# skit-ai/N-Best-ASR-Transformer

Hardware: AMD Instinct MI355X
Metric: utterances/sec fine-tune (bert-base, seq128, n_best=5) (higher is better)
Workload: dtype bf16

## Files before the change

### include/nbest_hip.h

```cpp
#ifndef NBEST_HIP_H
#define NBEST_HIP_H

#include <stddef.h>
#include <stdint.h>

#ifdef __cplusplus
extern "C" {
#endif

#define NBEST_ABI_VERSION 1

enum { NBEST_OK = 0, NBEST_ERR_ARG = -1, NBEST_ERR_SHAPE = -2, NBEST_ERR_DTYPE = -3, NBEST_ERR_ALIGN = -4,
       NBEST_ERR_LAUNCH = -5, NBEST_ERR_WORKSPACE = -6 };
enum { NBEST_F32 = 0, NBEST_BF16 = 1 };

typedef void* nbest_stream_t;

int nbest_version(void);
int nbest_last_error(char* buf, size_t n);

int nbest_embed_ln_fwd(const int64_t* ids, const int64_t* seg, const int64_t* pos, const void* word,
                       const void* type, const void* ptab, const float* gamma, const float* beta, void* out,
                       float* stats, int64_t M, int H, float eps, int dtype, float drop_p, uint64_t seed,
                       uint32_t drop_stream, nbest_stream_t stream);
int nbest_embed_ln_bwd(const int64_t* ids, const int64_t* seg, const int64_t* pos, const int32_t* perm, const void* word,
                       const void* type, const void* ptab, const float* gamma, const float* stats,
                       const void* dout, float* dword, float* dtype_tab, float* dptab, float* dgamma,
                       float* dbeta, int B, int S, int H, int n_types, int dtype, int64_t word_pad_id,
                       int64_t pos_pad_id, int accumulate, int tables_accumulate, float drop_p, uint64_t seed,
                       uint32_t drop_stream, void* ws, size_t ws_bytes, nbest_stream_t stream);
size_t nbest_embed_bwd_ws_bytes(int64_t M, int64_t H);
int nbest_embed_ln_fwd_interp(const int64_t* ids, const int64_t* base_ids, const float* alpha, const int64_t* seg, const int64_t* pos,
                              const void* word, const void* type, const void* ptab, const float* gamma, const float* beta, void* out,
                              float* stats, int B, int S, int H, float eps, int dtype, float drop_p, uint64_t seed, uint32_t drop_stream,
                              nbest_stream_t stream);
int nbest_embed_attrib(const int64_t* ids, const int64_t* base_ids, const float* alpha, const int64_t* seg, const int64_t* pos,
                       const void* word, const void* type, const void* ptab, const float* gamma, const void* dhidden, float* attr,
                       int pairs, int m, int S, int H, float eps, int dtype, nbest_stream_t stream);

int nbest_rows_gather(const float* table, const int64_t* rows, int64_t n_rows, int64_t cap, int64_t* ids_out, float* vals_out, int H,
                      nbest_stream_t stream);
int nbest_rows_zero(float* table, const int64_t* ids, int64_t n, int H, nbest_stream_t stream);
int nbest_rows_add(float* table, const int64_t* ids, const float* vals, int64_t n, int H, nbest_stream_t stream);

enum {
  NBEST_EPI_NONE = 0,
  NBEST_EPI_BIAS = 1,
  NBEST_EPI_BIAS_GELU = 2,
  NBEST_EPI_BIAS_DROP_RES = 3,
  NBEST_EPI_DGELU = 4,
  NBEST_EPI_RES = 5,
  NBEST_EPI_F32_SPLITK = 6
};
typedef struct nbest_gemm_args {
  const void* A;
  const void* B;
  void* C;
  const float* bias;
  const void* R;
  void* U;
  void* ws;
  size_t ws_bytes;
  int64_t M, N, K;
  int64_t lda, ldb, ldc, ldr, ldu;
  int32_t trans_a, trans_b;
  int32_t epilogue;
  int32_t dtype;
  int32_t accumulate;
  float drop_p;
  uint32_t drop_stream;
  uint64_t seed;
  float* colsum_out;
  int32_t colsum_accumulate;
  int32_t flags;
  const void* B_packed;
  int32_t b_pack_bn;
  int32_t pad_;
} nbest_gemm_args;
#define NBEST_GEMM_DEFER_REDUCE 1
size_t nbest_gemm_ws_bytes(const nbest_gemm_args* a);
int nbest_gemm(const nbest_gemm_args* a, nbest_stream_t stream);

size_t nbest_wgrad_pair_ws_bytes(const nbest_gemm_args* a, const nbest_gemm_args* b);
int nbest_wgrad_pair(const nbest_gemm_args* a, const nbest_gemm_args* b, nbest_stream_t stream);
int nbest_wgrad_group(const nbest_gemm_args* problems, int n, nbest_stream_t stream);

typedef struct nbest_gemm_fp8_args {
  const void* A;
  const void* B;
  void* C;
  const float* bias;
  const void* R;
  void* U;
  void* C8;
  int64_t M, N, K;
  int64_t lda, ldb, ldc, ldr, ldu, ldc8;
  int32_t epilogue;
  float out_scale;
  float drop_p;
  uint32_t drop_stream;
  uint64_t seed;
  const float* out_scale_dev;
  const uint32_t* a_amax;
  const uint32_t* c8_amax_prev;
  uint32_t* c8_amax_new;
  float* colsum_out;
  int32_t colsum_accumulate;
  int32_t pad;
  void* ws;
  size_t ws_bytes;
  const void* B_packed;
  int32_t b_pack_bn;
  int32_t pad3;
} nbest_gemm_fp8_args;
size_t nbest_gemm_fp8_ws_bytes(const nbest_gemm_fp8_args* a);
int nbest_gemm_fp8(const nbest_gemm_fp8_args* a, nbest_stream_t stream);
size_t nbest_wgrad_fp8_ws_bytes(int64_t M, int64_t N, int64_t K);
int nbest_wgrad_fp8(const void* dY8, const void* X8, float* dW, int64_t M, int64_t N, int64_t K, int64_t lda, int64_t ldb,
                    int64_t ldc, const uint32_t* a_amax, const uint32_t* x_amax, int accumulate, void* ws, size_t ws_bytes,
                    nbest_stream_t stream);
size_t nbest_wgrad_fp8_pair_ws_bytes(int64_t Ma, int64_t Mb, int64_t N, int64_t K);
int nbest_wgrad_fp8_pair(const void* dY8a, const void* X8a, float* dWa, int64_t Ma, int64_t lda_a, int64_t ldb_a, int64_t ldc_a,
                         const uint32_t* amax_a, const uint32_t* xamax_a, const void* dY8b, const void* X8b, float* dWb, int64_t Mb,
                         int64_t lda_b, int64_t ldb_b, int64_t ldc_b, const uint32_t* amax_b, const uint32_t* xamax_b, int64_t N, int64_t K,
                         int accumulate, void* ws, size_t ws_bytes, nbest_stream_t stream);
int nbest_cast_bf16_to_fp8(const void* src, void* dst, int64_t n, nbest_stream_t stream);

int nbest_attention_fwd(const void* qkv, const uint8_t* key_mask, void* ctx, float* lse, int B, int S,
                        int heads, int d, int dtype, float drop_p, uint64_t seed, uint32_t drop_stream,
                        nbest_stream_t stream);
// ... 75 lines not shown
int nbest_adam_clip_coef(const float* partial, int n_partial, float max_grad_norm, float* clip, nbest_stream_t stream);
int nbest_adam_update(int mode, float* p, const float* g, float* m, float* v, void* p_lowp, const nbest_tensor_desc* descs,
                      int n_tensors, int n_blocks, int blk_lo, int blk_hi, const float* clip, float lr_mult, float bc1,
                      float bc2_sqrt, double b1, double b2, float eps, nbest_stream_t stream);
int nbest_adam_step(int mode, float* p, float* g, float* m, float* v, void* p_lowp, const nbest_tensor_desc* descs,
                    int n_tensors, int n_blocks, float lr_mult, float bc1, float bc2_sqrt, double b1, double b2, float eps,
                    float max_grad_norm, void* ws, size_t ws_bytes, nbest_stream_t stream);
typedef struct nbest_matrix_desc {
  int64_t offset;
  int32_t rows, cols;
  int32_t tile_start, pad;
} nbest_matrix_desc;
#define NBEST_AMAX_TENSOR_WORDS 1024
int nbest_fp8_amax_fold(void* slots, void* out, int32_t n_tensors, nbest_stream_t stream);
int nbest_quantize_weights_fp8(const float* master, void* w8, void* w8t, const nbest_matrix_desc* descs, int n_matrices,
                               int n_tiles, float* inv_scale, void* ws, size_t ws_bytes, nbest_stream_t stream);
int nbest_transpose_weights(const void* src, void* dst, const nbest_matrix_desc* descs, int n_matrices, int n_tiles,
                            nbest_stream_t stream);
int nbest_pack_bn(int64_t N);
int nbest_pack_bn_fp8(int64_t N, int64_t K);
int nbest_pack_weights_fp8(const void* src, void* dst, const nbest_matrix_desc* descs, int n_matrices, int n_stages, nbest_stream_t stream);
int nbest_pack_weights(const void* src, void* dst, const nbest_matrix_desc* descs, int n_matrices, int n_stages, nbest_stream_t stream);
int nbest_cast_f32_to_bf16(const float* src, void* dst, int64_t n, nbest_stream_t stream);

typedef struct nbest_layer_offsets {
  int64_t wqkv, bqkv, wo, bo, ln1_g, ln1_b, w1, b1, w2, b2, ln2_g, ln2_b;
} nbest_layer_offsets;
typedef struct nbest_encoder_desc {
  int32_t dtype, B, S, H, L, heads, F;
  int32_t vocab, max_pos, n_types;
  float ln_eps, hidden_drop, attn_drop;
  int64_t word_pad_id, pos_pad_id;
  int64_t off_word, off_pos, off_type, off_emb_ln_g, off_emb_ln_b;
  const nbest_layer_offsets* layers_host;
  uint64_t seed;
  uint32_t drop_stream_base;
  int32_t wgrad_events_n;
  void** wgrad_events;
  const void* w8;
  const float* w8_inv_scale;
  const void* w8t;
  const uint32_t* gamax_prev;
  uint32_t* gamax_new;
  int32_t fp8_bwd;
  int32_t pad2;
  const void* wpk;
  const void* wpkt;
  const void* w8p;
  const void* w8tp;
  const int32_t* word_perm;
  const uint32_t* aamax_prev;
  uint32_t* aamax_new;
  int32_t fp8_act;
  int32_t pad4;
  int32_t first_trainable;
  int32_t no_input_grad;
  const uint8_t* wgrad_skip_host;
  const int64_t* base_ids;
  const float* alpha;
  int32_t no_param_grad;
  int32_t wgrad_group;
} nbest_encoder_desc;
enum { NBEST_WGRAD_GROUP_PLAN = 0, NBEST_WGRAD_GROUP_NEVER = 1, NBEST_WGRAD_GROUP_ALWAYS = 2 };
size_t nbest_encoder_act_bytes(const nbest_encoder_desc* d);
int nbest_encoder_act_view(const nbest_encoder_desc* d, void* act, int layer, void** qkv, float** lse);
size_t nbest_encoder_ws_bytes(const nbest_encoder_desc* d);
int nbest_encoder_wgrad_launches_per_layer(const nbest_encoder_desc* d);
int nbest_encoder_forward(const nbest_encoder_desc* d, const void* wts, const float* prm, const int64_t* ids,
                          const int64_t* seg, const int64_t* pos, const uint8_t* key_mask, void* act,
                          size_t act_bytes, void* ws, size_t ws_bytes, void** hidden_out, nbest_stream_t stream);
int nbest_encoder_backward(const nbest_encoder_desc* d, const void* wts, const void* wts_t, const float* prm, float* grad,
                           const int64_t* ids, const int64_t* seg, const int64_t* pos, const uint8_t* key_mask,
                           void* act, size_t act_bytes, void* dhidden, void* ws, size_t ws_bytes, int accumulate,
                           int layer_begin, int layer_end, int with_embeddings, nbest_stream_t stream);

size_t nbest_encoder_infer_ws_bytes(const nbest_encoder_desc* d);
int nbest_encoder_infer(const nbest_encoder_desc* d, const void* wts, const float* prm, const int64_t* ids, const int64_t* seg,
                        const int64_t* pos, const uint8_t* key_mask, void* ws, size_t ws_bytes, void* cls_out, nbest_stream_t stream);
int nbest_encoder_infer_attn(const nbest_encoder_desc* d, const void* wts, const float* prm, const int64_t* ids, const int64_t* seg,
                             const int64_t* pos, const uint8_t* key_mask, void* ws, size_t ws_bytes, void* cls_out, float* cls_attn,
                             nbest_stream_t stream);

#ifdef __cplusplus
}
#endif
#endif
```

### n-best-asr-transformer_amd/csrc/common.h

```cpp
#pragma once
#include <hip/hip_runtime.h>
#include <stdint.h>
#include <math.h>

#include "../../include/nbest_hip.h"
#include "internal.h"

typedef __bf16 bf16;
typedef __attribute__((ext_vector_type(2))) __bf16 bf16x2;
typedef __attribute__((ext_vector_type(4))) __bf16 bf16x4;
typedef __attribute__((ext_vector_type(8))) __bf16 bf16x8;
typedef __attribute__((ext_vector_type(2))) float f32x2;
typedef __attribute__((ext_vector_type(4))) float f32x4;
typedef __attribute__((ext_vector_type(16))) float f32x16;
typedef __attribute__((ext_vector_type(4))) int i32x4;
typedef __attribute__((ext_vector_type(2))) int i32x2;

#define LDS_PTR(p) ((void __attribute__((address_space(3)))*)(p))

#define NB_CHECK(cond, code, ...)            \
  do {                                       \
    if (!(cond)) {                           \
      nbest_set_error(__VA_ARGS__);          \
      return (code);                         \
// ... 236 lines not shown

struct Fp8Grad {
  uint8_t* out8;
  const uint32_t* amax_prev;
  uint32_t* amax_new;
};
__host__ __device__ __forceinline__ float fp8_pow2_scale(float amax, float target) {
  if (!(amax >= 7.8886e-31f) || !(amax <= 3.0e38f)) return 1.f;
  const float e = floorf(log2f(target / amax));
  return exp2f(e < -100.f ? -100.f : (e > 100.f ? 100.f : e));
}
__host__ __device__ __forceinline__ float fp8_scale_of(float amax) { return fp8_pow2_scale(amax, 224.f); }
__host__ __device__ __forceinline__ float fp8_gscale_of(float amax) { return fp8_pow2_scale(amax, 56.f); }
__device__ __forceinline__ float fp8_grad_scale(const uint32_t* amax_prev) { return amax_prev ? fp8_gscale_of(__uint_as_float(*amax_prev)) : 1.f; }
__host__ __device__ __forceinline__ float fp8_ascale_of(float amax) { return fp8_pow2_scale(amax, 224.f); }
__device__ __forceinline__ float fp8_act_scale(const uint32_t* amax_prev) { return amax_prev ? fp8_ascale_of(__uint_as_float(*amax_prev)) : 1.f; }
constexpr int kAmaxSlots = 16, kAmaxSlotStride = NBEST_AMAX_TENSOR_WORDS / 16;
__device__ __forceinline__ void amax_update(uint32_t* p, float v) {
  p += ((blockIdx.x + 5 * blockIdx.y + 3 * blockIdx.z) & (kAmaxSlots - 1)) * kAmaxSlotStride;
  const uint32_t b = __float_as_uint(v);
  if (b > __hip_atomic_load(p, __ATOMIC_RELAXED, __HIP_MEMORY_SCOPE_AGENT)) atomicMax(p, b);
}

__device__ __forceinline__ uint32_t nb_hash32(uint32_t x) {
  x ^= x >> 16; x *= 0x7feb352dU; x ^= x >> 15; x *= 0x846ca68bU; x ^= x >> 16;
  return x;
}
struct DropCfg {
  uint32_t thr16;
  float scale;
  uint32_t key;
};
__host__ __device__ __forceinline__ uint32_t nb_mix_key(uint64_t seed, uint32_t stream) {
  uint64_t z = seed + 0x9E3779B97F4A7C15ULL * (uint64_t)(stream + 1);
  z = (z ^ (z >> 30)) * 0xBF58476D1CE4E5B9ULL;
  z = (z ^ (z >> 27)) * 0x94D049BB133111EBULL;
  return (uint32_t)(z ^ (z >> 31));
}
__device__ __forceinline__ bool nb_keep(const DropCfg& d, uint32_t idx) {
  const uint32_t h = nb_hash32((idx >> 1) * 0x9E3779B9U + d.key);
  const uint32_t u = (idx & 1) ? (h >> 16) : (h & 0xFFFFu);
  return u >= d.thr16;
}
__device__ __forceinline__ uint32_t nb_keep2(const DropCfg& d, uint32_t idx) {
  const uint32_t h = nb_hash32((idx >> 1) * 0x9E3779B9U + d.key);
  return ((h & 0xFFFFu) >= d.thr16 ? 1u : 0u) | ((h >> 16) >= d.thr16 ? 2u : 0u);
}
__device__ __forceinline__ uint32_t nb_keep4(const DropCfg& d, uint32_t idx) {
  const uint32_t h0 = nb_hash32((idx >> 1) * 0x9E3779B9U + d.key);
  const uint32_t h1 = nb_hash32(((idx >> 1) + 1) * 0x9E3779B9U + d.key);
  return ((h0 & 0xFFFFu) >= d.thr16 ? 1u : 0u) | ((h0 >> 16) >= d.thr16 ? 2u : 0u) |
         ((h1 & 0xFFFFu) >= d.thr16 ? 4u : 0u) | ((h1 >> 16) >= d.thr16 ? 8u : 0u);
}
static inline DropCfg make_drop(float p, uint64_t seed, uint32_t stream) {
  DropCfg d;
  uint32_t thr = (p <= 0.f) ? 0u : (uint32_t)lrintf(p * 65536.0f);
  if (thr > 65535u) thr = 65535u;
  d.thr16 = thr;
  d.scale = 65536.0f / (float)(65536u - thr);
  d.key = nb_mix_key(seed, stream);
  return d;
}
```

### n-best-asr-transformer_amd/csrc/encoder.hip

```cpp
#include <algorithm>

#include "common.h"

namespace {

static inline size_t al(size_t x) { return (x + 255) & ~(size_t)255; }
static inline size_t take(size_t& o, size_t bytes) { const size_t at = o; o += bytes; return at; }

struct Sizes {
  size_t esz, MH, MF, M3H, MH8, MF8, st, lse;
  int64_t M;
};

static Sizes sizes(const nbest_encoder_desc* d) {
  Sizes z;
  z.esz = d->dtype == NBEST_BF16 ? 2 : 4;
  z.M = (int64_t)d->B * d->S;
  const size_t MHe = (size_t)z.M * d->H, MFe = (size_t)z.M * d->F;
  z.MH = al(MHe * z.esz); z.MF = al(MFe * z.esz); z.M3H = al(3 * MHe * z.esz);
  z.MH8 = al(MHe); z.MF8 = al(MFe);
  z.st = al((size_t)z.M * 2 * sizeof(float));
  z.lse = al((size_t)d->B * d->heads * d->S * sizeof(float));
  return z;
}

struct ActLayout {
  size_t X, emb_stats, layer0, layer_stride;
  size_t o_qkv, o_ctx, o_lse, o_r1, o_st1, o_x1, o_u, o_hact, o_r2, o_st2;
  size_t o_x8, o_ctx8, o_x18, o_h8;
  size_t o_keep, keep_bytes;
  size_t total;
  int K;
};

static int first_trainable(const nbest_encoder_desc* d) { return d->first_trainable < 0 ? 0 : (d->first_trainable > d->L ? d->L : d->first_trainable); }

static ActLayout act_layout(const nbest_encoder_desc* d, const Sizes& z) {
  ActLayout a;
  const bool bf16 = d->dtype == NBEST_BF16;
  a.K = first_trainable(d);
  size_t o = 0, p = 0;
  a.X = take(o, (size_t)(d->L + 1 - a.K) * z.MH);
  a.emb_stats = take(o, a.K ? 0 : z.st);
  a.layer0 = o;
  a.o_qkv = take(p, z.M3H); a.o_ctx = take(p, z.MH); a.o_lse = take(p, z.lse);
  a.o_r1 = take(p, z.MH); a.o_st1 = take(p, z.st); a.o_x1 = take(p, z.MH);
  a.o_u = take(p, bf16 ? z.MF8 : z.MF);
  a.o_hact = take(p, z.MF); a.o_r2 = take(p, z.MH); a.o_st2 = take(p, z.st);
  a.keep_bytes = bf16 ? nbest_internal_attention_keep_bytes(d->B, d->S, d->heads) : 0;
  a.o_keep = take(p, al(a.keep_bytes));
  a.o_x8 = a.o_ctx8 = a.o_x18 = a.o_h8 = 0;
  if (d->w8) {
    a.o_x8 = take(p, z.MH8); a.o_ctx8 = take(p, z.MH8); a.o_x18 = take(p, z.MH8); a.o_h8 = take(p, z.MF8);
  }
  a.layer_stride = p;
  a.total = o + (size_t)(d->L - a.K) * p;
  return a;
}

struct WsLayout {
  size_t dR, dRd, dB1, dctx, dBig, dqkv, red, slab, slab_bytes, red_bytes, emb, emb_bytes, f8, f8_bytes, total;
  size_t gset[2][4];
  size_t fz_x0, fz_x1, fz_emb_stats, fz_lse, fz_st1, fz_st2, fz_u;
};

static nbest_gemm_args wgrad_args(int dtype, int64_t rows, int64_t cols, int64_t tokens) {
  nbest_gemm_args g = {};
  g.M = rows; g.N = cols; g.K = tokens; g.lda = rows; g.ldb = cols; g.ldc = cols;
  g.trans_a = g.trans_b = 1; g.epilogue = NBEST_EPI_F32_SPLITK; g.dtype = dtype;
  return g;
}

static size_t wgrad_pair_bytes(const nbest_encoder_desc* d, bool fp8) {
  const int64_t H = d->H, M = (int64_t)d->B * d->S;
  if (fp8) return nbest_wgrad_fp8_pair_ws_bytes(3 * H, H, H, M);
  const nbest_gemm_args g1 = wgrad_args(NBEST_BF16, 3 * H, H, M), g2 = wgrad_args(NBEST_BF16, H, H, M);
  return nbest_wgrad_pair_ws_bytes(&g1, &g2);
}

static size_t max_splitk_bytes(const nbest_encoder_desc* d, int64_t M) {
  size_t mx = 0;
  const int64_t shapes[4][2] = {{3 * (int64_t)d->H, d->H}, {d->H, d->H}, {d->F, d->H}, {d->H, d->F}};
  for (int i = 0; i < 4; ++i) {
    const nbest_gemm_args g = wgrad_args(d->dtype, shapes[i][0], shapes[i][1], M);
    mx = std::max(mx, nbest_gemm_ws_bytes(&g));
    if (d->dtype == NBEST_BF16 && shapes[i][0] % 256 == 0 && shapes[i][1] % 256 == 0)
      mx = std::max(mx, nbest_wgrad_fp8_ws_bytes(shapes[i][0], shapes[i][1], M));
  }
// ... 73 lines not shown
  if (d->dtype == NBEST_BF16)
    NB_CHECK(d->H % 128 == 0 && d->F % 128 == 0, NBEST_ERR_SHAPE, "encoder(bf16): H and F must be multiples of 128");
  if (d->w8) NB_CHECK(d->dtype == NBEST_BF16 && d->w8_inv_scale && d->H % 256 == 0 && d->H <= 1024 && d->F % 256 == 0, NBEST_ERR_SHAPE,
                      "encoder(fp8 forward): needs the bf16 path, inverse scales and H, F multiples of 256");
  NB_CHECK(0 <= d->first_trainable && d->first_trainable <= d->L, NBEST_ERR_ARG, "encoder: first_trainable %d outside [0, L=%d]",
           d->first_trainable, d->L);
  NB_CHECK(!d->base_ids == !d->alpha, NBEST_ERR_ARG, "encoder: interpolated embeddings need both base_ids and alpha (or neither)");
  return NBEST_OK;
}

struct Ptrs {
  const char* wts;
  const float* prm;
  size_t esz;
  const void* W(int64_t off) const { return wts + (size_t)off * esz; }
  const float* P(int64_t off) const { return prm + off; }
};

#define RUN(x) do { int rc__ = (x); if (rc__) return rc__; } while (0)

static nbest_gemm_args gemm_nt(int dtype, const void* A, const void* B, void* C, int64_t M, int64_t N, int64_t K) {
  nbest_gemm_args g = {};
  g.A = A; g.B = B; g.C = C; g.dtype = dtype;
  g.M = M; g.N = N; g.K = K; g.lda = K; g.ldb = K; g.ldc = N;
  return g;
}

static void use_packed(nbest_gemm_args& g, const void* arena, int64_t off) {
  if (!arena || g.dtype != NBEST_BF16 || g.trans_a || g.trans_b) return;
  g.B_packed = (const char*)arena + off * 2;
  g.b_pack_bn = nbest_pack_bn(g.N);
}
static void use_packed(nbest_gemm_fp8_args& g, const void* arena, int64_t off) {
  if (!arena) return;
  g.B_packed = (const uint8_t*)arena + off;
  g.b_pack_bn = nbest_pack_bn_fp8(g.N, g.K);
}

struct GemmPass {
  int dtype; int64_t M; nbest_stream_t stream;
  uint64_t seed;
  Ptrs W; const void* packed; bool b_kn;
  bool fp8; const void *w8, *w8_packed; const float* inv_scale; const uint32_t* amax_prev; uint32_t* amax_new;
  void* colsum_ws; size_t colsum_ws_bytes; int accumulate;
};
struct GemmOp {
  const void* A; const uint8_t* A8; int a_idx;
  int64_t w_off; int mat;
  void* C; int64_t N, K; int epilogue;
  const float* bias;
  const void* R; float drop_p; uint32_t drop_stream;
  void* U; float* colsum;
  uint8_t* C8; int c_idx;
};

static int layer_gemm(const GemmPass& c, const GemmOp& o) {
  if (c.fp8) {
    nbest_gemm_fp8_args g = {};
    g.A = o.A8; g.B = (const uint8_t*)c.w8 + o.w_off; g.C = o.C; g.bias = o.bias; g.R = o.R; g.U = o.U; g.C8 = o.C8;
    g.M = c.M; g.N = o.N; g.K = o.K;
    g.lda = g.ldb = o.K; g.ldc = g.ldr = g.ldu = g.ldc8 = o.N;
    use_packed(g, c.w8_packed, o.w_off);
    g.epilogue = o.epilogue; g.out_scale = 1.f; g.out_scale_dev = c.inv_scale + o.mat;
    g.drop_p = o.drop_p; g.drop_stream = o.drop_stream; g.seed = c.seed;
    g.a_amax = c.amax_prev + o.a_idx;
    if (o.C8) {
      g.c8_amax_prev = c.amax_prev + o.c_idx;
      g.c8_amax_new = c.amax_new ? c.amax_new + (int64_t)o.c_idx * NBEST_AMAX_TENSOR_WORDS : nullptr;
    }
    g.colsum_out = o.colsum; g.colsum_accumulate = c.accumulate; g.ws = c.colsum_ws; g.ws_bytes = c.colsum_ws_bytes;
    return nbest_gemm_fp8(&g, c.stream);
  }
  nbest_gemm_args g = gemm_nt(c.dtype, o.A, c.W.W(o.w_off), o.C, c.M, o.N, o.K);
  if (c.b_kn) { g.trans_b = 1; g.ldb = o.N; }
  g.epilogue = o.epilogue; g.bias = o.bias;
  if (o.R) { g.R = o.R; g.ldr = o.N; }
  if (o.epilogue == NBEST_EPI_BIAS_DROP_RES) { g.drop_p = o.drop_p; g.drop_stream = o.drop_stream; g.seed = c.seed; }
  if (o.epilogue == NBEST_EPI_BIAS_GELU || o.epilogue == NBEST_EPI_DGELU) { g.U = o.U; g.ldu = o.N; }
  if (o.epilogue == NBEST_EPI_DGELU) {
    g.colsum_out = o.colsum; g.colsum_accumulate = g.accumulate = c.accumulate; g.ws = c.colsum_ws; g.ws_bytes = c.colsum_ws_bytes;
  }
  use_packed(g, c.packed, o.w_off);
  return nbest_gemm(&g, c.stream);
}

struct LayerBufs {
  void *qkv, *ctx, *r1, *x1, *u, *hact, *r2;
  float *lse, *st1, *st2;
  uint32_t* keep;
  uint8_t *x8, *ctx8, *x18, *h8;
};

static LayerBufs stashed_layer(const nbest_encoder_desc* d, const ActLayout& a, void* act, int l) {
  char* Lb = (char*)act + a.layer0 + (size_t)(l - a.K) * a.layer_stride;
  LayerBufs b = {};
  b.qkv = Lb + a.o_qkv; b.ctx = Lb + a.o_ctx; b.lse = (float*)(Lb + a.o_lse);
  b.r1 = Lb + a.o_r1; b.st1 = (float*)(Lb + a.o_st1); b.x1 = Lb + a.o_x1;
  b.u = Lb + a.o_u; b.r2 = Lb + a.o_r2; b.st2 = (float*)(Lb + a.o_st2);
  b.hact = fp8_backward_active(d) ? nullptr : Lb + a.o_hact;
  if (a.keep_bytes && d->attn_drop > 0.f) b.keep = (uint32_t*)(Lb + a.o_keep);
  if (fp8_forward_active(d)) {
    b.x8 = (uint8_t*)(Lb + a.o_x8); b.ctx8 = (uint8_t*)(Lb + a.o_ctx8);
    b.x18 = (uint8_t*)(Lb + a.o_x18); b.h8 = (uint8_t*)(Lb + a.o_h8);
  }
  return b;
}

static LayerBufs frozen_layer(const nbest_encoder_desc* d, const WsLayout& w, const Sizes& z, void* ws) {
  char* W = (char*)ws;
  const bool f8 = fp8_forward_active(d);
  LayerBufs b = {};
  b.qkv = W + w.dqkv; b.ctx = W + w.dctx; b.lse = (float*)(W + w.fz_lse);
  b.r1 = W + w.dR; b.st1 = (float*)(W + w.fz_st1); b.x1 = W + w.dRd;
  b.r2 = W + w.dB1; b.st2 = (float*)(W + w.fz_st2);
  b.u = f8 ? W + w.fz_u : nullptr; b.hact = f8 ? nullptr : W + w.dBig;
  if (f8) { b.x8 = (uint8_t*)(W + w.f8); b.ctx8 = b.x8 + z.MH8; b.x18 = b.ctx8 + z.MH8; b.h8 = b.x18 + z.MH8; }
  return b;
}

struct Fwd {
  const nbest_encoder_desc* d;
  GemmPass g;
  const uint8_t* key_mask;
  bool arec;
  const uint32_t* AP(int idx) const { return g.fp8 ? d->aamax_prev + idx : nullptr; }
  uint32_t* AN(int idx) const { return (g.fp8 && arec) ? d->aamax_new + (int64_t)idx * NBEST_AMAX_TENSOR_WORDS : nullptr; }
  int calib(const void* t, int64_t n, int idx) const {
    if (!arec || g.fp8) return NBEST_OK;
    return nbest_internal_amax_bf16(t, n, d->aamax_new + (int64_t)idx * NBEST_AMAX_TENSOR_WORDS, (hipStream_t)g.stream);
  }
};

static Fwd make_fwd(const nbest_encoder_desc* d, const void* wts, const float* prm, const Sizes& z, const uint8_t* key_mask,
                    nbest_stream_t stream) {
  const GemmPass g = {d->dtype, z.M, stream, d->seed, Ptrs{(const char*)wts, prm, z.esz}, d->wpk, false, fp8_forward_active(d),
                      d->w8, d->w8p, d->w8_inv_scale, d->aamax_prev, d->aamax_new, nullptr, 0, 0};
  return Fwd{d, g, key_mask, d->w8 && d->aamax_new && d->dtype == NBEST_BF16};
}

static int layer_forward(const Fwd& c, int l, const void* xin, void* xout, const LayerBufs& b, uint8_t* x8_next, float* cls_probs) {
  const nbest_encoder_desc* d = c.d;
  const nbest_layer_offsets& o = d->layers_host[l];
  const Ptrs& P = c.g.W;
  const nbest_stream_t stream = c.g.stream;
  const int64_t M = c.g.M;
  const int H = d->H, F = d->F, dt = d->dtype, t = 4 * l;
  const uint32_t s0 = d->drop_stream_base + 1 + 4 * l;
  if (c.g.fp8 && l == 0)
    RUN(nbest_internal_cast_bf16_to_fp8(xin, b.x8, M * H, c.AP(0), c.AN(0), (hipStream_t)stream));
  const GemmOp wqkv = {xin, b.x8, t + 0, o.wqkv, t + 0, b.qkv, 3 * H, H, NBEST_EPI_BIAS, P.P(o.bqkv)};
  RUN(layer_gemm(c.g, wqkv));
  if (cls_probs)
    RUN(nbest_internal_attention_cls_probs(b.qkv, (int64_t)d->S * H * 3, (const char*)b.qkv + H * P.esz, 3 * H, c.key_mask, cls_probs, d->S,
                                           d->B, d->S, d->heads, 64, dt, stream));
  RUN(c.calib(xin, M * H, t + 0));
  RUN(nbest_internal_attention_fwd8(b.qkv, c.key_mask, b.ctx, b.ctx8, b.lse, d->B, d->S, d->heads, 64, dt, d->attn_drop, d->seed, s0 + 0,
                                    stream, b.keep, c.AP(t + 1), c.AN(t + 1)));
  RUN(c.calib(b.ctx, M * H, t + 1));
  GemmOp wo = {b.ctx, b.ctx8, t + 1, o.wo, t + 1, b.r1, H, H, NBEST_EPI_BIAS_DROP_RES, P.P(o.bo)};
  wo.R = xin; wo.drop_p = d->hidden_drop; wo.drop_stream = s0 + 1;
  RUN(layer_gemm(c.g, wo));
  RUN(nbest_internal_layernorm_fwd8(b.r1, P.P(o.ln1_g), P.P(o.ln1_b), b.x1, b.x18, b.st1, M, H, d->ln_eps, dt, stream, c.AP(t + 2), c.AN(t + 2)));
  RUN(c.calib(b.x1, M * H, t + 2));
  GemmOp w1 = {b.x1, b.x18, t + 2, o.w1, t + 2, b.hact, F, H, NBEST_EPI_BIAS_GELU, P.P(o.b1)};
  w1.U = b.u; w1.C8 = b.h8; w1.c_idx = t + 3;
  RUN(layer_gemm(c.g, w1));
  GemmOp w2 = {b.hact, b.h8, t + 3, o.w2, t + 3, b.r2, H, F, NBEST_EPI_BIAS_DROP_RES, P.P(o.b2)};
  w2.R = b.x1; w2.drop_p = d->hidden_drop; w2.drop_stream = s0 + 2;
  RUN(layer_gemm(c.g, w2));
  RUN(c.calib(b.hact, M * F, t + 3));
  RUN(nbest_internal_layernorm_fwd8(b.r2, P.P(o.ln2_g), P.P(o.ln2_b), xout, x8_next, b.st2, M, H, d->ln_eps, dt, stream,
                                    x8_next ? c.AP(t + 4) : nullptr, x8_next ? c.AN(t + 4) : nullptr));
  return NBEST_OK;
}

}

extern "C" size_t nbest_encoder_act_bytes(const nbest_encoder_desc* d) { return d ? act_layout(d, sizes(d)).total : 0; }

extern "C" int nbest_encoder_act_view(const nbest_encoder_desc* d, void* act, int layer, void** qkv, float** lse) {
  RUN(check_desc(d));
  NB_CHECK(act && qkv && lse, NBEST_ERR_ARG, "encoder_act_view: null pointer");
  NB_CHECK(0 <= layer && layer < d->L, NBEST_ERR_ARG, "encoder_act_view: layer %d outside [0, L=%d)", layer, d->L);
  const ActLayout a = act_layout(d, sizes(d));
  NB_CHECK(layer >= a.K, NBEST_ERR_ARG, "encoder_act_view: layer %d < first_trainable %d (frozen layers are not stashed)", layer, a.K);
  const LayerBufs b = stashed_layer(d, a, act, layer);
  *qkv = b.qkv; *lse = b.lse;
  return NBEST_OK;
}
extern "C" size_t nbest_encoder_ws_bytes(const nbest_encoder_desc* d) { return d ? ws_layout(d, sizes(d)).total : 0; }
extern "C" int nbest_encoder_wgrad_launches_per_layer(const nbest_encoder_desc* d) {
  if (!d) return 0;
  if (wgrad_group_layers(d) > 0) return 1;
  return wgrad_paired(d, fp8_backward_active(d)) ? 3 : 4;
}

extern "C" int nbest_encoder_forward(const nbest_encoder_desc* d, const void* wts, const float* prm, const int64_t* ids,
                                     const int64_t* seg, const int64_t* pos, const uint8_t* key_mask, void* act, size_t act_bytes,
                                     void* ws, size_t ws_bytes, void** hidden_out, nbest_stream_t stream) {
  RUN(check_desc(d));
  NB_CHECK(wts && prm && ids && pos && key_mask && act, NBEST_ERR_ARG, "encoder_forward: null pointer");
  const Sizes z = sizes(d);
  const ActLayout a = act_layout(d, z);
  NB_CHECK(act_bytes >= a.total, NBEST_ERR_WORKSPACE, "encoder_forward: activation stash too small (%zu < %zu)", act_bytes, a.total);
  const Fwd c = make_fwd(d, wts, prm, z, key_mask, stream);
  const WsLayout wl = ws_layout(d, z);
  const int FT = a.K;
  if (c.g.fp8 || FT > 0)
    NB_CHECK(ws && ws_bytes >= wl.total, NBEST_ERR_WORKSPACE, "encoder_forward(%s): workspace too small (%zu < %zu)",
             FT > 0 ? "first_trainable > 0" : "fp8", ws_bytes, wl.total);
  const Ptrs& P = c.g.W;
  char *A = (char*)act, *W = (char*)ws;
  const int H = d->H, dt = d->dtype;
  auto X = [&](int l) { return l >= FT ? (void*)(A + a.X + (size_t)(l - FT) * z.MH) : (void*)(W + ((l & 1) ? wl.fz_x1 : wl.fz_x0)); };
  auto bufs = [&](int l) { return l >= FT ? stashed_layer(d, a, act, l) : frozen_layer(d, wl, z, ws); };

  float* emb_stats = (float*)(FT > 0 ? W + wl.fz_emb_stats : A + a.emb_stats);
  if (d->base_ids)
    RUN(nbest_embed_ln_fwd_interp(ids, d->base_ids, d->alpha, seg, pos, P.W(d->off_word), P.W(d->off_type), P.W(d->off_pos),
                                  P.P(d->off_emb_ln_g), P.P(d->off_emb_ln_b), X(0), emb_stats, d->B, d->S, H, d->ln_eps, dt,
                                  d->hidden_drop, d->seed, d->drop_stream_base, (hipStream_t)stream));
  else
    RUN(nbest_embed_ln_fwd(ids, seg, pos, P.W(d->off_word), P.W(d->off_type), P.W(d->off_pos), P.P(d->off_emb_ln_g),
                           P.P(d->off_emb_ln_b), X(0), emb_stats, z.M, H, d->ln_eps, dt, d->hidden_drop, d->seed, d->drop_stream_base,
                           (hipStream_t)stream));
  for (int l = 0; l < d->L; ++l) {
    uint8_t* x8_next = (l + 1 < d->L) ? bufs(l + 1).x8 : nullptr;
    RUN(layer_forward(c, l, X(l), X(l + 1), bufs(l), x8_next, nullptr));
  }
  if (hidden_out) *hidden_out = X(d->L);
  return NBEST_OK;
}

namespace {
struct WGrad {
  const void *dY, *X;
  const uint8_t *dY8, *X8;
  int64_t w_off, rows, cols;
  int g_idx, a_idx;
};
}

extern "C" int nbest_encoder_backward(const nbest_encoder_desc* d, const void* wts, const void* wts_t, const float* prm, float* grad,
                                      const int64_t* ids, const int64_t* seg, const int64_t* pos, const uint8_t* key_mask,
                                      void* act, size_t act_bytes, void* dhidden, void* ws, size_t ws_bytes, int accumulate,
                                      int layer_begin, int layer_end, int with_embeddings, nbest_stream_t stream) {
  RUN(check_desc(d));
  NB_CHECK(0 <= layer_begin && layer_begin <= layer_end && layer_end <= d->L, NBEST_ERR_ARG, "encoder_backward: bad layer range");
  const bool npg = d->no_param_grad != 0;
  NB_CHECK(!npg || (!with_embeddings && d->first_trainable == 0 && !d->no_input_grad && !d->w8), NBEST_ERR_ARG,
           "encoder_backward: no_param_grad refuses with_embeddings (%d), first_trainable > 0 (%d), no_input_grad (%d) and the fp8 "
           "forward (w8): it forms the input gradient only, of a full stash", with_embeddings, d->first_trainable, d->no_input_grad);
  NB_CHECK(wts && prm && (grad || npg) && ids && pos && key_mask && act && dhidden && ws, NBEST_ERR_ARG, "encoder_backward: null pointer");
  NB_CHECK(!with_embeddings || d->word_perm, NBEST_ERR_ARG, "encoder_backward: desc.word_perm (stable argsort of this pass's ids) is required");
  NB_CHECK(layer_begin >= d->first_trainable, NBEST_ERR_ARG, "encoder_backward: layer_begin %d < first_trainable %d (those layers are not stashed)",
           layer_begin, d->first_trainable);
  NB_CHECK(!with_embeddings || (d->first_trainable == 0 && !d->no_input_grad), NBEST_ERR_ARG,
           "encoder_backward: with_embeddings needs first_trainable == 0 and no_input_grad == 0");
  const Sizes z = sizes(d);
  const ActLayout a = act_layout(d, z);
  const WsLayout w = ws_layout(d, z);
  NB_CHECK(act_bytes >= a.total, NBEST_ERR_WORKSPACE, "encoder_backward: activation stash too small");
  NB_CHECK(ws_bytes >= w.total, NBEST_ERR_WORKSPACE, "encoder_backward: workspace too small (%zu < %zu)", ws_bytes, w.total);
  hipStream_t st = (hipStream_t)stream;
  const Ptrs P{(const char*)wts, prm, z.esz};
  const bool wt = (wts_t != nullptr);
  char *A = (char*)act, *W = (char*)ws;
  const int64_t M = z.M;
  const int H = d->H, F = d->F, dt = d->dtype;
  const int FT = a.K;
  auto X = [&](int l) { return (void*)(A + a.X + (size_t)(l - FT) * z.MH); };
  auto G = [&](int64_t off) { return grad + off; };
  auto GP = [&](int64_t off) -> float* { return npg ? nullptr : grad + off; };
  auto skip = [&](int l, int j) -> bool { return npg || (d->wgrad_skip_host && d->wgrad_skip_host[4 * l + j]); };
  void* dA = dhidden; void* dR = W + w.dR;
  const bool hdrop = d->hidden_drop > 0.f;
  void* dRd = hdrop ? (void*)(W + w.dRd) : dR;
  void* dB1 = W + w.dB1; void* dctx = W + w.dctx; void* dBig = W + w.dBig; void* dqkv = W + w.dqkv;
  void* red = W + w.red; void* slab = W + w.slab;
  void* red1 = W + w.red + w.red_bytes; void* red2 = W + w.red + 2 * w.red_bytes; void* red3 = W + w.red + 3 * w.red_bytes;
  const bool f8b = fp8_backward_active(d);
  const bool paired = wgrad_paired(d, f8b);
  const int gl = wgrad_group_layers(d);
  const bool grouped = gl > 0;
  int ev_i = (grouped ? 1 : paired ? 3 : 4) * (d->L - layer_end);
  auto stamp = [&](int which) {
    if (d->wgrad_events && 2 * ev_i + which < d->wgrad_events_n) (void)hipEventRecord((hipEvent_t)d->wgrad_events[2 * ev_i + which], st);
    ev_i += which;
  };

  const bool rec = !npg && d->gamax_new && dt == NBEST_BF16;
  uint8_t* dqkv8 = f8b ? (uint8_t*)W + w.f8 : nullptr;
  uint8_t* dBig8 = f8b ? dqkv8 + 3 * z.MH8 : nullptr;
  uint8_t* dRd8 = f8b ? dBig8 + z.MF8 : nullptr;
  auto GN = [&](int idx) { return d->gamax_new + (int64_t)idx * NBEST_AMAX_TENSOR_WORDS; };
  auto fg = [&](uint8_t* out8, int idx) -> Fp8Grad {
    if (!rec) return Fp8Grad{nullptr, nullptr, nullptr};
    return Fp8Grad{f8b ? out8 : nullptr, f8b ? d->gamax_prev + idx : nullptr, GN(idx)};
  };
  const GemmPass dg = {dt, M, stream, 0, Ptrs{(const char*)(wt ? wts_t : wts), prm, z.esz}, wt ? d->wpkt : nullptr, !wt, f8b,
                       d->w8t, d->w8tp, d->w8_inv_scale, d->gamax_prev, d->gamax_new, red1, w.red_bytes, accumulate};
  auto wgrad_args_of = [&](const WGrad* x) {
    nbest_gemm_args g = wgrad_args(dt, x->rows, x->cols, M);
    g.A = x->dY; g.B = x->X; g.C = G(x->w_off); g.accumulate = accumulate;
    return g;
  };
  auto wgrad_launch = [&](int l, const WGrad* wg, int j, int j2) -> int {
    const WGrad* p = skip(l, j) ? nullptr : wg + j;
    const WGrad* q = (j2 >= 0 && !skip(l, j2)) ? wg + j2 : nullptr;
    if (!p) { p = q; q = nullptr; }
    if (p && f8b) {
      const uint32_t *gp = d->gamax_prev, *ap = d->aamax_prev;
      if (q)
        RUN(nbest_wgrad_fp8_pair(p->dY8, p->X8, G(p->w_off), p->rows, p->rows, p->cols, p->cols, gp + p->g_idx, ap + p->a_idx, q->dY8, q->X8,
                                 G(q->w_off), q->rows, q->rows, q->cols, q->cols, gp + q->g_idx, ap + q->a_idx, p->cols, M, accumulate, slab,
                                 w.slab_bytes, stream));
      else
        RUN(nbest_wgrad_fp8(p->dY8, p->X8, G(p->w_off), p->rows, p->cols, M, p->rows, p->cols, p->cols, gp + p->g_idx, ap + p->a_idx,
                            accumulate, slab, w.slab_bytes, stream));
    } else if (p) {
      nbest_gemm_args g1 = wgrad_args_of(p), g2 = wgrad_args_of(q ? q : p);
      g1.ws = slab; g1.ws_bytes = w.slab_bytes;
      RUN(q ? nbest_wgrad_pair(&g1, &g2, stream) : nbest_gemm(&g1, stream));
    }
    return NBEST_OK;
  };
  auto wgrad = [&](int l, const WGrad* wg, int j, int j2) -> int {
    stamp(0);
    RUN(wgrad_launch(l, wg, j, j2));
    stamp(1);
    return NBEST_OK;
  };
  nbest_gemm_args pend[8];
  int n_pend = 0;

  struct BatchGuard { ~BatchGuard() { nbest_internal_rowred_batch_abort(); } } batch_guard;
  for (int l = layer_end - 1; l >= layer_begin; --l) {
    const nbest_layer_offsets& o = d->layers_host[l];
    const LayerBufs b = stashed_layer(d, a, act, l);
    const bool input_grad = !(d->no_input_grad && l == FT);
    const int t = 4 * l;
    const uint32_t s0 = d->drop_stream_base + 1 + 4 * l;
    const int gpos = grouped ? (layer_end - 1 - l) % gl : 0;
    const bool group_ends = grouped && (gpos == gl - 1 || l == layer_begin);
    void *dR2 = dR, *dR1 = dR, *dRd2 = dRd, *dRd1 = dRd, *dBigL = dBig, *dqkvL = dqkv;
    if (grouped) {
      dRd2 = W + w.gset[gpos][0]; dBigL = W + w.gset[gpos][1]; dRd1 = W + w.gset[gpos][2]; dqkvL = W + w.gset[gpos][3];
      if (!hdrop) { dR2 = dRd2; dR1 = dRd1; }
    }
    const WGrad wg[4] = {{dqkvL, X(l), dqkv8, b.x8, o.wqkv, 3 * H, H, t + 3, t + 0},
                         {dRd1, b.ctx, dRd8, b.ctx8, o.wo, H, H, t + 2, t + 1},
                         {dBigL, b.x1, dBig8, b.x18, o.w1, F, H, t + 1, t + 2},
                         {dRd2, b.hact, dRd8, b.h8, o.w2, H, F, t + 0, t + 3}};
    if (!npg) nbest_internal_rowred_batch_begin();
    RUN(nbest_internal_layernorm_bwd8(dA, b.r2, b.st2, P.P(o.ln2_g), dR2, (hdrop && !f8b) ? dRd2 : nullptr, GP(o.ln2_g), GP(o.ln2_b), GP(o.b2), M, H,
                                      dt, accumulate, d->hidden_drop, d->seed, s0 + 2, red, w.red_bytes, stream, fg(dRd8, t + 0)));
    GemmOp dw2 = {dRd2, dRd8, t + 0, o.w2, t + 3, f8b ? nullptr : dBigL, F, H, NBEST_EPI_DGELU};
    dw2.U = b.u; dw2.colsum = GP(o.b1); dw2.C8 = dBig8; dw2.c_idx = t + 1;
    RUN(layer_gemm(dg, dw2));
    if (rec && !f8b) RUN(nbest_internal_amax_bf16(dBigL, M * F, GN(t + 1), st));
    if (!grouped) RUN(wgrad(l, wg, 3, -1));
    GemmOp dw1 = {dBigL, dBig8, t + 1, o.w1, t + 2, dB1, H, F, NBEST_EPI_RES};
    dw1.R = dR2;
    RUN(layer_gemm(dg, dw1));
    if (!grouped) RUN(wgrad(l, wg, 2, -1));
    RUN(nbest_internal_layernorm_bwd8(dB1, b.r1, b.st1, P.P(o.ln1_g), dR1, (hdrop && !f8b) ? dRd1 : nullptr, GP(o.ln1_g), GP(o.ln1_b), GP(o.bo), M, H,
                                      dt, accumulate, d->hidden_drop, d->seed, s0 + 1, red2, w.red_bytes, stream, fg(dRd8, t + 2)));
    const GemmOp dwo = {dRd1, dRd8, t + 2, o.wo, t + 1, dctx, H, H, NBEST_EPI_NONE};
    RUN(layer_gemm(dg, dwo));
    if (!paired && !grouped) RUN(wgrad(l, wg, 1, -1));
    RUN(nbest_internal_attention_bwd8(b.qkv, key_mask, b.ctx, dctx, b.lse, f8b ? nullptr : dqkvL, GP(o.bqkv), accumulate, red3, w.red_bytes, d->B, d->S,
                                      d->heads, 64, dt, d->attn_drop, d->seed, s0 + 0, stream, fg(dqkv8, t + 3), b.keep));
    if (input_grad) {
      GemmOp dwqkv = {dqkvL, dqkv8, t + 3, o.wqkv, t + 0, dA, H, 3 * H, NBEST_EPI_RES};
      dwqkv.R = dR1;
      RUN(layer_gemm(dg, dwqkv));
    }
    if (!grouped) {
      RUN(wgrad(l, wg, 0, paired ? 1 : -1));
    } else if (group_ends && gpos + 1 < gl && d->wgrad_group != NBEST_WGRAD_GROUP_ALWAYS) {
      stamp(0);
      RUN(wgrad_launch(l, wg, 3, -1));
      RUN(wgrad_launch(l, wg, 2, -1));
      if (!paired) RUN(wgrad_launch(l, wg, 1, -1));
      RUN(wgrad_launch(l, wg, 0, paired ? 1 : -1));
      stamp(1);
    } else {
      for (int j = 0; j < 4; ++j)
        if (!skip(l, j)) pend[n_pend++] = wgrad_args_of(wg + j);
      if (group_ends) {
        stamp(0);
        if (n_pend) RUN(nbest_wgrad_group(pend, n_pend, stream));
        stamp(1);
        for (int i = 0; i < gpos; ++i) { stamp(0); stamp(1); }
        n_pend = 0;
      }
    }
    if (!npg) RUN(nbest_internal_rowred_batch_flush(st));
  }
  if (!with_embeddings) return NBEST_OK;
  if (!accumulate) {
    hipError_t e = hipMemsetAsync(G(d->off_word), 0, (size_t)d->vocab * H * sizeof(float), st);
    if (e == hipSuccess) e = hipMemsetAsync(G(d->off_pos), 0, (size_t)d->max_pos * H * sizeof(float), st);
    if (e == hipSuccess) e = hipMemsetAsync(G(d->off_type), 0, (size_t)d->n_types * H * sizeof(float), st);
    NB_CHECK(e == hipSuccess, NBEST_ERR_LAUNCH, "encoder_backward: memset failed: %s", hipGetErrorString(e));
  }
  RUN(nbest_embed_ln_bwd(ids, seg, pos, d->word_perm, P.W(d->off_word), P.W(d->off_type), P.W(d->off_pos), P.P(d->off_emb_ln_g),
                         (const float*)(A + a.emb_stats), dA, G(d->off_word), G(d->off_type), G(d->off_pos), G(d->off_emb_ln_g),
                         G(d->off_emb_ln_b), d->B, d->S, H, d->n_types, dt, d->word_pad_id, d->pos_pad_id, accumulate, accumulate,
                         d->hidden_drop, d->seed, d->drop_stream_base, W + w.emb, w.emb_bytes, stream));
  return NBEST_OK;
}

namespace {
struct InferLayout {
  size_t X0, X1, emb_stats, qkv, ctx, r1, x1, r2, hact, lse, st1, st2, total;
};
static InferLayout infer_layout(const Sizes& z) {
  InferLayout w;
  size_t o = 0;
  w.X0 = take(o, z.MH); w.X1 = take(o, z.MH); w.emb_stats = take(o, z.st);
  w.qkv = take(o, z.M3H); w.ctx = take(o, z.MH); w.r1 = take(o, z.MH); w.x1 = take(o, z.MH); w.r2 = take(o, z.MH);
  w.hact = take(o, z.MF); w.lse = take(o, z.lse); w.st1 = take(o, z.st); w.st2 = take(o, z.st);
  w.total = o;
  return w;
}
static LayerBufs infer_layer(const InferLayout& w, void* ws) {
  char* W = (char*)ws;
  LayerBufs b = {};
  b.qkv = W + w.qkv; b.ctx = W + w.ctx; b.lse = (float*)(W + w.lse);
  b.r1 = W + w.r1; b.st1 = (float*)(W + w.st1); b.x1 = W + w.x1;
  b.hact = W + w.hact; b.r2 = W + w.r2; b.st2 = (float*)(W + w.st2);
  return b;
}
}

extern "C" size_t nbest_encoder_infer_ws_bytes(const nbest_encoder_desc* d) { return d ? infer_layout(sizes(d)).total : 0; }

extern "C" int nbest_encoder_infer_attn(const nbest_encoder_desc* d, const void* wts, const float* prm, const int64_t* ids, const int64_t* seg,
                                        const int64_t* pos, const uint8_t* key_mask, void* ws, size_t ws_bytes, void* cls_out,
                                        float* cls_attn, nbest_stream_t stream) {
  RUN(check_desc(d));
// ... 54 lines not shown
```

### n-best-asr-transformer_amd/csrc/gemm.hip

```cpp
#include "common.h"

namespace {

__global__ __launch_bounds__(256) void splitk_reduce_kernel(const float* __restrict__ slab, float* __restrict__ C, int64_t MN,
                                                            int64_t N, int64_t ldc, int splits, int accumulate,
                                                            float* __restrict__ C2, int64_t m_split, int64_t ldc2) {
  for (int64_t i = ((int64_t)blockIdx.x * blockDim.x + threadIdx.x) * 4; i < MN; i += (int64_t)gridDim.x * blockDim.x * 4) {
    f32x4 s = *(const f32x4*)(slab + i);
    for (int z = 1; z < splits; ++z) s += *(const f32x4*)(slab + (int64_t)z * MN + i);
    const int64_t m = i / N, n = i - m * N;
    float* c = (m < m_split) ? C + m * ldc + n : C2 + (m - m_split) * ldc2 + n;
    if (accumulate) s += *(const f32x4*)c;
    *(f32x4*)c = s;
  }
}

int check_epilogue_operands(const nbest_gemm_args* a, int64_t ld_mult, uintptr_t align) {
  const int epi = a->epilogue;
  if (epi == NBEST_EPI_BIAS || epi == NBEST_EPI_BIAS_GELU || epi == NBEST_EPI_BIAS_DROP_RES)
    NB_CHECK(a->bias, NBEST_ERR_ARG, "gemm: epilogue %d needs bias", epi);
  if (epi == NBEST_EPI_BIAS_DROP_RES || epi == NBEST_EPI_RES)
    NB_CHECK(a->R && a->ldr % ld_mult == 0 && ((uintptr_t)a->R & (align - 1)) == 0, NBEST_ERR_ARG, "gemm: epilogue %d needs R", epi);
  if ((epi == NBEST_EPI_BIAS_GELU && a->U) || epi == NBEST_EPI_DGELU)
    NB_CHECK(a->U && a->ldu % ld_mult == 0 && ((uintptr_t)a->U & (align - 1)) == 0, NBEST_ERR_ARG, "gemm: epilogue %d needs U", epi);
  return NBEST_OK;
}

int check_bf16(const nbest_gemm_args* a) {
  NB_CHECK(!(a->trans_a && !a->trans_b), NBEST_ERR_ARG, "gemm(bf16): trans_a without trans_b is not built");
  NB_CHECK(!a->trans_a || a->M % 128 == 0, NBEST_ERR_SHAPE, "gemm(bf16): trans_a needs M %% 128 == 0");
  NB_CHECK(a->lda % 8 == 0 && a->ldb % 8 == 0 && a->ldc % 8 == 0, NBEST_ERR_ALIGN, "gemm(bf16): leading dimensions must be multiples of 8");
  NB_CHECK(((uintptr_t)a->A & 15) == 0 && ((uintptr_t)a->B & 15) == 0 && ((uintptr_t)a->C & 15) == 0, NBEST_ERR_ALIGN,
           "gemm(bf16): pointers must be 16-byte aligned");
  const int64_t a_rows = a->trans_a ? a->K : a->M, a_cols = a->trans_a ? a->M : a->K;
  const int64_t b_rows = a->trans_b ? a->K : a->N, b_cols = a->trans_b ? a->N : a->K;
  const int64_t ab = ((a_rows - 1) * a->lda + a_cols) * 2, bb = ((b_rows - 1) * a->ldb + b_cols) * 2;
  NB_CHECK(ab < ((int64_t)1 << 32) && bb < ((int64_t)1 << 32), NBEST_ERR_SHAPE, "gemm(bf16): operand larger than 4 GiB");
  NB_CHECK(a->M * a->N < ((int64_t)1 << 32) || make_drop(a->drop_p, a->seed, a->drop_stream).thr16 == 0, NBEST_ERR_SHAPE,
           "gemm(bf16): dropout counter overflow");
  return check_epilogue_operands(a, 8, 16);
}

}

void nb_splitk_plan(int64_t tiles, int64_t K, int64_t slots, int64_t min_blocks, int* splits, int64_t* k_per_split) {
  const int64_t maxs = (K / 512 < 1) ? 1 : ((K / 512 > 32) ? 32 : K / 512);
  int64_t best_s = 1;
  double best = -1.0;
  for (int64_t s = 1; s <= maxs; ++s) {
    const int64_t blocks = tiles * s;
    const double eff = (double)blocks / (double)(((blocks + slots - 1) / slots) * slots);
    if (eff > best + 1e-9) { best = eff; best_s = s; }
    if (blocks >= min_blocks && eff >= 0.93) { best_s = s; break; }
  }
  const int64_t k = round_up((K + best_s - 1) / best_s, 64);
  *splits = (int)((K + k - 1) / k);
  *k_per_split = k;
}

int nbest_internal_splitk_reduce(const float* slab, float* C, int64_t M, int64_t N, int64_t ldc, int splits, int accumulate,
                                 float* C2, int64_t m_split, int64_t ldc2, hipStream_t st) {
  const int64_t MN = M * N;
  int64_t g = (MN / 4 + 255) / 256;
  if (g > 2048) g = 2048;
  splitk_reduce_kernel<<<(int)g, 256, 0, st>>>(slab, C, MN, N, ldc, splits, accumulate, C2, m_split, ldc2);
  NB_LAUNCH_CHECK();
  return NBEST_OK;
}

extern "C" size_t nbest_gemm_ws_bytes(const nbest_gemm_args* a) {
  if (!a) return 0;
  if (a->dtype == NBEST_F32) return (a->colsum_out && a->epilogue != NBEST_EPI_F32_SPLITK) ? nbest_rowred_ws_bytes(a->M, a->N) : 0;
  if (a->dtype != NBEST_BF16) return 0;
  const size_t w1 = nbest_gemm_bf16_ws_bytes(a), w2 = nbest_gemm_bf16_v2_ws_bytes(a);
  return w1 > w2 ? w1 : w2;
}

extern "C" int nbest_gemm(const nbest_gemm_args* a, nbest_stream_t stream) {
  NB_CHECK(a && a->A && a->B && a->C, NBEST_ERR_ARG, "gemm: null pointer");
  NB_CHECK(a->M > 0 && a->N > 0 && a->K > 0, NBEST_ERR_SHAPE, "gemm: bad shape %lld x %lld x %lld", (long long)a->M,
           (long long)a->N, (long long)a->K);
  if (a->dtype == NBEST_F32) {
    if (int rc = check_epilogue_operands(a, 1, 1)) return rc;
    if (int rc = nbest_gemm_f32(a, (hipStream_t)stream)) return rc;
    if (a->colsum_out && a->epilogue != NBEST_EPI_F32_SPLITK) {
      NB_CHECK(a->ws && a->ws_bytes >= nbest_rowred_ws_bytes(a->M, a->N), NBEST_ERR_WORKSPACE, "gemm(f32): column-sum workspace too small");
      return nbest_colsum(a->C, a->colsum_out, a->M, a->N, a->ldc, NBEST_F32, a->colsum_accumulate, a->ws, a->ws_bytes, stream);
    }
    return NBEST_OK;
  }
  if (a->dtype == NBEST_BF16) {
    if (int rc = check_bf16(a)) return rc;
// ... 43 lines not shown
```

### n-best-asr-transformer_amd/csrc/gemm_bf16.hip

```cpp
#include "common.h"

namespace {

constexpr int BM = 128, BN = 128, BK = 64;
constexpr int kTileBytes = BM * BK * 2;
constexpr int kStageBytes = 2 * kTileBytes;
constexpr int kLdsBytes = 2 * kStageBytes;

struct GemmP {
  const bf16* A; const bf16* B; void* C; const float* bias; const bf16* R; bf16* U; float* slab; float* colpart;
  int64_t M, N, K, lda, ldb, ldc, ldr, ldu;
  int64_t k_per_split;
  int tiles_m, tiles_n, splits, accumulate;
  uint32_t a_bytes, b_bytes;
  DropCfg drop;
  int stream_out;
  int gn;
};

template <bool TR>
__device__ __forceinline__ void stage_tile(__amdgpu_buffer_rsrc_t rs, char* lds_tile, int64_t row0, int64_t k0, int64_t ld,
                                           int tid) {
  const int wave = tid >> 6;
#pragma unroll
  for (int i = 0; i < 4; ++i) {
    const int p = i * 256 + tid;
    uint32_t voff;
    if (!TR) {
      const int row = p >> 3, slot = p & 7;
      const int kc = slot ^ ((row >> 1) & 7);
      voff = (uint32_t)(((row0 + row) * ld + k0 + kc * 8) * 2);
    } else {
      const int krow = p >> 4, slot = p & 15;
      const int mc = slot ^ (2 * (krow & 3) + 8 * ((krow >> 3) & 1));
      voff = (uint32_t)(((k0 + krow) * ld + row0 + mc * 8) * 2);
    }
    char* dst = lds_tile + (i * 256 + wave * 64) * 16;
    __builtin_amdgcn_raw_ptr_buffer_load_lds(rs, LDS_PTR(dst), 16, voff, 0, 0, 0);
  }
}

template <bool TR>
__device__ __forceinline__ bf16x8 read_frag(const char* lds_tile, int row_base, int ks, int lane) {
  if (!TR) {
    const int row = row_base + (lane & 15);
    const int kc = (lane >> 4) + 4 * ks;
    return *(const bf16x8*)(lds_tile + row * 128 + ((kc ^ ((row >> 1) & 7)) << 4));
  } else {
    const int g = lane >> 4, i = lane & 15, q = i >> 2, pq = i & 3;
    const int col = row_base + 4 * pq;
    bf16x8 out;
#pragma unroll
    for (int half = 0; half < 2; ++half) {
      const int krow = 32 * ks + 8 * g + 4 * half + q;
      const int f = 2 * (krow & 3) + 8 * ((krow >> 3) & 1);
      const char* addr = lds_tile + krow * 256 + (((col >> 3) ^ f) << 4) + ((col & 4) ? 8 : 0);
      bf16x4 v = __builtin_amdgcn_ds_read_tr16_b64_v4bf16((bf16x4 __attribute__((address_space(3)))*)addr);
      out[4 * half + 0] = v[0]; out[4 * half + 1] = v[1]; out[4 * half + 2] = v[2]; out[4 * half + 3] = v[3];
    }
    return out;
  }
}

template <bool TA, bool TB, int EPI>
__global__ __launch_bounds__(256) void gemm_bf16_kernel(GemmP p) {
// ... 64 lines not shown
      }
      if (kt + 1 < nk) {
        char* nxt = lds + ((kt + 1) & 1) * kStageBytes;
        const int64_t k0 = kbeg + (int64_t)(kt + 1) * BK;
        stage_tile<TA>(rsA, nxt, m0, k0, p.lda, tid);
        stage_tile<TB>(rsB, nxt + kTileBytes, n0, k0, p.ldb, tid);
      }
#pragma unroll
      for (int ks = 0; ks < 2; ++ks)
#pragma unroll
        for (int i = 0; i < 4; ++i)
#pragma unroll
          for (int j = 0; j < 4; ++j)
            acc[i][j] = __builtin_amdgcn_mfma_f32_16x16x32_bf16(bfr[ks][j], af[ks][i], acc[i][j], 0, 0, 0);
    } else {
      if (kt + 1 < nk) {
        char* nxt = lds + ((kt + 1) & 1) * kStageBytes;
        const int64_t k0 = kbeg + (int64_t)(kt + 1) * BK;
        stage_tile<TA>(rsA, nxt, m0, k0, p.lda, tid);
        stage_tile<TB>(rsB, nxt + kTileBytes, n0, k0, p.ldb, tid);
      }
#pragma unroll
      for (int ks = 0; ks < 2; ++ks) {
        bf16x8 af[4], bfr[4];
#pragma unroll
        for (int i = 0; i < 4; ++i) af[i] = read_frag<TA>(cur, wm * 64 + i * 16, ks, lane);
#pragma unroll
        for (int j = 0; j < 4; ++j) bfr[j] = read_frag<TB>(cur + kTileBytes, wn * 64 + j * 16, ks, lane);
#pragma unroll
        for (int i = 0; i < 4; ++i)
#pragma unroll
          for (int j = 0; j < 4; ++j)
            acc[i][j] = __builtin_amdgcn_mfma_f32_16x16x32_bf16(bfr[j], af[i], acc[i][j], 0, 0, 0);
      }
    }
  }

  __syncthreads();
  float* ep = (float*)lds + wave * 4096;
#pragma unroll
  for (int i = 0; i < 4; ++i) {
    const int row = i * 16 + (lane & 15);
#pragma unroll
    for (int j = 0; j < 4; ++j) {
      const int c = j * 4 + (lane >> 4);
      *(f32x4*)(ep + row * 64 + ((c ^ (row & 15)) << 2)) = acc[i][j];
    }
  }
  asm volatile("s_waitcnt lgkmcnt(0)" ::: "memory");
  float colacc[8] = {0, 0, 0, 0, 0, 0, 0, 0};
  const int64_t er0 = m0 + wm * 64 + (lane >> 3), ec8 = n0 + wn * 64 + (lane & 7) * 8;
  int64_t oC = er0 * p.ldc + ec8, oU = er0 * p.ldu + ec8, oS = ((int64_t)z * p.M + er0) * p.N + ec8;
  const int64_t sC = 8 * p.ldc, sU = 8 * p.ldu, sS = 8 * p.N;
  uint32_t dbase = (uint32_t)(er0 * p.N + ec8);
  const uint32_t sD = 8u * (uint32_t)p.N;
#pragma unroll
  for (int it = 0; it < 8; ++it, oC += sC, oU += sU, oS += sS, dbase += sD) {
    const int pidx = it * 64 + lane, row = pidx >> 3, c8 = pidx & 7;
    const int64_t m = m0 + wm * 64 + row;
    f32x4 v0 = *(const f32x4*)(ep + row * 64 + (((2 * c8) ^ (row & 15)) << 2));
    f32x4 v1 = *(const f32x4*)(ep + row * 64 + (((2 * c8 + 1) ^ (row & 15)) << 2));
    if (m >= p.M) continue;
    if (EPI == NBEST_EPI_F32_SPLITK) {
      float* c = (p.splits > 1) ? p.slab + oS : (float*)p.C + oC;
      if (p.splits == 1 && p.accumulate) { v0 += *(const f32x4*)c; v1 += *(const f32x4*)(c + 4); }
      *(f32x4*)c = v0;
      *(f32x4*)(c + 4) = v1;
      continue;
    }
    float v[8] = {v0[0], v0[1], v0[2], v0[3], v1[0], v1[1], v1[2], v1[3]};
    if (kHasBias) {
#pragma unroll
      for (int e = 0; e < 4; ++e) { v[e] += pb0[e]; v[4 + e] += pb1[e]; }
    }
    if (EPI == kEpiBiasGeluNoU) {
#pragma unroll
      for (int e = 0; e < 8; e += 2) {
        f32x2 h2, g2;
        gelu_pair_fast(f32x2{v[e], v[e + 1]}, h2, g2);
        v[e] = h2[0]; v[e + 1] = h2[1];
      }
    }
    if (EPI == NBEST_EPI_BIAS_GELU) {
      float gp[8];
#pragma unroll
      for (int e = 0; e < 8; e += 2) {
        f32x2 h2, g2;
        gelu_pair_fast(f32x2{v[e], v[e + 1]}, h2, g2);
        gp[e] = g2[0]; gp[e + 1] = g2[1]; v[e] = h2[0]; v[e + 1] = h2[1];
      }
      st_stream((i32x2*)((uint8_t*)p.U + oU), i32x2{(int)gd_pack4(gp), (int)gd_pack4(gp + 4)}, p.stream_out);
    }
    if (EPI == NBEST_EPI_BIAS_DROP_RES) {
      if (p.drop.thr16) {
        const uint32_t k = nb_keep4(p.drop, dbase) | (nb_keep4(p.drop, dbase + 4) << 4);
#pragma unroll
        for (int e = 0; e < 8; ++e) v[e] = (k >> e & 1) ? v[e] * p.drop.scale : 0.f;
      }
    }
    if (EPI == NBEST_EPI_BIAS_DROP_RES || EPI == NBEST_EPI_RES) {
      const bf16x8 r = __builtin_bit_cast(bf16x8, pre[it]);
#pragma unroll
      for (int e = 0; e < 8; ++e) v[e] += (float)r[e];
    }
    if (EPI == NBEST_EPI_DGELU) {
      float gd[8];
      gd_unpack4((uint32_t)pre[it][0], gd);
      gd_unpack4((uint32_t)pre[it][1], gd + 4);
// ... 27 lines not shown
  if (a->epilogue == NBEST_EPI_F32_SPLITK) nb_splitk_plan(((a->M + BM - 1) / BM) * (a->N / BN), a->K, 512, 400, splits, kps);
}

template <bool TA, bool TB>
static int launch_epi(const GemmP& p, int epi, int grid, hipStream_t st) {
#define L(E)                                                                          \
  case E:                                                                             \
    (void)hipFuncSetAttribute((const void*)gemm_bf16_kernel<TA, TB, E>, hipFuncAttributeMaxDynamicSharedMemorySize, kLdsBytes); \
    gemm_bf16_kernel<TA, TB, E><<<grid, 256, kLdsBytes, st>>>(p);                      \
    break;
  switch (epi) {
    L(NBEST_EPI_NONE) L(NBEST_EPI_BIAS) L(NBEST_EPI_BIAS_GELU) L(NBEST_EPI_BIAS_DROP_RES) L(NBEST_EPI_DGELU)
    L(NBEST_EPI_RES) L(NBEST_EPI_F32_SPLITK) L(kEpiBiasGeluNoU)
    default:
      nbest_set_error("gemm: bad epilogue %d", epi);
      return NBEST_ERR_ARG;
  }
#undef L
  NB_LAUNCH_CHECK();
  return NBEST_OK;
}

}

size_t nbest_gemm_bf16_ws_bytes(const nbest_gemm_args* a) {
  if (a->epilogue != NBEST_EPI_F32_SPLITK) return a->colsum_out ? (size_t)((a->M + BM - 1) / BM) * 2 * a->N * sizeof(float) : 0;
  int splits;
  int64_t kps;
  plan_splits(a, &splits, &kps);
  return splits > 1 ? (size_t)splits * a->M * a->N * sizeof(float) : 0;
}

int nbest_gemm_bf16(const nbest_gemm_args* a, hipStream_t st) {
  NB_CHECK(a->N % BN == 0, NBEST_ERR_SHAPE, "gemm(bf16): N=%lld must be a multiple of %d", (long long)a->N, BN);
  NB_CHECK(a->trans_a || a->K % BK == 0, NBEST_ERR_SHAPE, "gemm(bf16): K=%lld must be a multiple of %d", (long long)a->K, BK);
  GemmP p;
  p.A = (const bf16*)a->A; p.B = (const bf16*)a->B; p.C = a->C; p.bias = a->bias; p.R = (const bf16*)a->R; p.U = (bf16*)a->U;
  p.M = a->M; p.N = a->N; p.K = a->K; p.lda = a->lda; p.ldb = a->ldb; p.ldc = a->ldc; p.ldr = a->ldr; p.ldu = a->ldu;
  p.tiles_m = (int)((a->M + BM - 1) / BM);
  p.tiles_n = (int)(a->N / BN);
  plan_splits(a, &p.splits, &p.k_per_split);
  p.accumulate = a->accumulate;
  p.slab = (float*)a->ws;
  p.colpart = nullptr;
  if (a->colsum_out && a->epilogue != NBEST_EPI_F32_SPLITK) {
    NB_CHECK(a->ws && a->ws_bytes >= nbest_gemm_bf16_ws_bytes(a), NBEST_ERR_WORKSPACE, "gemm: column-sum workspace too small");
    p.colpart = (float*)a->ws;
  }
  const int64_t a_rows = a->trans_a ? a->K : a->M, a_cols = a->trans_a ? a->M : a->K;
  const int64_t b_rows = a->trans_b ? a->K : a->N, b_cols = a->trans_b ? a->N : a->K;
  const int64_t ab = ((a_rows - 1) * a->lda + a_cols) * 2, bb = ((b_rows - 1) * a->ldb + b_cols) * 2;
  p.a_bytes = (uint32_t)ab; p.b_bytes = (uint32_t)bb;
  p.drop = make_drop(a->drop_p, a->seed, a->drop_stream);
  p.stream_out = 1;
  p.gn = (int)(a->N / BN);
  const int epi = a->epilogue;
  if (epi == NBEST_EPI_F32_SPLITK && p.splits > 1)
    NB_CHECK(a->ws && a->ws_bytes >= (size_t)p.splits * a->M * a->N * sizeof(float), NBEST_ERR_WORKSPACE,
             "gemm: split-K workspace too small (%zu < %zu)", a->ws_bytes, (size_t)p.splits * a->M * a->N * sizeof(float));
  const int grid = p.tiles_m * p.tiles_n * p.splits;
  int rc;
  const int kepi = nb_kernel_epilogue(epi, a->U);
  if (!a->trans_a && !a->trans_b) rc = launch_epi<false, false>(p, kepi, grid, st);
  else if (!a->trans_a && a->trans_b) rc = launch_epi<false, true>(p, kepi, grid, st);
  else rc = launch_epi<true, true>(p, kepi, grid, st);
  if (rc) return rc;
  if (p.colpart) return nbest_internal_partial_rows_sum(p.colpart, p.tiles_m * 2, (int)a->N, a->colsum_out, a->colsum_accumulate, st);
  if (epi == NBEST_EPI_F32_SPLITK && p.splits > 1 && !(a->flags & NBEST_GEMM_DEFER_REDUCE))
    return nbest_internal_splitk_reduce(p.slab, (float*)a->C, a->M, a->N, a->ldc, p.splits, a->accumulate, nullptr, a->M, 0, st);
  return NBEST_OK;
}
```

### n-best-asr-transformer_amd/csrc/gemm_bf16_v2.hip

```cpp
#include "common.h"
#include <type_traits>

namespace {

constexpr int BK = 32;

struct GemmP2 {
  const bf16* A; const bf16* B; void* C; const float* bias; const bf16* R; bf16* U; float* slab; float* colpart;
  int64_t M, N, K, lda, ldb, ldc, ldr, ldu;
  int64_t k_per_split;
  int tiles_m, tiles_n, splits, accumulate;
  uint32_t a_bytes, b_bytes;
  uint32_t c_bytes, r_bytes, u_bytes;
  DropCfg drop;
  int stream_out;
  int gn;
  const bf16* A2; const bf16* B2;
  int64_t lda2, ldb2, m_split;
  uint32_t a2_bytes, b2_bytes;
  const bf16* Bp;
  uint32_t bp_bytes;
  int bp_bn;
};

template <bool TR, int ROWS, int NT, int PW = 0>
__device__ __forceinline__ void stage_tile2(__amdgpu_buffer_rsrc_t rs, char* tile, int64_t row0, int64_t k0, int64_t ld, int tid,
                                            char* dump = nullptr) {
  const int wave = tid >> 6;
  constexpr int NI = (ROWS * 4 + NT - 1) / NT;
#pragma unroll
  for (int i = 0; i < NI; ++i) {
    const int p = i * NT + tid;
    uint32_t voff;
    if (!TR) {
      const int row = p >> 2, slot = p & 3;
      const int kc = slot ^ ((-(row >> 2)) & 3);
      int grow = row;
      if constexpr (PW > 0) { const int x = row % PW; grow = row - x + (PW / 16) * (x & 15) + (x >> 4); }
      voff = (uint32_t)(((row0 + grow) * ld + k0 + kc * 8) * 2);

    } else {
      constexpr int CPR = ROWS / 8;
      const int krow = p / CPR, slot = p % CPR;
      const int mc = slot ^ (2 * (krow & 3) + 8 * ((krow >> 3) & 1));
      voff = (uint32_t)(((k0 + krow) * ld + row0 + mc * 8) * 2);
    }
    char* dst = tile + (i * NT + wave * 64) * 16;
    if constexpr ((ROWS * 4) % NT != 0) {
      if (i == NI - 1 && (i * NT + wave * 64) * 16 >= ROWS * 64) {
        voff = 0xFFFFFFF0u;
        dst = dump + (wave % (NT / 64)) * 1024;
      }
    }
    __builtin_amdgcn_raw_ptr_buffer_load_lds(rs, LDS_PTR(dst), 16, voff, 0, 0, 0);
  }
}

template <int ROWS, int NT>
__device__ __forceinline__ void stage_tile_packed(__amdgpu_buffer_rsrc_t rs, char* tile, uint32_t stage_byte0, int tid, char* dump = nullptr) {
  const int wave = tid >> 6;
  constexpr int NI = (ROWS * 4 + NT - 1) / NT;
#pragma unroll
  for (int i = 0; i < NI; ++i) {
// ... 503 lines not shown
      __builtin_amdgcn_sched_barrier(0);
      __builtin_amdgcn_s_barrier();
      __builtin_amdgcn_sched_barrier(0);
      buf = (buf + 1 == STAGES) ? 0 : buf + 1;
    }
    if (grp == 0) __builtin_amdgcn_s_barrier();
  } else {
#pragma unroll
  for (int s = 0; s < STAGES - 1; ++s) {
    if (s < nk) {
      stage_tile2<TA, BM, NT>(rsA, lds + s * STAGE, m0a, kbeg + (int64_t)s * BK, lda_, tid);
      stage_tile2<TB, BN, NT, kPW>(rsB, lds + s * STAGE + A_BYTES, n0, kbeg + (int64_t)s * BK, ldb_, tid);
    }
  }
  int buf = 0;
  for (int kt = 0; kt < nk; ++kt) {
    const int younger = (nk - 1 - kt < STAGES - 2) ? nk - 1 - kt : STAGES - 2;
    if (STAGES >= 4 && younger == 2) wait_vm<2 * NDMA>();
    else if (younger >= 1) wait_vm<NDMA>();
    else wait_vm<0>();
    __builtin_amdgcn_s_barrier();
    asm volatile("" ::: "memory");
    if (kt + STAGES - 1 < nk) {
      int nb = buf + STAGES - 1;
      if (nb >= STAGES) nb -= STAGES;
      const int64_t k0 = kbeg + (int64_t)(kt + STAGES - 1) * BK;
      stage_tile2<TA, BM, NT>(rsA, lds + nb * STAGE, m0a, k0, lda_, tid);
      stage_tile2<TB, BN, NT, kPW>(rsB, lds + nb * STAGE + A_BYTES, n0, k0, ldb_, tid, lds + STAGES * STAGE);
    }
    const char* cur = lds + buf * STAGE;
    bf16x8 af[TMt], bfr[TNt];
#pragma unroll
    for (int j = 0; j < TNt; ++j) bfr[j] = read_frag2<TB, BN>(cur + A_BYTES, wn * WTN + j * 16, lane);
#pragma unroll
    for (int i = 0; i < TMt; ++i) af[i] = read_frag2<TA, BM>(cur, wm * WTM + i * 16, lane);
#pragma unroll
    for (int i = 0; i < TMt; ++i)
#pragma unroll
      for (int j = 0; j < TNt; ++j) acc[i][j] = kDirect ? __builtin_amdgcn_mfma_f32_16x16x32_bf16(af[i], bfr[j], acc[i][j], 0, 0, 0)
                                : __builtin_amdgcn_mfma_f32_16x16x32_bf16(bfr[j], af[i], acc[i][j], 0, 0, 0);
    buf = (buf + 1 == STAGES) ? 0 : buf + 1;
  }
  }

  if constexpr (kDirect) {
    if (kHasR || kHasUin) {
#pragma unroll
      for (int i = 1; i < TMt; ++i) load_dpre(i);
    }
    float colacc[TNt];
#pragma unroll
    for (int j = 0; j < TNt; ++j) colacc[j] = 0.f;
    const uint32_t voC = (uint32_t)((drow0 * p.ldc + dcol) * 2), svC = (uint32_t)(2 * p.ldc);
    const uint32_t dbase0 = (uint32_t)(drow0 * p.N + dcol), sD = (uint32_t)p.N;
    constexpr bool kCols = (EPI == NBEST_EPI_DGELU);
    const bool want_cols = kCols && p.colpart != nullptr;
#pragma unroll
    for (int i = 0; i < TMt; ++i) {
#pragma unroll
      for (int e = 0; e < 4; ++e) {
        const uint32_t rr = (uint32_t)(16 * i + e);
        float v[TNt];
#pragma unroll
        for (int j = 0; j < TNt; ++j) v[j] = acc[i][j][e];
        if (kHasBias) {
#pragma unroll
          for (int j = 0; j < TNt; ++j) v[j] += db[j];
        }
        if (EPI == kEpiBiasGeluNoU) {
#pragma unroll
          for (int j = 0; j < TNt; j += 2) {
            f32x2 h2, g2;
            gelu_pair_fast(f32x2{v[j], v[j + 1]}, h2, g2);
            v[j] = h2[0]; v[j + 1] = h2[1];
          }
        }
        if (EPI == NBEST_EPI_BIAS_GELU) {
          float gp[TNt];
#pragma unroll
          for (int j = 0; j < TNt; j += 2) {
            f32x2 h2, g2;
            gelu_pair_fast(f32x2{v[j], v[j + 1]}, h2, g2);
            gp[j] = g2[0]; gp[j + 1] = g2[1]; v[j] = h2[0]; v[j + 1] = h2[1];
          }
          if constexpr (TNt == 8) nb_bstore8(rsU, voU + rr * svU, gd_pack4(gp), gd_pack4(gp + 4));
          else __builtin_amdgcn_raw_buffer_store_b32(gd_pack4(gp), rsU, voU + rr * svU, 0, 2);
        }
        if (EPI == NBEST_EPI_BIAS_DROP_RES && p.drop.thr16) {
          const uint32_t dbase = dbase0 + rr * sD;
          uint32_t k = 0;
#pragma unroll
          for (int q = 0; q < TNt / 2; ++q) k |= nb_keep2(p.drop, dbase + 2 * q) << (2 * q);
#pragma unroll
          for (int j = 0; j < TNt; ++j) v[j] = (k >> j & 1) ? v[j] * p.drop.scale : 0.f;
        }
        if (kHasR) {
          const bf16x8 r8 = __builtin_bit_cast(bf16x8, dpre[i][e]);
#pragma unroll
          for (int j = 0; j < TNt; ++j) v[j] += (float)r8[j];
        }
        if (kHasUin) {
          float gd[8];
          gd_unpack4(dpre[i][e][0], gd);
          if constexpr (TNt == 8) gd_unpack4(dpre[i][e][1], gd + 4);
#pragma unroll
          for (int j = 0; j < TNt; ++j) v[j] *= gd[j];
        }
        if constexpr (TNt == 8) nb_bstore_bf16x8(rsC, voC + rr * svC, v);
        else if constexpr (TNt == 6) {
          bf16x2 o0 = {(bf16)v[0], (bf16)v[1]}, o1 = {(bf16)v[2], (bf16)v[3]}, o2 = {(bf16)v[4], (bf16)v[5]};
          __builtin_amdgcn_raw_buffer_store_b96(u32x3{__builtin_bit_cast(uint32_t, o0), __builtin_bit_cast(uint32_t, o1), __builtin_bit_cast(uint32_t, o2)},
                                                rsC, voC + rr * svC, 0, 2);
        } else {
          bf16x4 o;
#pragma unroll
          for (int j = 0; j < 4; ++j) o[j] = (bf16)v[j];
          __builtin_amdgcn_raw_buffer_store_b64(__builtin_bit_cast(u32x2, o), rsC, voC + rr * svC, 0, 2);
        }
        if constexpr (kCols) {
          const bool live = want_cols && (drow0 + rr) < p.M;
#pragma unroll
          for (int j = 0; j < TNt; ++j) colacc[j] += live ? v[j] : 0.f;
        }
      }
    }
    if (kCols && want_cols) {
#pragma unroll
      for (int j = 0; j < TNt; ++j) {
        float x = colacc[j];
        x += __shfl_xor(x, 16, 64); x += __shfl_xor(x, 32, 64);
        colacc[j] = x;
      }
      if (dg == 0) {
        float* o = p.colpart + ((int64_t)tile_m * WM + wm) * p.N + dcol;
#pragma unroll
        for (int q = 0; q < TNt / 2; ++q) *(f32x2*)(o + 2 * q) = f32x2{colacc[2 * q], colacc[2 * q + 1]};
      }
    }
    return;
  }
  float* ep = (float*)lds + wave * 2048;
  float colacc[8] = {0, 0, 0, 0, 0, 0, 0, 0};
  if (kPre) {
#pragma unroll
    for (int c = 1; c < TMt / 2; ++c)
#pragma unroll
      for (int it = 0; it < 4; ++it) pre[c][it] = load_pre(erow0 + c * 32 + it * 8);
  }
  __builtin_amdgcn_s_barrier();
  asm volatile("" ::: "memory");
  int64_t oC = erow0 * p.ldc + en8, oU = erow0 * p.ldu + en8;
  int64_t oS = ((int64_t)z * p.M + erow0) * p.N + en8;
  const int64_t sC = 8 * p.ldc, sU = 8 * p.ldu, sS = 8 * p.N;
  uint32_t dbase = (uint32_t)(erow0 * p.N + en8);
  const uint32_t sD = 8u * (uint32_t)p.N;
#pragma unroll
  for (int c = 0; c < TMt / 2; ++c) {
#pragma unroll
    for (int ii = 0; ii < 2; ++ii) {
      const int row = ii * 16 + (lane & 15);
#pragma unroll
      for (int j = 0; j < TNt; ++j) {
        const int cidx = j * 4 + (lane >> 4);
        *(f32x4*)(ep + row * 64 + ((cidx ^ (row & 15)) << 2)) = acc[2 * c + ii][j];
      }
    }
    asm volatile("s_waitcnt lgkmcnt(0)" ::: "memory");
#pragma unroll
    for (int it = 0; it < 4; ++it) {
      const int pidx = it * 64 + lane, row = pidx >> 3, c8 = pidx & 7;
      const int64_t m = m0 + wm * WTM + c * 32 + row;
      f32x4 v0 = *(const f32x4*)(ep + row * 64 + (((2 * c8) ^ (row & 15)) << 2));
      f32x4 v1 = *(const f32x4*)(ep + row * 64 + (((2 * c8 + 1) ^ (row & 15)) << 2));
      if (m < p.M) {
      if (EPI == NBEST_EPI_F32_SPLITK) {
        float* cp = (p.splits > 1) ? p.slab + oS : (float*)p.C + oC;
        if (p.splits == 1 && p.accumulate) { v0 += *(const f32x4*)cp; v1 += *(const f32x4*)(cp + 4); }
        *(f32x4*)cp = v0;
        *(f32x4*)(cp + 4) = v1;
      } else {
      float v[8] = {v0[0], v0[1], v0[2], v0[3], v1[0], v1[1], v1[2], v1[3]};
      if (kHasBias) {
#pragma unroll
        for (int e = 0; e < 4; ++e) { v[e] += pb0[e]; v[4 + e] += pb1[e]; }
      }
      if (EPI == kEpiBiasGeluNoU) {
#pragma unroll
        for (int e = 0; e < 8; e += 2) {
          f32x2 h2, g2;
          gelu_pair_fast(f32x2{v[e], v[e + 1]}, h2, g2);
          v[e] = h2[0]; v[e + 1] = h2[1];
        }
      }
      if (EPI == NBEST_EPI_BIAS_GELU) {
        float gp[8];
#pragma unroll
        for (int e = 0; e < 8; e += 2) {
          f32x2 h2, g2;
          gelu_pair_fast(f32x2{v[e], v[e + 1]}, h2, g2);
          gp[e] = g2[0]; gp[e + 1] = g2[1]; v[e] = h2[0]; v[e + 1] = h2[1];
        }
        st_stream((i32x2*)((uint8_t*)p.U + oU), i32x2{(int)gd_pack4(gp), (int)gd_pack4(gp + 4)}, p.stream_out);
      }
      if (EPI == NBEST_EPI_BIAS_DROP_RES && p.drop.thr16) {
        const uint32_t k = nb_keep4(p.drop, dbase) | (nb_keep4(p.drop, dbase + 4) << 4);
#pragma unroll
        for (int e = 0; e < 8; ++e) v[e] = (k >> e & 1) ? v[e] * p.drop.scale : 0.f;
      }
// ... 188 lines not shown
  const Plan pl = make_plan(a);
  return pl.splits > 1 ? (size_t)pl.splits * a->M * a->N * sizeof(float) : 0;
}

static int gemm_v2_impl(const nbest_gemm_args* a, const nbest_gemm_args* b2, int64_t m_split, hipStream_t st) {
  NB_CHECK(a->N % 64 == 0, NBEST_ERR_SHAPE, "gemm(bf16): N=%lld must be a multiple of 64", (long long)a->N);
  NB_CHECK(a->trans_a || a->K % BK == 0, NBEST_ERR_SHAPE, "gemm(bf16): K=%lld must be a multiple of %d", (long long)a->K, BK);
  const Plan pl = make_plan(a);
  GemmP2 p;
  p.A = (const bf16*)a->A; p.B = (const bf16*)a->B; p.C = a->C; p.bias = a->bias; p.R = (const bf16*)a->R; p.U = (bf16*)a->U;
  p.M = a->M; p.N = a->N; p.K = a->K; p.lda = a->lda; p.ldb = a->ldb; p.ldc = a->ldc; p.ldr = a->ldr; p.ldu = a->ldu;
  p.tiles_m = (int)((a->M + pl.bm - 1) / pl.bm);
  p.tiles_n = (int)(a->N / pl.bn);
  p.splits = pl.splits;
  p.k_per_split = pl.kps;
  p.accumulate = a->accumulate;
  p.slab = (float*)a->ws;
  p.colpart = nullptr;
  p.A2 = p.B2 = nullptr; p.lda2 = p.ldb2 = p.m_split = 0; p.a2_bytes = p.b2_bytes = 0;
  p.Bp = nullptr; p.bp_bytes = 0; p.bp_bn = 0;
  if (a->B_packed && ((a->b_pack_bn == pl.bn && pl.bm == 256 && (pl.bn == 256 || pl.bn == 192)) || (pl.bm == 128 && pl.bn == 384 && a->b_pack_bn == 192) || (pl.bm == 128 && pl.bn == 512 && a->b_pack_bn == 256)) &&
      !a->trans_a && !a->trans_b &&
      a->epilogue != NBEST_EPI_F32_SPLITK && a->K % BK == 0 && a->N * a->K * 2 < ((int64_t)1 << 32) && ((uintptr_t)a->B_packed & 15) == 0) {
    p.Bp = (const bf16*)a->B_packed;
    p.bp_bytes = (uint32_t)(a->N * a->K * 2);
    p.bp_bn = a->b_pack_bn;
  }
  if (a->colsum_out && a->epilogue != NBEST_EPI_F32_SPLITK) {
    NB_CHECK(a->epilogue == NBEST_EPI_DGELU || a->trans_a || a->trans_b, NBEST_ERR_ARG,
             "gemm(bf16, generation 2): column sums are fused into the x GELU' epilogue only (nbest_gemm routes the others to generation 1)");
    NB_CHECK(a->ws && a->ws_bytes >= nbest_gemm_bf16_v2_ws_bytes(a), NBEST_ERR_WORKSPACE, "gemm: column-sum workspace too small");
    p.colpart = (float*)a->ws;
  }
  const int64_t a_rows = a->trans_a ? a->K : a->M, a_cols = a->trans_a ? (b2 ? m_split : a->M) : a->K;
  const int64_t b_rows = a->trans_b ? a->K : a->N, b_cols = a->trans_b ? a->N : a->K;
  const int64_t ab = ((a_rows - 1) * a->lda + a_cols) * 2, bb = ((b_rows - 1) * a->ldb + b_cols) * 2;
  p.a_bytes = (uint32_t)ab; p.b_bytes = (uint32_t)bb;
  if (b2) {
    const int64_t ab2 = ((a->K - 1) * b2->lda + b2->M) * 2, bb2 = ((a->K - 1) * b2->ldb + a->N) * 2;
    p.A2 = (const bf16*)b2->A; p.B2 = (const bf16*)b2->B; p.lda2 = b2->lda; p.ldb2 = b2->ldb; p.m_split = m_split;
    p.a2_bytes = (uint32_t)ab2; p.b2_bytes = (uint32_t)bb2;
    NB_CHECK(pl.bm == 256 && pl.bn == 256 && pl.splits > 1 && m_split % 256 == 0, NBEST_ERR_SHAPE, "wgrad pair: not a 256 x 256 split-K plan");
  }
  p.c_bytes = p.r_bytes = p.u_bytes = 0;
  if (a->epilogue != NBEST_EPI_F32_SPLITK) {
    const int64_t mpad = a->M + 256;
    NB_CHECK(mpad * a->ldc * 2 < ((int64_t)1 << 32) && mpad * a->ldr * 2 < ((int64_t)1 << 32) && mpad * a->ldu < ((int64_t)1 << 32),
             NBEST_ERR_SHAPE, "gemm(bf16): output / residual larger than 4 GiB");
    p.c_bytes = (uint32_t)(a->M * a->ldc * 2);
    p.r_bytes = a->R ? (uint32_t)(a->M * a->ldr * 2) : 0;
    p.u_bytes = a->U ? (uint32_t)(a->M * a->ldu) : 0;
  }
  p.drop = make_drop(a->drop_p, a->seed, a->drop_stream);
  p.stream_out = 1;
  p.gn = (!a->trans_a && !a->trans_b) ? nb_group_cols(a->N / pl.bn, (int64_t)pl.bn * a->K * 2, 2400) : (int)(a->N / pl.bn);
  if (pl.bm == 128 && pl.bn >= 384 && (a->N / pl.bn) % 2 == 0) p.gn = 2;
  const int epi = a->epilogue;
  if (epi == NBEST_EPI_F32_SPLITK && p.splits > 1)
    NB_CHECK(a->ws && a->ws_bytes >= (size_t)p.splits * a->M * a->N * sizeof(float), NBEST_ERR_WORKSPACE,
             "gemm: split-K workspace too small (%zu < %zu)", a->ws_bytes, (size_t)p.splits * a->M * a->N * sizeof(float));
  const int grid = p.tiles_m * p.tiles_n * p.splits;
  const int kepi = nb_kernel_epilogue(epi, a->U);
  int rc, wave_rows = 2;
  NB_CHECK(a->N % pl.bn == 0, NBEST_ERR_SHAPE, "gemm(bf16): N=%lld is not a multiple of the %d-column tile", (long long)a->N, pl.bn);
  if (pl.bm == 128 && pl.bn == 512) {
    rc = launch2<128, 512, 2, 4, 4, false, false>(p, kepi, grid, st);
  } else if (pl.bm == 128 && pl.bn == 384) {
    if (a->K >= 2048) rc = launch2<128, 384, 2, 4, 5, false, false>(p, kepi, grid, st);
    else rc = launch2<128, 384, 2, 4, 4, false, false>(p, kepi, grid, st);
  } else if (pl.bm == 256 && pl.bn == 192) {
    if (a->K >= 2048) rc = launch2<256, 192, 4, 2, 5, false, false>(p, kepi, grid, st);
    else rc = launch2<256, 192, 4, 2, 4, false, false>(p, kepi, grid, st);
    wave_rows = 4;
  } else if (pl.bm == 256 && pl.bn == 256) {
    if (!a->trans_a && !a->trans_b && epi != NBEST_EPI_F32_SPLITK) {
      if (a->K >= 2048) rc = launch2<256, 256, 4, 2, 5, false, false>(p, kepi, grid, st);
      else rc = launch2<256, 256, 4, 2, 4, false, false>(p, kepi, grid, st);
      wave_rows = 4;
    }
    else if (!a->trans_a && !a->trans_b) rc = launch2<256, 256, 2, 4, 4, false, false>(p, kepi, grid, st);
    else if (!a->trans_a && a->trans_b) rc = launch2<256, 256, 2, 4, 4, false, true>(p, kepi, grid, st);
    else rc = launch2<256, 256, 2, 4, 4, true, true>(p, kepi, grid, st);
  } else if (pl.bm == 256) {
    if (!a->trans_b && epi != NBEST_EPI_F32_SPLITK) { rc = launch2<256, 128, 4, 1, 3, false, false>(p, kepi, grid, st); wave_rows = 4; }
    else if (!a->trans_b) rc = launch2<256, 128, 2, 2, 3, false, false>(p, kepi, grid, st);
    else rc = launch2<256, 128, 2, 2, 3, false, true>(p, kepi, grid, st);
  } else {
    nbest_set_error("gemm(bf16, generation 2): no kernel for the %d x %d plan", pl.bm, pl.bn);
    return NBEST_ERR_SHAPE;
  }
  if (rc) return rc;
  if (p.colpart) return nbest_internal_partial_rows_sum(p.colpart, p.tiles_m * wave_rows, (int)a->N, a->colsum_out, a->colsum_accumulate, st);
  if (epi == NBEST_EPI_F32_SPLITK && p.splits > 1 && !(a->flags & NBEST_GEMM_DEFER_REDUCE))
    return nbest_internal_splitk_reduce(p.slab, (float*)a->C, a->M, a->N, a->ldc, p.splits, a->accumulate, b2 ? (float*)b2->C : nullptr,
                                        b2 ? m_split : a->M, b2 ? b2->ldc : 0, st);
  return NBEST_OK;
}

int nbest_gemm_bf16_v2(const nbest_gemm_args* a, hipStream_t st) { return gemm_v2_impl(a, nullptr, 0, st); }

static bool pair_virtual(const nbest_gemm_args* a, const nbest_gemm_args* b, nbest_gemm_args* v) {
  if (a->dtype != NBEST_BF16 || b->dtype != NBEST_BF16 || !a->trans_a || !a->trans_b || !b->trans_a || !b->trans_b) return false;
  if (a->epilogue != NBEST_EPI_F32_SPLITK || b->epilogue != NBEST_EPI_F32_SPLITK) return false;
  if (a->N != b->N || a->K != b->K || a->accumulate != b->accumulate || a->M % 256 || b->M % 256 || a->N % 256) return false;
  if ((a->flags | b->flags) & NBEST_GEMM_DEFER_REDUCE) return false;
  *v = *a;
// ... 56 lines not shown
```

### n-best-asr-transformer_amd/csrc/gemm_f32.hip

```cpp
#include "common.h"

namespace {

constexpr int TM = 64, TN = 64, TK = 16;

struct GemmF {
  const float* A; const float* B; float* C; const float* bias; const float* R; float* U;
  int64_t M, N, K, lda, ldb, ldc, ldr, ldu;
  int accumulate;
  DropCfg drop;
};

template <bool TA, bool TB, int EPI>
__global__ __launch_bounds__(256) void gemm_f32_kernel(GemmF p) {
  __shared__ float As[TK][TM + 4];
  __shared__ float Bs[TK][TN + 4];
  const int tid = threadIdx.x, tx = tid & 15, ty = tid >> 4;
  const int64_t m0 = (int64_t)blockIdx.y * TM, n0 = (int64_t)blockIdx.x * TN;
  float acc[4][4] = {};
  for (int64_t k0 = 0; k0 < p.K; k0 += TK) {
#pragma unroll
    for (int i = 0; i < 4; ++i) {
      const int idx = tid + 256 * i;
      int mm, kk;
      if (TA) { kk = idx >> 6; mm = idx & 63; } else { mm = idx >> 4; kk = idx & 15; }
      const int64_t m = m0 + mm, k = k0 + kk;
      float v = 0.f;
      if (m < p.M && k < p.K) v = TA ? p.A[k * p.lda + m] : p.A[m * p.lda + k];
      As[kk][mm] = v;
      int nn;
      if (TB) { kk = idx >> 6; nn = idx & 63; } else { nn = idx >> 4; kk = idx & 15; }
      const int64_t n = n0 + nn;
      const int64_t kb = k0 + kk;
      v = 0.f;
      if (n < p.N && kb < p.K) v = TB ? p.B[kb * p.ldb + n] : p.B[n * p.ldb + kb];
      Bs[kk][nn] = v;
    }
    __syncthreads();
#pragma unroll
    for (int kk = 0; kk < TK; ++kk) {
      float a[4], b[4];
#pragma unroll
      for (int i = 0; i < 4; ++i) a[i] = As[kk][ty * 4 + i];
#pragma unroll
      for (int j = 0; j < 4; ++j) b[j] = Bs[kk][tx * 4 + j];
#pragma unroll
      for (int i = 0; i < 4; ++i)
#pragma unroll
        for (int j = 0; j < 4; ++j) acc[i][j] = fmaf(a[i], b[j], acc[i][j]);
    }
    __syncthreads();
  }
#pragma unroll
  for (int i = 0; i < 4; ++i) {
    const int64_t m = m0 + ty * 4 + i;
    if (m >= p.M) continue;
#pragma unroll
    for (int j = 0; j < 4; ++j) {
      const int64_t n = n0 + tx * 4 + j;
      if (n >= p.N) continue;
      float v = acc[i][j];
      if (EPI == NBEST_EPI_F32_SPLITK) {
        float* c = p.C + m * p.ldc + n;
        *c = p.accumulate ? *c + v : v;
        continue;
      }
      if (EPI == NBEST_EPI_BIAS || EPI == NBEST_EPI_BIAS_GELU || EPI == kEpiBiasGeluNoU || EPI == NBEST_EPI_BIAS_DROP_RES) v += p.bias[n];
      if (EPI == NBEST_EPI_BIAS_GELU) { p.U[m * p.ldu + n] = dgelu_f(v); v = gelu_f(v); }
      if (EPI == kEpiBiasGeluNoU) v = gelu_f(v);
      if (EPI == NBEST_EPI_BIAS_DROP_RES) {
        if (p.drop.thr16) v = nb_keep(p.drop, (uint32_t)(m * p.N + n)) ? v * p.drop.scale : 0.f;
        v += p.R[m * p.ldr + n];
      }
      if (EPI == NBEST_EPI_RES) v += p.R[m * p.ldr + n];
      if (EPI == NBEST_EPI_DGELU) v *= p.U[m * p.ldu + n];
      p.C[m * p.ldc + n] = v;
    }
  }
}

template <bool TA, bool TB>
static int launch_epi(const GemmF& p, int epi, dim3 grid, hipStream_t st) {
#define L(E) case E: gemm_f32_kernel<TA, TB, E><<<grid, 256, 0, st>>>(p); break;
  switch (epi) {
    L(NBEST_EPI_NONE) L(NBEST_EPI_BIAS) L(NBEST_EPI_BIAS_GELU) L(NBEST_EPI_BIAS_DROP_RES) L(NBEST_EPI_DGELU)
    L(NBEST_EPI_RES) L(NBEST_EPI_F32_SPLITK) L(kEpiBiasGeluNoU)
    default:
      nbest_set_error("gemm: bad epilogue %d", epi);
      return NBEST_ERR_ARG;
  }
#undef L
  NB_LAUNCH_CHECK();
  return NBEST_OK;
}

}

int nbest_gemm_f32(const nbest_gemm_args* a, hipStream_t st) {
  GemmF p;
  p.A = (const float*)a->A; p.B = (const float*)a->B; p.C = (float*)a->C; p.bias = a->bias; p.R = (const float*)a->R;
  p.U = (float*)a->U;
  p.M = a->M; p.N = a->N; p.K = a->K; p.lda = a->lda; p.ldb = a->ldb; p.ldc = a->ldc; p.ldr = a->ldr; p.ldu = a->ldu;
  p.accumulate = a->accumulate;
  p.drop = make_drop(a->drop_p, a->seed, a->drop_stream);
  dim3 grid((unsigned)((a->N + TN - 1) / TN), (unsigned)((a->M + TM - 1) / TM));
  const int kepi = nb_kernel_epilogue(a->epilogue, a->U);
  if (!a->trans_a && !a->trans_b) return launch_epi<false, false>(p, kepi, grid, st);
  if (!a->trans_a && a->trans_b) return launch_epi<false, true>(p, kepi, grid, st);
  if (a->trans_a && a->trans_b) return launch_epi<true, true>(p, kepi, grid, st);
  return launch_epi<true, false>(p, kepi, grid, st);
}
```

### n-best-asr-transformer_amd/csrc/internal.h

```cpp
#pragma once
#include <hip/hip_runtime_api.h>
#include <stddef.h>
#include <stdint.h>

#include "../../include/nbest_hip.h"

struct Fp8Grad;

void nbest_set_error(const char* fmt, ...);

int nbest_internal_layernorm_fwd8(const void* x, const float* gamma, const float* beta, void* y, void* y8, float* stats,
                                  int64_t M, int H, float eps, int dtype, nbest_stream_t stream, const uint32_t* a_prev, uint32_t* a_new);
int nbest_internal_layernorm_bwd8(const void* dy, const void* x, const float* stats, const float* gamma, void* dx,
                                  void* dx_drop, float* dgamma, float* dbeta, float* dbias, int64_t M, int H, int dtype,
                                  int accumulate, float drop_p, uint64_t seed, uint32_t drop_stream, void* ws,
                                  size_t ws_bytes, nbest_stream_t stream, Fp8Grad f8);
int nbest_internal_partial_rows_sum(const float* part, int nrows, int N, float* out, int accumulate, hipStream_t st);
void nbest_internal_rowred_batch_begin();
void nbest_internal_rowred_batch_abort();
int nbest_internal_rowred_batch_flush(hipStream_t st);

int nbest_internal_attention_fwd8(const void* qkv, const uint8_t* key_mask, void* ctx, void* ctx8, float* lse, int B, int S, int heads,
                                  int d, int dtype, float drop_p, uint64_t seed, uint32_t drop_stream, nbest_stream_t stream,
                                  uint32_t* keep, const uint32_t* a_prev, uint32_t* a_new);
int nbest_internal_attention_bwd8(const void* qkv, const uint8_t* key_mask, const void* ctx, const void* dctx, const float* lse,
                                  void* dqkv, float* dbias, int accumulate, void* ws, size_t ws_bytes, int B, int S, int heads,
                                  int d, int dtype, float drop_p, uint64_t seed, uint32_t drop_stream, nbest_stream_t stream, Fp8Grad f8,
                                  const uint32_t* keep);
size_t nbest_internal_attention_keep_bytes(int B, int S, int heads);
int nbest_attention_cls_fwd_internal(const void* q, int64_t ldq, const void* kv, int64_t ldkv, const uint8_t* key_mask, void* ctx,
                                     int64_t ldctx, int B, int S, int heads, int d, int dtype, nbest_stream_t stream);
int nbest_internal_attention_cls_probs(const void* q, int64_t ldq, const void* kv, int64_t ldkv, const uint8_t* key_mask, float* probs,
                                       int64_t ldp, int B, int S, int heads, int d, int dtype, nbest_stream_t stream);

void nb_splitk_plan(int64_t tiles, int64_t K, int64_t slots, int64_t min_blocks, int* splits, int64_t* k_per_split);
int nbest_internal_splitk_reduce(const float* slab, float* C, int64_t M, int64_t N, int64_t ldc, int splits, int accumulate,
                                 float* C2, int64_t m_split, int64_t ldc2, hipStream_t st);

int nbest_gemm_f32(const nbest_gemm_args* a, hipStream_t st);
size_t nbest_gemm_bf16_ws_bytes(const nbest_gemm_args* a);
int nbest_gemm_bf16(const nbest_gemm_args* a, hipStream_t st);
size_t nbest_gemm_bf16_v2_ws_bytes(const nbest_gemm_args* a);
int nbest_gemm_bf16_v2(const nbest_gemm_args* a, hipStream_t st);
bool nbest_gemm_bf16_v2_wins(const nbest_gemm_args* a);
size_t nbest_wgrad_pair_bf16_ws_bytes(const nbest_gemm_args* a, const nbest_gemm_args* b);
int nbest_wgrad_pair_bf16(const nbest_gemm_args* a, const nbest_gemm_args* b, hipStream_t st);
int nbest_wgrad_group_bf16(const nbest_gemm_args* problems, int n, hipStream_t st);
int nbest_pack_bn_internal(int64_t N);
int nbest_pack_weights_bf16(const void* src, void* dst, const nbest_matrix_desc* descs, int n_matrices, int n_stages, hipStream_t st);

int nbest_internal_amax_bf16(const void* x, int64_t n, uint32_t* out, hipStream_t st);
int nbest_internal_cast_bf16_to_fp8(const void* src, void* dst, int64_t n, const uint32_t* a_prev, uint32_t* a_new, hipStream_t st);
```

### n-best-asr-transformer_amd/csrc/norm_embed.hip

```cpp
#include "common.h"

namespace {

constexpr int kMaxRowredBlocks = 512;
constexpr int kMaxLnBwdBlocks = 1024;
static inline int rowred_blocks(int64_t M) {
  int64_t b = (M + 31) / 32;
  if (b < 1) b = 1;
  if (b > kMaxRowredBlocks) b = kMaxRowredBlocks;
  return (int)b;
}

__device__ __forceinline__ float sum4(f32x4 v) { return (v[0] + v[1]) + (v[2] + v[3]); }

template <typename T, int VPL>
__global__ __launch_bounds__(256) void ln_fwd_kernel(const T* __restrict__ x, const float* __restrict__ gamma,
                                                     const float* __restrict__ beta, T* __restrict__ y,
                                                     float* __restrict__ stats, int64_t M, int H, float eps) {
  const int lane = threadIdx.x & 63, wpb = blockDim.x >> 6, nvec = H >> 2;
  const float invH = 1.0f / (float)H;
  for (int64_t row = (int64_t)blockIdx.x * wpb + (threadIdx.x >> 6); row < M; row += (int64_t)gridDim.x * wpb) {
    const T* xr = x + row * H;
    f32x4 v[VPL];
    float s = 0.f;
#pragma unroll
    for (int i = 0; i < VPL; ++i) {
      const int c = lane + 64 * i;
      if (c < nvec) { v[i] = Vec4<T>::load(xr + 4 * c); s += sum4(v[i]); } else v[i] = f32x4{0, 0, 0, 0};
    }
    const float mean = wave_sum(s) * invH;
    float q = 0.f;
#pragma unroll
    for (int i = 0; i < VPL; ++i) {
      const int c = lane + 64 * i;
      if (c < nvec) { f32x4 d = v[i] - mean; q += sum4(d * d); }
    }
    const float rstd = 1.0f / sqrtf(wave_sum(q) * invH + eps);
    T* yr = y + row * H;
#pragma unroll
    for (int i = 0; i < VPL; ++i) {
      const int c = lane + 64 * i;
      if (c < nvec) {
        f32x4 g = *(const f32x4*)(gamma + 4 * c), b = *(const f32x4*)(beta + 4 * c);
        Vec4<T>::store(yr + 4 * c, (v[i] - mean) * rstd * g + b);
      }
    }
    if (lane == 0) { stats[2 * row] = mean; stats[2 * row + 1] = rstd; }
  }
}

__device__ __forceinline__ f32x2 unpack2(uint32_t w) {
  return f32x2{__builtin_bit_cast(float, w << 16), __builtin_bit_cast(float, w & 0xFFFF0000u)};
}
__device__ __forceinline__ uint32_t pack2(f32x2 v) {
  bf16x2 o;
  o[0] = (bf16)v[0]; o[1] = (bf16)v[1];
  return __builtin_bit_cast(uint32_t, o);
}
template <int VPL>
__global__ __launch_bounds__(256) void ln_fwd_fast_kernel(const bf16* __restrict__ x, const float* __restrict__ gamma,
                                                          const float* __restrict__ beta, bf16* __restrict__ y,
                                                          float* __restrict__ stats, int64_t M, float eps,
                                                          uint8_t* __restrict__ y8,
                                                          const uint32_t* __restrict__ a_prev, uint32_t* __restrict__ a_new) {
  const float s8 = fp8_act_scale(a_prev);
  float amax8 = 0.f;
  constexpr int H = VPL * 256;
  constexpr float invH = 1.0f / (float)H;
  const int lane = threadIdx.x & 63;
  const int64_t stride = (int64_t)gridDim.x * 4;
  int64_t row = (int64_t)blockIdx.x * 4 + (threadIdx.x >> 6);
  if (row >= M) return;
  f32x2 gm[VPL][2], bt[VPL][2];
#pragma unroll
  for (int i = 0; i < VPL; ++i) {
    const f32x4 g4 = *(const f32x4*)(gamma + 4 * (lane + 64 * i)), b4 = *(const f32x4*)(beta + 4 * (lane + 64 * i));
    gm[i][0] = f32x2{g4[0], g4[1]}; gm[i][1] = f32x2{g4[2], g4[3]};
    bt[i][0] = f32x2{b4[0], b4[1]}; bt[i][1] = f32x2{b4[2], b4[3]};
  }
  uint2 nx[VPL];
#pragma unroll
  for (int i = 0; i < VPL; ++i) nx[i] = *(const uint2*)(x + row * H + 4 * (lane + 64 * i));
  for (; row < M; row += stride) {
    uint2 cx[VPL];
#pragma unroll
    for (int i = 0; i < VPL; ++i) cx[i] = nx[i];
    const int64_t nrow = (row + stride < M) ? row + stride : row;
#pragma unroll
    for (int i = 0; i < VPL; ++i) nx[i] = *(const uint2*)(x + nrow * H + 4 * (lane + 64 * i));
    f32x2 v[VPL][2];
    f32x2 ps = {0.f, 0.f};
#pragma unroll
    for (int i = 0; i < VPL; ++i) {
      v[i][0] = unpack2(cx[i].x); v[i][1] = unpack2(cx[i].y);
      ps += v[i][0]; ps += v[i][1];
    }
    const float mean = wave_sum_dpp(ps[0] + ps[1]) * invH;
    f32x2 pq = {0.f, 0.f};
#pragma unroll
    for (int i = 0; i < VPL; ++i) {
      v[i][0] = v[i][0] - mean; v[i][1] = v[i][1] - mean;
      pq += v[i][0] * v[i][0]; pq += v[i][1] * v[i][1];
    }
    const float rstd = 1.0f / sqrtf(wave_sum_dpp(pq[0] + pq[1]) * invH + eps);
#pragma unroll
    for (int i = 0; i < VPL; ++i) {
      const f32x2 o0 = v[i][0] * rstd * gm[i][0] + bt[i][0], o1 = v[i][1] * rstd * gm[i][1] + bt[i][1];
      const uint2 pk = uint2{pack2(o0), pack2(o1)};
      *(uint2*)(y + row * H + 4 * (lane + 64 * i)) = pk;
      if (y8) {
        const f32x2 r0 = unpack2(pk.x), r1 = unpack2(pk.y);
        if (a_new) amax8 = fmaxf(fmaxf(amax8, fmaxf(fabsf(r0[0]), fabsf(r0[1]))), fmaxf(fabsf(r1[0]), fabsf(r1[1])));
        const float q[4] = {r0[0] * s8, r0[1] * s8, r1[0] * s8, r1[1] * s8};
        *(uint32_t*)(y8 + row * H + 4 * (lane + 64 * i)) = fp8_pack4(q);
      }
    }
    if (lane == 0) *(f32x2*)(stats + 2 * row) = f32x2{mean, rstd};
  }
  if (y8 && a_new) {
    amax8 = wave_max(amax8);
    if (lane == 0) amax_update(a_new, amax8);
  }
}

template <typename T, int VPL, bool PARAMS = true>
__global__ __launch_bounds__(256) void ln_bwd_kernel(const T* __restrict__ dy, const T* __restrict__ x,
                                                     const float* __restrict__ stats, const float* __restrict__ gamma,
                                                     T* __restrict__ dx, T* __restrict__ dx_drop, float* __restrict__ part,
                                                     int64_t M, int H, int rows_per_block, int with_dbias, DropCfg drop) {
  extern __shared__ __attribute__((aligned(16))) float acc[];
  const int lane = threadIdx.x & 63, wave = threadIdx.x >> 6, wpb = blockDim.x >> 6, nvec = H >> 2;
  const float invH = 1.0f / (float)H;
  if constexpr (PARAMS) {
    for (int i = threadIdx.x; i < 3 * H; i += blockDim.x) acc[i] = 0.f;
    __syncthreads();
  }
  f32x4 ag[VPL], ab[VPL], ad[VPL], gm[VPL];
#pragma unroll
  for (int i = 0; i < VPL; ++i) {
    ag[i] = ab[i] = ad[i] = f32x4{0, 0, 0, 0};
    const int c = lane + 64 * i;
    gm[i] = (c < nvec) ? *(const f32x4*)(gamma + 4 * c) : f32x4{0, 0, 0, 0};
  }
  const int64_t r0 = (int64_t)blockIdx.x * rows_per_block;
  const int64_t r1 = (r0 + rows_per_block < M) ? r0 + rows_per_block : M;
  typename Vec4<T>::raw_t nx[VPL], nd[VPL];
  float nmean = 0.f, nrstd = 0.f;
  {
    const int64_t row = r0 + wave;
    if (row < r1) {
      nmean = stats[2 * row]; nrstd = stats[2 * row + 1];
#pragma unroll
      for (int i = 0; i < VPL; ++i) {
        const int c = lane + 64 * i;
        if (c < nvec) { nx[i] = Vec4<T>::raw_load(x + row * H + 4 * c); nd[i] = Vec4<T>::raw_load(dy + row * H + 4 * c); }
      }
    }
  }
  for (int64_t row = r0 + wave; row < r1; row += wpb) {
    const float mean = nmean, rstd = nrstd;
    typename Vec4<T>::raw_t cx[VPL], cd[VPL];
#pragma unroll
    for (int i = 0; i < VPL; ++i) { cx[i] = nx[i]; cd[i] = nd[i]; }
    const int64_t nrow = row + wpb;
    if (nrow < r1) {
      nmean = stats[2 * nrow]; nrstd = stats[2 * nrow + 1];
#pragma unroll
      for (int i = 0; i < VPL; ++i) {
        const int c = lane + 64 * i;
        if (c < nvec) { nx[i] = Vec4<T>::raw_load(x + nrow * H + 4 * c); nd[i] = Vec4<T>::raw_load(dy + nrow * H + 4 * c); }
      }
    }
    f32x4 xh[VPL], g[VPL], d[VPL];
    float s1 = 0.f, s2 = 0.f;
#pragma unroll
    for (int i = 0; i < VPL; ++i) {
      const int c = lane + 64 * i;
      if (c < nvec) {
        xh[i] = (Vec4<T>::cvt(cx[i]) - mean) * rstd;
        d[i] = Vec4<T>::cvt(cd[i]);
        g[i] = d[i] * gm[i];
        s1 += sum4(g[i]);
        s2 += sum4(g[i] * xh[i]);
      } else {
        xh[i] = g[i] = d[i] = f32x4{0, 0, 0, 0};
      }
    }
    s1 = wave_sum(s1) * invH;
    s2 = wave_sum(s2) * invH;
#pragma unroll
    for (int i = 0; i < VPL; ++i) {
      const int c = lane + 64 * i;
      if (c < nvec) {
        f32x4 o = (g[i] - s1 - xh[i] * s2) * rstd;
        Vec4<T>::store(dx + row * H + 4 * c, o);
        if constexpr (PARAMS) {
          ag[i] += d[i] * xh[i];
          ab[i] += d[i];
        }
        if (drop.thr16) {
          const uint32_t k = nb_keep4(drop, (uint32_t)(row * H + 4 * c));
#pragma unroll
          for (int e = 0; e < 4; ++e) o[e] = (k >> e & 1) ? o[e] * drop.scale : 0.f;
          Vec4<T>::store(dx_drop + row * H + 4 * c, o);
        }
        if constexpr (PARAMS) ad[i] += o;
      }
    }
  }
  if constexpr (!PARAMS) return;
  for (int w = 0; w < wpb; ++w) {
    if (wave == w) {
#pragma unroll
      for (int i = 0; i < VPL; ++i) {
        const int c = lane + 64 * i;
        if (c < nvec) {
          *(f32x4*)&acc[4 * c] += ag[i];
          *(f32x4*)&acc[H + 4 * c] += ab[i];
          if (with_dbias) *(f32x4*)&acc[2 * H + 4 * c] += ad[i];
        }
      }
    }
    __syncthreads();
  }
  const int nblk = gridDim.x;
  for (int i = threadIdx.x; i < H; i += blockDim.x) {
    part[((int64_t)0 * nblk + blockIdx.x) * H + i] = acc[i];
    part[((int64_t)1 * nblk + blockIdx.x) * H + i] = acc[H + i];
    if (with_dbias) part[((int64_t)2 * nblk + blockIdx.x) * H + i] = acc[2 * H + i];
  }
}

__device__ __forceinline__ f32x2 unpack_bf16x2(uint32_t w) { return unpack2(w); }
__device__ __forceinline__ uint32_t pack_bf16x2(f32x2 v) { return pack2(v); }

template <int VPL, bool DROP, bool DBIAS, int WAVES, bool PARAMS = true>
__global__ __launch_bounds__(WAVES * 64) void ln_bwd_fast_kernel(const bf16* __restrict__ dy, const bf16* __restrict__ x,
                                                          const float* __restrict__ stats, const float* __restrict__ gamma,
                                                          bf16* __restrict__ dx, bf16* __restrict__ dx_drop,
                                                          float* __restrict__ part, int64_t M, int rows_per_block, DropCfg drop,
                                                          Fp8Grad f8) {
  constexpr int H = VPL * 256;
  extern __shared__ __attribute__((aligned(16))) float acc[];
  const int lane = threadIdx.x & 63, wave = threadIdx.x >> 6;
  const float s8 = fp8_grad_scale(f8.amax_prev);
  float amax8 = 0.f;
  f32x2 gm[VPL][2], ag[VPL][2], ab[VPL][2], ad[VPL][2];
#pragma unroll
  for (int i = 0; i < VPL; ++i) {
    const f32x4 g4 = *(const f32x4*)(gamma + 4 * (lane + 64 * i));
    gm[i][0] = f32x2{g4[0], g4[1]}; gm[i][1] = f32x2{g4[2], g4[3]};
    ag[i][0] = ag[i][1] = ab[i][0] = ab[i][1] = ad[i][0] = ad[i][1] = f32x2{0.f, 0.f};
  }
  const int64_t stride = rows_per_block < 0 ? -(int64_t)rows_per_block : WAVES;
// ... 777 lines not shown
  }
}

static int finalize(const float* part, int nblk, int N, float* o0, int a0, float* o1, int a1, float* o2, int a2,
                    hipStream_t st) {
  RowredOut o;
  o.out[0] = o0; o.out[1] = o1; o.out[2] = o2;
  o.accumulate[0] = a0; o.accumulate[1] = a1; o.accumulate[2] = a2;
  const int nout = o2 ? 3 : (o1 ? 2 : 1);
  if (t_batch != nullptr && t_batch_n < kMaxBatch) {
    RowredJob& jb = t_batch->j[t_batch_n++];
    jb.part = part; jb.nblk = nblk; jb.N = N; jb.nout = nout; jb.o = o;
    return NBEST_OK;
  }
  rowred_finalize_kernel<<<dim3((N + 31) / 32, nout), dim3(32, 32), 0, st>>>(part, nblk, N, o);
  NB_LAUNCH_CHECK();
  return NBEST_OK;
}

}

static thread_local RowredJobs t_jobs_storage;
void nbest_internal_rowred_batch_begin() { t_batch = &t_jobs_storage; t_batch_n = 0; }
void nbest_internal_rowred_batch_abort() { t_batch = nullptr; t_batch_n = 0; }
int nbest_internal_rowred_batch_flush(hipStream_t st) {
  RowredJobs* b = t_batch;
  const int n = t_batch_n;
  t_batch = nullptr; t_batch_n = 0;
  if (b == nullptr || n == 0) return NBEST_OK;
  int maxN = 0, maxout = 1;
  for (int i = 0; i < n; ++i) { if (b->j[i].N > maxN) maxN = b->j[i].N; if (b->j[i].nout > maxout) maxout = b->j[i].nout; }
  rowred_finalize_multi_kernel<<<dim3((maxN + 31) / 32, maxout, n), dim3(32, 32), 0, st>>>(*b);
  NB_LAUNCH_CHECK();
  return NBEST_OK;
}

int nbest_internal_partial_rows_sum(const float* part, int nrows, int N, float* out, int accumulate, hipStream_t st) {
  return finalize(part, nrows, N, out, accumulate, nullptr, 0, nullptr, 0, st);
}

extern "C" size_t nbest_rowred_ws_bytes(int64_t M, int64_t N) {
  int64_t b = (M + 31) / 32;
  if (b < 1) b = 1;
  if (b > kMaxLnBwdBlocks) b = kMaxLnBwdBlocks;
  return (size_t)3 * b * N * sizeof(float);
}
constexpr int kEmbTpc = 16;
extern "C" size_t nbest_embed_bwd_ws_bytes(int64_t M, int64_t H) {
  const int64_t chunks = (M + kEmbTpc - 1) / kEmbTpc;
  return (size_t)5 * kMaxLnBwdBlocks * H * sizeof(float) + (size_t)kMaxLnBwdBlocks * (sizeof(int64_t) + 2 * sizeof(int)) +
         (size_t)chunks * 2 * H * sizeof(float) + (size_t)(chunks + 4) * sizeof(int);
}

int nbest_internal_layernorm_fwd8(const void* x, const float* gamma, const float* beta, void* y, void* y8, float* stats,
                                  int64_t M, int H, float eps, int dtype, nbest_stream_t stream, const uint32_t* a_prev, uint32_t* a_new) {
  if (int e = check_h(H)) return e;
  NB_CHECK(x && gamma && beta && y && stats && M > 0, NBEST_ERR_ARG, "layernorm_fwd: null pointer or M <= 0");
  NB_CHECK(!y8 || (dtype == NBEST_BF16 && H % 256 == 0 && H <= 1024), NBEST_ERR_SHAPE, "layernorm_fwd: fp8 copy needs bf16 and H in {256..1024}");
  hipStream_t st = (hipStream_t)stream;
  const int grid0 = grid_rows(M, 4);
  if (dtype == NBEST_F32) {
    DISPATCH_VPL(H, (ln_fwd_kernel<float, VPL><<<grid0, 256, 0, st>>>((const float*)x, gamma, beta, (float*)y, stats, M, H, eps)));
  } else if (dtype == NBEST_BF16 && H % 256 == 0 && H <= 1024) {
    const int grid = grid0 < 1024 ? grid0 : 1024;
    switch (H / 256) {
      case 1: ln_fwd_fast_kernel<1><<<grid, 256, 0, st>>>((const bf16*)x, gamma, beta, (bf16*)y, stats, M, eps, (uint8_t*)y8, a_prev, a_new); break;
      case 2: ln_fwd_fast_kernel<2><<<grid, 256, 0, st>>>((const bf16*)x, gamma, beta, (bf16*)y, stats, M, eps, (uint8_t*)y8, a_prev, a_new); break;
      case 3: ln_fwd_fast_kernel<3><<<grid, 256, 0, st>>>((const bf16*)x, gamma, beta, (bf16*)y, stats, M, eps, (uint8_t*)y8, a_prev, a_new); break;
      default: ln_fwd_fast_kernel<4><<<grid, 256, 0, st>>>((const bf16*)x, gamma, beta, (bf16*)y, stats, M, eps, (uint8_t*)y8, a_prev, a_new); break;
    }
  } else if (dtype == NBEST_BF16) {
    DISPATCH_VPL(H, (ln_fwd_kernel<bf16, VPL><<<grid0, 256, 0, st>>>((const bf16*)x, gamma, beta, (bf16*)y, stats, M, H, eps)));
  } else NB_CHECK(false, NBEST_ERR_DTYPE, "layernorm_fwd: bad dtype %d", dtype);
  NB_LAUNCH_CHECK();
  return NBEST_OK;
}

extern "C" int nbest_layernorm_fwd(const void* x, const float* gamma, const float* beta, void* y, float* stats,
                                   int64_t M, int H, float eps, int dtype, nbest_stream_t stream) {
  return nbest_internal_layernorm_fwd8(x, gamma, beta, y, nullptr, stats, M, H, eps, dtype, stream, nullptr, nullptr);
}

int nbest_internal_layernorm_bwd8(const void* dy, const void* x, const float* stats, const float* gamma, void* dx,
                                  void* dx_drop, float* dgamma, float* dbeta, float* dbias, int64_t M, int H, int dtype,
                                  int accumulate, float drop_p, uint64_t seed, uint32_t drop_stream, void* ws,
                                  size_t ws_bytes, nbest_stream_t stream, Fp8Grad f8) {
  if (int e = check_h(H)) return e;
  NB_CHECK(!f8.amax_new || (dtype == NBEST_BF16 && H % 256 == 0 && H <= 1024), NBEST_ERR_SHAPE, "layernorm_bwd: fp8 copy needs bf16 and H in {256..1024}");
  const bool params = dgamma || dbeta || dbias;
  NB_CHECK(dy && x && stats && gamma && dx && M > 0 && (!params || (dgamma && dbeta && ws)), NBEST_ERR_ARG, "layernorm_bwd: null pointer");
  NB_CHECK(!params || ws_bytes >= nbest_rowred_ws_bytes(M, H), NBEST_ERR_WORKSPACE, "layernorm_bwd: workspace too small");
  const DropCfg d = make_drop(drop_p, seed, drop_stream);
  NB_CHECK(d.thr16 == 0 || (dx_drop && dx_drop != dx) || (!dx_drop && f8.out8), NBEST_ERR_ARG, "layernorm_bwd: dropout needs a separate dx_drop buffer");
  NB_CHECK(M * (int64_t)H < (int64_t)1 << 32 || d.thr16 == 0, NBEST_ERR_SHAPE, "layernorm_bwd: dropout counter overflow");
  hipStream_t st = (hipStream_t)stream;
  int nblk = (int)((M + 31) / 32 < 1 ? 1 : ((M + 31) / 32 > kMaxLnBwdBlocks ? kMaxLnBwdBlocks : (M + 31) / 32));
  if (nblk > 512) nblk = 512;
  int rpb = (int)((M + nblk - 1) / nblk);
  nblk = (int)((M + rpb - 1) / rpb);
  constexpr int waves = 4;
  float* part = (float*)ws;
  const size_t smem = (size_t)3 * H * sizeof(float);
  const int wb = dbias ? 1 : 0;
  if (!params) {
    if (dtype == NBEST_F32) {
      DISPATCH_VPL(H, (ln_bwd_kernel<float, VPL, false><<<nblk, 256, 0, st>>>((const float*)dy, (const float*)x, stats, gamma,
                                                                               (float*)dx, (float*)dx_drop, nullptr, M, H, rpb, 0, d)));
    } else if (dtype == NBEST_BF16 && H % 256 == 0 && H <= 1024) {
#define NB_LNB0(V, D) ln_bwd_fast_kernel<V, D, false, waves, false><<<nblk, waves * 64, 0, st>>>((const bf16*)dy, (const bf16*)x, stats, gamma, \
                                                                                               (bf16*)dx, (bf16*)dx_drop, nullptr, M, rpb, d, f8)
#define NB_LNB0_V(V)                      \
  do {                                     \
    if (d.thr16) NB_LNB0(V, true);         \
    else NB_LNB0(V, false);                \
  } while (0)
      switch (H / 256) {
        case 1: NB_LNB0_V(1); break;
        case 2: NB_LNB0_V(2); break;
        case 3: NB_LNB0_V(3); break;
        default: NB_LNB0_V(4); break;
      }
#undef NB_LNB0_V
#undef NB_LNB0
    } else if (dtype == NBEST_BF16) {
      DISPATCH_VPL(H, (ln_bwd_kernel<bf16, VPL, false><<<nblk, 256, 0, st>>>((const bf16*)dy, (const bf16*)x, stats, gamma,
                                                                              (bf16*)dx, (bf16*)dx_drop, nullptr, M, H, rpb, 0, d)));
    } else NB_CHECK(false, NBEST_ERR_DTYPE, "layernorm_bwd: bad dtype %d", dtype);
    NB_LAUNCH_CHECK();
    return NBEST_OK;
  }
  if (dtype == NBEST_F32) {
    DISPATCH_VPL(H, (ln_bwd_kernel<float, VPL><<<nblk, 256, smem, st>>>((const float*)dy, (const float*)x, stats, gamma,
                                                                         (float*)dx, (float*)dx_drop, part, M, H, rpb, wb, d)));
  } else if (dtype == NBEST_BF16 && H % 256 == 0 && H <= 1024) {
#define NB_LNB(V, D, B)                                                                                                        \
  do {                                                                                                                         \
    if (waves == 8) {                                                                                                          \
      (void)hipFuncSetAttribute((const void*)ln_bwd_fast_kernel<V, D, B, 8>, hipFuncAttributeMaxDynamicSharedMemorySize, 8 * 3 * H * 4); \
      ln_bwd_fast_kernel<V, D, B, 8><<<nblk, 512, 8 * 3 * H * 4, st>>>((const bf16*)dy, (const bf16*)x, stats, gamma, (bf16*)dx,       \
                                                                       (bf16*)dx_drop, part, M, rpb, d, f8);                   \
    } else {                                                                                                                   \
      ln_bwd_fast_kernel<V, D, B, 4><<<nblk, 256, 4 * 3 * H * 4, st>>>((const bf16*)dy, (const bf16*)x, stats, gamma, (bf16*)dx,       \
                                                                       (bf16*)dx_drop, part, M, rpb, d, f8);                   \
    }                                                                                                                          \
  } while (0)
#define NB_LNB_V(V)                                                     \
  do {                                                                  \
    if (d.thr16) { if (wb) NB_LNB(V, true, true); else NB_LNB(V, true, false); } \
    else { if (wb) NB_LNB(V, false, true); else NB_LNB(V, false, false); }       \
  } while (0)
    switch (H / 256) {
      case 1: NB_LNB_V(1); break;
      case 2: NB_LNB_V(2); break;
      case 3: NB_LNB_V(3); break;
      default: NB_LNB_V(4); break;
    }
#undef NB_LNB_V
#undef NB_LNB
  } else if (dtype == NBEST_BF16) {
    DISPATCH_VPL(H, (ln_bwd_kernel<bf16, VPL><<<nblk, 256, smem, st>>>((const bf16*)dy, (const bf16*)x, stats, gamma,
                                                                        (bf16*)dx, (bf16*)dx_drop, part, M, H, rpb, wb, d)));
  } else NB_CHECK(false, NBEST_ERR_DTYPE, "layernorm_bwd: bad dtype %d", dtype);
  NB_LAUNCH_CHECK();
  return finalize(part, nblk, H, dgamma, accumulate, dbeta, accumulate, dbias, accumulate, st);
}

extern "C" int nbest_layernorm_bwd(const void* dy, const void* x, const float* stats, const float* gamma, void* dx,
                                   void* dx_drop, float* dgamma, float* dbeta, float* dbias, int64_t M, int H, int dtype,
                                   int accumulate, float drop_p, uint64_t seed, uint32_t drop_stream, void* ws,
                                   size_t ws_bytes, nbest_stream_t stream) {
  return nbest_internal_layernorm_bwd8(dy, x, stats, gamma, dx, dx_drop, dgamma, dbeta, dbias, M, H, dtype, accumulate, drop_p, seed,
                                       drop_stream, ws, ws_bytes, stream, Fp8Grad{nullptr, nullptr, nullptr});
}

extern "C" int nbest_colsum(const void* X, float* out, int64_t M, int64_t N, int64_t ld, int dtype, int accumulate,
                            void* ws, size_t ws_bytes, nbest_stream_t stream) {
  NB_CHECK(X && out && ws && M > 0 && N > 0 && N % 4 == 0 && ld % 4 == 0, NBEST_ERR_ARG, "colsum: bad arguments");
  NB_CHECK(ws_bytes >= nbest_rowred_ws_bytes(M, N), NBEST_ERR_WORKSPACE, "colsum: workspace too small");
  hipStream_t st = (hipStream_t)stream;
  const int nblk = rowred_blocks(M);
  const int rpb = (int)((M + nblk - 1) / nblk);
  float* part = (float*)ws;
  dim3 grid((unsigned)((N + 255) / 256), nblk);
  if (dtype == NBEST_F32) colsum_kernel<float><<<grid, 256, 0, st>>>((const float*)X, part, M, N, ld, rpb);
  else if (dtype == NBEST_BF16) colsum_kernel<bf16><<<grid, 256, 0, st>>>((const bf16*)X, part, M, N, ld, rpb);
  else NB_CHECK(false, NBEST_ERR_DTYPE, "colsum: bad dtype %d", dtype);
  NB_LAUNCH_CHECK();
  return finalize(part, nblk, (int)N, out, accumulate, nullptr, 0, nullptr, 0, st);
}

extern "C" int nbest_embed_ln_fwd(const int64_t* ids, const int64_t* seg, const int64_t* pos, const void* word,
                                  const void* type, const void* ptab, const float* gamma, const float* beta, void* out,
                                  float* stats, int64_t M, int H, float eps, int dtype, float drop_p, uint64_t seed,
                                  uint32_t drop_stream, nbest_stream_t stream) {
  if (int e = check_h(H)) return e;
  NB_CHECK(ids && pos && word && type && ptab && gamma && beta && out && stats && M > 0, NBEST_ERR_ARG, "embed_ln_fwd: null pointer");
  NB_CHECK(M * (int64_t)H < (int64_t)1 << 32, NBEST_ERR_SHAPE, "embed_ln_fwd: M*H must fit 32 bits (dropout counter)");
  hipStream_t st = (hipStream_t)stream;
  const DropCfg d = make_drop(drop_p, seed, drop_stream);
  const int grid = grid_rows(M, 4);
  if (dtype == NBEST_F32) {
    DISPATCH_VPL(H, (embed_fwd_kernel<float, VPL><<<grid, 256, 0, st>>>(ids, seg, pos, (const float*)word, (const float*)type,
                                                                        (const float*)ptab, gamma, beta, (float*)out, stats, M, H, eps, d)));
  } else if (dtype == NBEST_BF16) {
    DISPATCH_VPL(H, (embed_fwd_kernel<bf16, VPL><<<grid, 256, 0, st>>>(ids, seg, pos, (const bf16*)word, (const bf16*)type,
                                                                       (const bf16*)ptab, gamma, beta, (bf16*)out, stats, M, H, eps, d)));
  } else NB_CHECK(false, NBEST_ERR_DTYPE, "embed_ln_fwd: bad dtype %d", dtype);
  NB_LAUNCH_CHECK();
  return NBEST_OK;
}

extern "C" int nbest_embed_ln_fwd_interp(const int64_t* ids, const int64_t* base_ids, const float* alpha, const int64_t* seg,
                                         const int64_t* pos, const void* word, const void* type, const void* ptab, const float* gamma,
                                         const float* beta, void* out, float* stats, int B, int S, int H, float eps, int dtype,
                                         float drop_p, uint64_t seed, uint32_t drop_stream, nbest_stream_t stream) {
  if (int e = check_h(H)) return e;
  NB_CHECK(ids && base_ids && alpha && pos && word && type && ptab && gamma && beta && out && stats && B > 0 && S > 0, NBEST_ERR_ARG,
// ... 149 lines not shown
```

### n-best-asr-transformer_amd/hipabi.py

```python
import ctypes as C
import os

import torch

_HERE = os.path.dirname(os.path.abspath(__file__))
LIB_PATH = os.environ.get("NBEST_LIB") or os.path.join(_HERE, "csrc", "libnbest_hip.so")

F32, BF16 = 0, 1
ADAM_L2, ADAMW = 0, 1
EPI_NONE, EPI_BIAS, EPI_BIAS_GELU, EPI_BIAS_DROP_RES, EPI_DGELU, EPI_RES, EPI_F32_SPLITK = range(7)

EXPORTS = [
    "nbest_version", "nbest_last_error", "nbest_embed_ln_fwd", "nbest_embed_ln_bwd", "nbest_embed_bwd_ws_bytes", "nbest_rows_gather", "nbest_rows_zero", "nbest_rows_add",
    "nbest_gemm_ws_bytes", "nbest_gemm", "nbest_wgrad_pair_ws_bytes", "nbest_wgrad_pair", "nbest_wgrad_group", "nbest_pack_bn", "nbest_pack_weights", "nbest_pack_bn_fp8", "nbest_pack_weights_fp8", "nbest_attention_fwd", "nbest_attention_bwd", "nbest_attention_bwd_ws_bytes", "nbest_attention_keep_bytes", "nbest_attention_fwd_keep", "nbest_attention_bwd_keep", "nbest_layernorm_fwd",
    "nbest_layernorm_bwd", "nbest_rowred_ws_bytes", "nbest_colsum", "nbest_heads_ws_bytes", "nbest_stc_heads",
    "nbest_stc_heads_vjp", "nbest_cls_mse", "nbest_cls_grad_scatter", "nbest_stc_decode", "nbest_stream_stamp", "nbest_fp8_amax_fold", "nbest_bertadam_chunk", "nbest_bertadam_step", "nbest_bertadam_norms", "nbest_bertadam_update",
    "nbest_adam_clip_coef", "nbest_adam_update", "nbest_adam_step",
    "nbest_cast_f32_to_bf16", "nbest_transpose_weights", "nbest_encoder_act_bytes", "nbest_encoder_ws_bytes", "nbest_encoder_wgrad_launches_per_layer", "nbest_encoder_forward",
    "nbest_encoder_backward", "nbest_gemm_fp8", "nbest_gemm_fp8_ws_bytes", "nbest_wgrad_fp8", "nbest_wgrad_fp8_ws_bytes", "nbest_wgrad_fp8_pair", "nbest_wgrad_fp8_pair_ws_bytes", "nbest_cast_bf16_to_fp8", "nbest_quantize_weights_fp8",
    "nbest_attention_cls_fwd", "nbest_encoder_infer_ws_bytes", "nbest_encoder_infer",
    "nbest_attention_probs", "nbest_attention_cls_probs", "nbest_encoder_act_view", "nbest_encoder_infer_attn",
    "nbest_embed_ln_fwd_interp", "nbest_embed_attrib",
]


class GemmArgs(C.Structure):
    _fields_ = [("A", C.c_void_p), ("B", C.c_void_p), ("C", C.c_void_p), ("bias", C.c_void_p), ("R", C.c_void_p),
                ("U", C.c_void_p), ("ws", C.c_void_p), ("ws_bytes", C.c_size_t),
                ("M", C.c_int64), ("N", C.c_int64), ("K", C.c_int64),
                ("lda", C.c_int64), ("ldb", C.c_int64), ("ldc", C.c_int64), ("ldr", C.c_int64), ("ldu", C.c_int64),
                ("trans_a", C.c_int32), ("trans_b", C.c_int32), ("epilogue", C.c_int32), ("dtype", C.c_int32),
                ("accumulate", C.c_int32), ("drop_p", C.c_float), ("drop_stream", C.c_uint32), ("seed", C.c_uint64),
                ("colsum_out", C.c_void_p), ("colsum_accumulate", C.c_int32), ("flags", C.c_int32),
                ("B_packed", C.c_void_p), ("b_pack_bn", C.c_int32), ("pad_", C.c_int32)]


class GemmFp8Args(C.Structure):
    _fields_ = [("A", C.c_void_p), ("B", C.c_void_p), ("C", C.c_void_p), ("bias", C.c_void_p), ("R", C.c_void_p), ("U", C.c_void_p),
                ("C8", C.c_void_p), ("M", C.c_int64), ("N", C.c_int64), ("K", C.c_int64),
                ("lda", C.c_int64), ("ldb", C.c_int64), ("ldc", C.c_int64), ("ldr", C.c_int64), ("ldu", C.c_int64), ("ldc8", C.c_int64),
                ("epilogue", C.c_int32), ("out_scale", C.c_float), ("drop_p", C.c_float), ("drop_stream", C.c_uint32), ("seed", C.c_uint64),
                ("out_scale_dev", C.c_void_p), ("a_amax", C.c_void_p), ("c8_amax_prev", C.c_void_p), ("c8_amax_new", C.c_void_p),
                ("colsum_out", C.c_void_p), ("colsum_accumulate", C.c_int32), ("pad", C.c_int32), ("ws", C.c_void_p), ("ws_bytes", C.c_size_t),
                ("B_packed", C.c_void_p), ("b_pack_bn", C.c_int32), ("pad3", C.c_int32)]


class LabelSpaceC(C.Structure):
    _fields_ = [("n_top", C.c_int32), ("n_bottom", C.c_int32), ("n_rows", C.c_int32),
                ("bottom_off", C.c_void_p), ("bottom_ids", C.c_void_p), ("head_row", C.c_void_p)]


class TensorDesc(C.Structure):
    _fields_ = [("offset", C.c_int64), ("numel", C.c_int64), ("lr", C.c_float), ("wd", C.c_float),
                ("active", C.c_int32), ("block_start", C.c_int32)]


class MatrixDesc(C.Structure):
    _fields_ = [("offset", C.c_int64), ("rows", C.c_int32), ("cols", C.c_int32), ("tile_start", C.c_int32), ("pad", C.c_int32)]


class LayerOffsets(C.Structure):
    _fields_ = [(n, C.c_int64) for n in ("wqkv", "bqkv", "wo", "bo", "ln1_g", "ln1_b", "w1", "b1", "w2", "b2", "ln2_g", "ln2_b")]


class EncoderDesc(C.Structure):
    _fields_ = [("dtype", C.c_int32), ("B", C.c_int32), ("S", C.c_int32), ("H", C.c_int32), ("L", C.c_int32),
                ("heads", C.c_int32), ("F", C.c_int32), ("vocab", C.c_int32), ("max_pos", C.c_int32), ("n_types", C.c_int32),
                ("ln_eps", C.c_float), ("hidden_drop", C.c_float), ("attn_drop", C.c_float),
                ("word_pad_id", C.c_int64), ("pos_pad_id", C.c_int64),
                ("off_word", C.c_int64), ("off_pos", C.c_int64), ("off_type", C.c_int64),
                ("off_emb_ln_g", C.c_int64), ("off_emb_ln_b", C.c_int64),
                ("layers_host", C.POINTER(LayerOffsets)), ("seed", C.c_uint64), ("drop_stream_base", C.c_uint32),
                ("wgrad_events_n", C.c_int32), ("wgrad_events", C.POINTER(C.c_void_p)),
                ("w8", C.c_void_p), ("w8_inv_scale", C.c_void_p), ("w8t", C.c_void_p), ("gamax_prev", C.c_void_p),
                ("gamax_new", C.c_void_p), ("fp8_bwd", C.c_int32), ("pad2", C.c_int32),
                ("wpk", C.c_void_p), ("wpkt", C.c_void_p), ("w8p", C.c_void_p), ("w8tp", C.c_void_p),
                ("word_perm", C.c_void_p), ("aamax_prev", C.c_void_p), ("aamax_new", C.c_void_p), ("fp8_act", C.c_int32), ("pad4", C.c_int32),
                ("first_trainable", C.c_int32), ("no_input_grad", C.c_int32), ("wgrad_skip_host", C.c_void_p),
                ("base_ids", C.c_void_p), ("alpha", C.c_void_p), ("no_param_grad", C.c_int32), ("pad5", C.c_int32)]
    wgrad_group = property(lambda self: self.pad5, lambda self, v: setattr(self, "pad5", int(v)))


_lib = None


def lib():
    global _lib
    if _lib is None:
        if not os.path.exists(LIB_PATH):
            raise RuntimeError("nbest_amd: %s is missing - build it with `make -C %s` (hipcc, gfx950). "
                               "There is no CPU fallback for the product path." % (LIB_PATH, os.path.dirname(LIB_PATH)))
        L = C.CDLL(LIB_PATH)
        for name in EXPORTS:
            if not hasattr(L, name):
                raise RuntimeError("nbest_amd: %s does not export %s" % (LIB_PATH, name))
        for name in ("nbest_embed_bwd_ws_bytes", "nbest_gemm_ws_bytes", "nbest_wgrad_pair_ws_bytes", "nbest_rowred_ws_bytes", "nbest_heads_ws_bytes",
                     "nbest_attention_bwd_ws_bytes", "nbest_attention_keep_bytes",
                     "nbest_encoder_act_bytes", "nbest_encoder_ws_bytes", "nbest_encoder_infer_ws_bytes"):
            getattr(L, name).restype = C.c_size_t
        L.nbest_embed_bwd_ws_bytes.argtypes = [C.c_int64, C.c_int64]
        L.nbest_rows_gather.argtypes = [C.c_void_p, C.c_void_p, C.c_int64, C.c_int64, C.c_void_p, C.c_void_p, C.c_int, C.c_void_p]
        L.nbest_rows_zero.argtypes = [C.c_void_p, C.c_void_p, C.c_int64, C.c_int, C.c_void_p]
        L.nbest_rows_add.argtypes = [C.c_void_p, C.c_void_p, C.c_void_p, C.c_int64, C.c_int, C.c_void_p]
        L.nbest_rowred_ws_bytes.argtypes = [C.c_int64, C.c_int64]
        L.nbest_heads_ws_bytes.argtypes = [C.c_int, C.c_int, C.c_int]
        L.nbest_gemm_ws_bytes.argtypes = [C.POINTER(GemmArgs)]
        L.nbest_gemm.argtypes = [C.POINTER(GemmArgs), C.c_void_p]
        L.nbest_wgrad_pair_ws_bytes.argtypes = [C.POINTER(GemmArgs), C.POINTER(GemmArgs)]
        L.nbest_wgrad_pair.argtypes = [C.POINTER(GemmArgs), C.POINTER(GemmArgs), C.c_void_p]
        L.nbest_wgrad_group.argtypes = [C.POINTER(GemmArgs), C.c_int32, C.c_void_p]
        L.nbest_encoder_act_bytes.argtypes = [C.POINTER(EncoderDesc)]
        L.nbest_encoder_ws_bytes.argtypes = [C.POINTER(EncoderDesc)]
        L.nbest_encoder_wgrad_launches_per_layer.argtypes = [C.POINTER(EncoderDesc)]
        vp, i64, i32, f32, u64, u32, sz = C.c_void_p, C.c_int64, C.c_int, C.c_float, C.c_uint64, C.c_uint32, C.c_size_t
        L.nbest_embed_ln_fwd.argtypes = [vp] * 10 + [i64, i32, f32, i32, f32, u64, u32, vp]
        L.nbest_embed_ln_bwd.argtypes = [vp] * 15 + [i32, i32, i32, i32, i32, i64, i64, i32, i32, f32, u64, u32, vp, sz, vp]
        L.nbest_embed_ln_fwd_interp.argtypes = [vp] * 12 + [i32, i32, i32, f32, i32, f32, u64, u32, vp]
        L.nbest_embed_attrib.argtypes = [vp] * 11 + [i32, i32, i32, i32, f32, i32, vp]
        L.nbest_attention_fwd.argtypes = [vp] * 4 + [i32] * 5 + [f32, u64, u32, vp]
        L.nbest_attention_bwd.argtypes = [vp] * 7 + [i32, vp, sz] + [i32] * 5 + [f32, u64, u32, vp]
        L.nbest_attention_bwd_ws_bytes.argtypes = [i32, i32, i32]
        L.nbest_attention_keep_bytes.argtypes = [i32, i32, i32]
        L.nbest_attention_fwd_keep.argtypes = [vp] * 4 + [i32] * 5 + [f32, u64, u32, vp, vp]
        L.nbest_attention_bwd_keep.argtypes = [vp] * 7 + [i32, vp, sz] + [i32] * 5 + [f32, u64, u32, vp, vp]
        L.nbest_layernorm_fwd.argtypes = [vp] * 5 + [i64, i32, f32, i32, vp]
        L.nbest_layernorm_bwd.argtypes = [vp] * 9 + [i64, i32, i32, i32, f32, u64, u32, vp, sz, vp]
        L.nbest_colsum.argtypes = [vp, vp, i64, i64, i64, i32, i32, vp, sz, vp]
        L.nbest_stc_heads.argtypes = [vp, i64, vp, vp, C.POINTER(LabelSpaceC)] + [vp] * 8 + [i32] * 5 + [f32, u64, u32, vp, sz, vp]
        L.nbest_stc_heads_vjp.argtypes = [vp, C.POINTER(LabelSpaceC)] + [vp] * 8 + [i32, i32, i32, f32, u64, u32, vp, sz, vp]
        L.nbest_cls_mse.argtypes = [vp, i64, vp, i64, vp, vp, vp, i32, i32, i32, f32, vp]
# ... 67 lines not shown


def _ws(nbytes, device):
    return torch.empty(max(int(nbytes), 16), dtype=torch.uint8, device=device)


def gemm_prepared(A, B, M, N, K, out, trans_a=False, trans_b=False, epilogue=EPI_NONE, defer_reduce=False):
    g = GemmArgs()
    g.A, g.B, g.C = A.data_ptr(), B.data_ptr(), out.data_ptr()
    g.M, g.N, g.K = M, N, K
    g.lda, g.ldb, g.ldc = A.stride(0), B.stride(0), out.stride(0)
    g.trans_a, g.trans_b, g.epilogue, g.dtype = int(trans_a), int(trans_b), epilogue, dtype_code(A.dtype)
    g.flags = 1 if defer_reduce else 0
    ws = _ws(lib().nbest_gemm_ws_bytes(C.byref(g)), A.device)
    g.ws, g.ws_bytes = ws.data_ptr(), ws.numel()
    fn, ref, st = lib().nbest_gemm, C.byref(g), stream_ptr()

    def launch():
        rc = fn(ref, st)
        if rc:
            check(rc, "gemm")
    launch.keepalive = (g, ws, A, B, out)
    return launch


def pack_weight(W):
    N, K = W.shape
    bn = lib().nbest_pack_bn(N)
    if bn == 0 or K % 32 or N % bn:
        return None, 0
    d = (MatrixDesc * 1)()
    d[0].offset, d[0].rows, d[0].cols, d[0].tile_start, d[0].pad = 0, N, K, 0, bn
    dd = torch.frombuffer(bytearray(bytes(d)), dtype=torch.uint8).to(W.device)
    out = torch.empty_like(W)
    check(lib().nbest_pack_weights(ptr(W), ptr(out), ptr(dd), 1, (N // bn) * (K // 32), stream_ptr()), "pack_weights")
    return out, bn


def pack_weight_fp8(W8):
    N, K = W8.shape
    bn = lib().nbest_pack_bn_fp8(N, K)
    if bn == 0 or K % 64 or N % bn:
        return None, 0
    d = (MatrixDesc * 1)()
    d[0].offset, d[0].rows, d[0].cols, d[0].tile_start, d[0].pad = 0, N, K, 0, bn
    dd = torch.frombuffer(bytearray(bytes(d)), dtype=torch.uint8).to(W8.device)
    out = torch.empty_like(W8)
    check(lib().nbest_pack_weights_fp8(ptr(W8), ptr(out), ptr(dd), 1, (N // bn) * (K // 64), stream_ptr()), "pack_weights_fp8")
    return out, bn


def gemm(A, B, M, N, K, trans_a=False, trans_b=False, epilogue=EPI_NONE, bias=None, R=None, U=None, out=None,
         accumulate=False, drop_p=0.0, seed=0, drop_stream=0, colsum_out=None, defer_reduce=False, B_packed=None, b_pack_bn=0,
         want_u=True):
    dt = dtype_code(A.dtype)
    dev = A.device
    if out is None:
        out = torch.empty(M, N, dtype=torch.float32 if epilogue == EPI_F32_SPLITK else A.dtype, device=dev)
    if epilogue == EPI_BIAS_GELU and U is None and want_u:
        U = torch.empty(M, N, dtype=torch.float32 if A.dtype == torch.float32 else torch.uint8, device=dev)
    g = GemmArgs()
    g.A, g.B, g.C = A.data_ptr(), B.data_ptr(), out.data_ptr()
    g.bias = bias.data_ptr() if bias is not None else None
    g.R = R.data_ptr() if R is not None else None
    g.U = U.data_ptr() if U is not None else None
    g.M, g.N, g.K = M, N, K
    g.lda, g.ldb, g.ldc = A.stride(0), B.stride(0), out.stride(0)
    g.ldr = R.stride(0) if R is not None else 0
    g.ldu = U.stride(0) if U is not None else 0
    g.trans_a, g.trans_b, g.epilogue, g.dtype = int(trans_a), int(trans_b), epilogue, dt
    g.accumulate, g.drop_p, g.drop_stream, g.seed = int(accumulate), drop_p, drop_stream, seed
    g.colsum_out = colsum_out.data_ptr() if colsum_out is not None else None
    g.flags = 1 if defer_reduce else 0
    if B_packed is not None:
        g.B_packed, g.b_pack_bn = B_packed.data_ptr(), b_pack_bn
    nb = lib().nbest_gemm_ws_bytes(C.byref(g))
    ws = _ws(nb, dev)
    g.ws, g.ws_bytes = ws.data_ptr(), ws.numel()
    check(lib().nbest_gemm(C.byref(g), stream_ptr()), "gemm")
    return (out, U) if epilogue == EPI_BIAS_GELU and want_u else out


def wgrad_pair(dY1, X1, dY2, X2, out1=None, out2=None, accumulate=False):
    K, N = X1.shape
    outs, gs = [], []
    for dY, X, out in ((dY1, X1, out1), (dY2, X2, out2)):
        M = dY.shape[1]
        if out is None:
            out = torch.empty(M, N, dtype=torch.float32, device=X.device)
        g = GemmArgs()
        g.A, g.B, g.C = dY.data_ptr(), X.data_ptr(), out.data_ptr()
        g.M, g.N, g.K = M, N, K
        g.lda, g.ldb, g.ldc = dY.stride(0), X.stride(0), out.stride(0)
        g.trans_a = g.trans_b = 1
        g.epilogue, g.dtype, g.accumulate = EPI_F32_SPLITK, dtype_code(X.dtype), int(accumulate)
        outs.append(out)
        gs.append(g)
    nb = lib().nbest_wgrad_pair_ws_bytes(C.byref(gs[0]), C.byref(gs[1]))
    ws = _ws(nb, X1.device)
    gs[0].ws, gs[0].ws_bytes = ws.data_ptr(), ws.numel()
    check(lib().nbest_wgrad_pair(C.byref(gs[0]), C.byref(gs[1]), stream_ptr()), "wgrad_pair")
    return outs


WGRAD_GROUP_PLAN, WGRAD_GROUP_NEVER, WGRAD_GROUP_ALWAYS = 0, 1, 2


def wgrad_group(problems, outs=None, accumulate=False):
    n = len(problems)
    gs = (GemmArgs * max(n, 1))()
    res = []
    for i, (dY, X) in enumerate(problems):
        M, N = dY.shape[1], X.shape[1]
        out = outs[i] if outs is not None else torch.empty(M, N, dtype=torch.float32, device=X.device)
        g = gs[i]
        g.A, g.B, g.C = dY.data_ptr(), X.data_ptr(), out.data_ptr()
        g.M, g.N, g.K = M, N, X.shape[0]
        g.lda, g.ldb, g.ldc = dY.stride(0), X.stride(0), out.stride(0)
        g.trans_a = g.trans_b = 1
        g.epilogue, g.dtype, g.accumulate = EPI_F32_SPLITK, dtype_code(X.dtype), int(accumulate)
        res.append(out)
    check(lib().nbest_wgrad_group(gs, n, stream_ptr()), "wgrad_group")
    return res


def rows_gather(table, rows, cap):
# ... 330 lines not shown
```

### n-best-asr-transformer_amd/model.py

```python
import collections
import ctypes as C
import os

import torch
import torch.nn as nn

from . import hipabi as hb
from .arena import ParamArena
from .config import EncoderConfig, LabelSpace, NAMED


def position_ids_for(cfg, input_ids):
    B, S = input_ids.shape
    if cfg.family in ("roberta", "xlm-roberta"):
        nonpad = input_ids.ne(cfg.pad_token_id).long()
        return (torch.cumsum(nonpad, dim=1) * nonpad + cfg.pad_token_id).contiguous()
    return torch.arange(S, dtype=torch.long, device=input_ids.device).unsqueeze(0).expand(B, S).contiguous()


class _Holder(nn.Module):
    """module tree node that only carries arena-backed parameters under HF names"""


def _attach(root, dotted, param):
# ... 7 lines not shown


class FreezePlan(collections.namedtuple("FreezePlan", "key trainable first_trainable no_input_grad with_embeddings skip")):
    __slots__ = ()

    @property
    def skip_ptr(self):
        return None if self.skip is None else C.cast(self.skip, C.c_void_p)


def freeze_plan(model):
    flags = tuple(p.requires_grad and "pooler" not in n for n, p in model._params)
    plan = model._plans.get(flags)
    if plan is not None:
        return plan
    trainable = frozenset(n for (n, _), f in zip(model._params, flags) if f)
    L = model.cfg.num_hidden_layers
    emb = any(n.startswith("bert_encoder.embeddings.") for n in trainable)
    layer = [any(n.startswith("bert_encoder.encoder.layer.%d." % l) for n in trainable) for l in range(L)]
    first = 0 if emb else next((l for l in range(L) if layer[l]), L)
    pre = "bert_encoder.encoder.layer.%d."
    mats = (["attention.self.%s.weight" % q for q in ("query", "key", "value")], ["attention.output.dense.weight"],
            ["intermediate.dense.weight"], ["output.dense.weight"])
    skip = [int(not any((pre % l) + m in trainable for m in ms)) for l in range(L) for ms in mats]
    plan = FreezePlan(flags, trainable, first, int(not emb), emb, (C.c_uint8 * len(skip))(*skip) if any(skip) else None)
    if len(model._plans) >= 64:
        model._plans.clear()
    model._plans[flags] = plan
    return plan


class _Pass:

    def __init__(self, model, B, S, slot, first_trainable=0):
        a, cfg = model.arena, model.cfg
        train = isinstance(slot, int)
        d = hb.EncoderDesc()
        d.dtype = hb.dtype_code(model.compute_dtype)
        d.B, d.S, d.H, d.L, d.heads, d.F = B, S, cfg.hidden_size, cfg.num_hidden_layers, cfg.num_attention_heads, cfg.intermediate_size
        d.vocab, d.max_pos, d.n_types = cfg.vocab_size, cfg.max_position_embeddings, cfg.type_vocab_size
        d.ln_eps = cfg.layer_norm_eps
        d.word_pad_id = cfg.pad_token_id
        d.pos_pad_id = cfg.pad_token_id if cfg.family in ("roberta", "xlm-roberta") else -1
        pre = "bert_encoder.embeddings."
        d.off_word = a.by_name[pre + "word_embeddings.weight"].offset
        d.off_pos = a.by_name[pre + "position_embeddings.weight"].offset
        d.off_type = a.by_name[pre + "token_type_embeddings.weight"].offset
        d.off_emb_ln_g = a.by_name[pre + "LayerNorm.weight"].offset
        d.off_emb_ln_b = a.by_name[pre + "LayerNorm.bias"].offset
        d.layers_host = C.cast(a.layer_offsets, C.POINTER(hb.LayerOffsets))
        d.drop_stream_base = 1000 * slot if train else 0
        d.first_trainable = first_trainable
        d.wgrad_group = model.wgrad_group
        if model.fp8_forward and train:
            d.w8, d.w8_inv_scale = a.w8.data_ptr(), a.w8_inv_scale.data_ptr()
        self.desc = d
        self.act_bytes = hb.lib().nbest_encoder_act_bytes(C.byref(d))
        self.B, self.S = B, S


class _PassRecord(collections.namedtuple("_PassRecord", "ps slot inputs perm hidden gen plan")):
    __slots__ = ()

    @property
    def cls(self):
        return self.hidden.view(self.ps.B, self.ps.S, -1)[:, 0, :]


class _STCBridge(torch.autograd.Function):

    @staticmethod
    def forward(ctx, anchor, model, input_ids, trans_input_ids, seg_ids, trans_seg_ids, feats_from_transcript):
        ctx.set_materialize_grads(False)
        from_t = bool(feats_from_transcript and trans_input_ids is not None)
        ws = hb.heads_ws(input_ids.shape[0], model.dls.n_rows, model.cfg.hidden_size, model.device)
        plan = model._training_plan()
        ra, rt, (top, bott, fin, _, _, _, _) = model._passes_and_heads(input_ids, seg_ids, trans_input_ids, trans_seg_ids, True,
                                                                       from_transcript=from_t, ws=ws, plan=plan)
        ctx.model, ctx.ra, ctx.rt, ctx.ws, ctx.seed, ctx.from_t = model, ra, rt, ws, model._step_seed(), from_t
        ctx.save_for_backward(top, bott)
        trans_cls = rt.cls.float() if rt is not None else torch.zeros(0, device=model.device)
        return top, bott, fin, ra.cls.float(), trans_cls

    @staticmethod
    def backward(ctx, dtop, dbott, dfin, dasr, dtrans):
        m = ctx.model
        m._check_stash(ctx.ra, ctx.rt)
        _require_trainable(ctx.ra.plan)
        top, bott = ctx.saved_tensors
        B, H = top.shape[0], m.cfg.hidden_size
        z = lambda g, like: torch.zeros_like(like) if g is None else g.contiguous().float()
        fin_like = torch.empty(B, m.labels.n_bottom, dtype=torch.float32, device=m.device)
        dWh, dbh = m.arena.heads_grad_wb()
        dcls = hb.stc_heads_vjp(m.arena.heads_wb()[0], m.dls, top, bott, z(dtop, top), z(dbott, bott), z(dfin, fin_like), B, H, dWh, dbh, ctx.ws,
                                accumulate=True, drop_p=m.dropout, seed=ctx.seed, drop_stream=900)
        d_asr = dasr.contiguous().float() if dasr is not None else None
        d_tr = dtrans.contiguous().float() if (dtrans is not None and ctx.rt is not None) else None
        if ctx.from_t:
            d_tr = dcls if d_tr is None else d_tr + dcls
        else:
            d_asr = dcls if d_asr is None else d_asr + dcls
        if d_tr is not None and ctx.rt is not None:
            m._backward_pass(ctx.rt, d_tr, accumulate=True)
        if d_asr is not None:
            m._backward_pass(ctx.ra, d_asr, accumulate=True)
        m._end_of_step(True)
        return (None,) * 7


def _require_trainable(plan):
    if plan is not None and not plan.trainable:
        raise RuntimeError("nbest_amd: no parameter requires grad: a backward has nothing to compute (every tensor of the model "
                           "has requires_grad=False)")


class NBestSTCModel(nn.Module):
    def __init__(self, cfg: EncoderConfig, labels: LabelSpace, device="cuda", compute_dtype=torch.bfloat16, dropout=0.0,
                 seed=999, fp8_forward=False, fp8_backward=None, wgrad_group=hb.WGRAD_GROUP_PLAN):
        super().__init__()
        self.cfg, self.labels, self.compute_dtype = cfg, labels, compute_dtype
        self.dropout = float(dropout)
        self.device = torch.device(device)
        self.wgrad_group = int(wgrad_group)
        self.arena = ParamArena(cfg, labels, self.device, compute_dtype)
        self.fp8_forward = bool(fp8_forward)
        self.fp8_backward = self.fp8_forward if fp8_backward is None else bool(fp8_backward)
        self._gamax_valid = False
        self._aamax_valid = False
        if self.fp8_forward:
            if compute_dtype != torch.bfloat16:
                raise RuntimeError("nbest_amd: fp8_forward rides on the bf16 path")
            self.arena.enable_fp8_forward()
        elif self.fp8_backward:
            raise RuntimeError("nbest_amd: fp8_backward needs fp8_forward (it shares the e4m3 weight copy)")
        self.bert_encoder = _Holder()
        self.clf = _Holder()
        for s in self.arena.slots:
            p = nn.Parameter(self.arena.view(self.arena.p, s.name), requires_grad="pooler" not in s.name)
            if p.requires_grad:
                p.grad = self.arena.view(self.arena.g, s.name)
            root, rest = s.name.split(".", 1)
            _attach(getattr(self, root), rest, p)
        self._params = [(s.name, self.get_parameter(s.name)) for s in self.arena.slots]
        self._plans = {}
        self._plan_key = None
        self.dls = hb.DeviceLabelSpace(labels, self.device)
        self.seed = int(seed)
        self.step_counter = 0
        self._passes = {}
        self._stash = {}
        self._stash_gen = collections.Counter()
        self._ws = None
        self._dh = None
        self._infer_ws = None
        self._anchor = None

    def zero_grad(self, set_to_none=False):
        self.arena.g.zero_()

    def _drop_fp8_history(self):
        if self.fp8_backward and self._gamax_valid:
            self._gamax_valid = False
            self.arena.gamax.zero_()
            self.arena.gamax_slots.zero_()
        if self.fp8_forward and self._aamax_valid:
            self._aamax_valid = False
            self.arena.aamax.zero_()
            self.arena.aamax_slots.zero_()

    def load_reference_state(self, sd, strict=True):
        self._drop_fp8_history()
        return self.arena.load_state(sd, strict)

    def save_model(self, path):
        torch.save({k: v.detach().cpu() for k, v in self.state_dict().items()}, path)

# ... 434 lines not shown
```

Measured before the change: 12840.

## Compute only CLS rows after attention in the last encoder layer

In the last encoder layer, after attention, only the CLS token row of each sequence goes through the output projection, LayerNorms and FFN. The backward pass does the same using strided GEMMs and row-strided LayerNorm, which cuts the last-layer post-attention FLOPs by a factor of S. Dropout indexing gets a row-pitch parameter so the masks match the full-token layout. The cost is new strided code paths, zero-fill memsets for the non-CLS gradient rows, and a hidden output that is only valid at CLS positions. The path is on by default but disabled when fp8 weights are used.

Result: faster. 13230, median of 6 (+3.1%).

```diff
diff --git a/include/nbest_hip.h b/include/nbest_hip.h
--- a/include/nbest_hip.h
+++ b/include/nbest_hip.h
@@ -76,6 +76,8 @@
   const void* B_packed;
   int32_t b_pack_bn;
   int32_t pad_;
+  int32_t drop_row_stride;
+  int32_t pad2_;
 } nbest_gemm_args;
 #define NBEST_GEMM_DEFER_REDUCE 1
 size_t nbest_gemm_ws_bytes(const nbest_gemm_args* a);
@@ -257,7 +259,7 @@
   const uint32_t* aamax_prev;
   uint32_t* aamax_new;
   int32_t fp8_act;
-  int32_t pad4;
+  int32_t cls_last_layer;
   int32_t first_trainable;
   int32_t no_input_grad;
   const uint8_t* wgrad_skip_host;
diff --git a/n-best-asr-transformer_amd/csrc/common.h b/n-best-asr-transformer_amd/csrc/common.h
--- a/n-best-asr-transformer_amd/csrc/common.h
+++ b/n-best-asr-transformer_amd/csrc/common.h
@@ -312,6 +312,7 @@
   return ((h0 & 0xFFFFu) >= d.thr16 ? 1u : 0u) | ((h0 >> 16) >= d.thr16 ? 2u : 0u) |
          ((h1 & 0xFFFFu) >= d.thr16 ? 4u : 0u) | ((h1 >> 16) >= d.thr16 ? 8u : 0u);
 }
+static inline int64_t nb_drop_pitch(const nbest_gemm_args* a) { return a->N * (a->drop_row_stride > 1 ? a->drop_row_stride : 1); }
 static inline DropCfg make_drop(float p, uint64_t seed, uint32_t stream) {
   DropCfg d;
   uint32_t thr = (p <= 0.f) ? 0u : (uint32_t)lrintf(p * 65536.0f);
diff --git a/n-best-asr-transformer_amd/csrc/encoder.hip b/n-best-asr-transformer_amd/csrc/encoder.hip
--- a/n-best-asr-transformer_amd/csrc/encoder.hip
+++ b/n-best-asr-transformer_amd/csrc/encoder.hip
@@ -34,6 +34,10 @@
 };
 
 static int first_trainable(const nbest_encoder_desc* d) { return d->first_trainable < 0 ? 0 : (d->first_trainable > d->L ? d->L : d->first_trainable); }
+
+static bool cls_last_layer(const nbest_encoder_desc* d) {
+  return d->cls_last_layer && (d->dtype == NBEST_BF16 || d->dtype == NBEST_F32) && !d->w8 && d->L - 1 >= first_trainable(d);
+}
 
 static ActLayout act_layout(const nbest_encoder_desc* d, const Sizes& z) {
   ActLayout a;
@@ -213,6 +217,7 @@
   const void* R; float drop_p; uint32_t drop_stream;
   void* U; float* colsum;
   uint8_t* C8; int c_idx;
+  int64_t lda, ldr, ldc; int drop_rows;
 };
 
 static int layer_gemm(const GemmPass& c, const GemmOp& o) {
@@ -235,8 +240,10 @@
   nbest_gemm_args g = gemm_nt(c.dtype, o.A, c.W.W(o.w_off), o.C, c.M, o.N, o.K);
   if (c.b_kn) { g.trans_b = 1; g.ldb = o.N; }
   g.epilogue = o.epilogue; g.bias = o.bias;
-  if (o.R) { g.R = o.R; g.ldr = o.N; }
-  if (o.epilogue == NBEST_EPI_BIAS_DROP_RES) { g.drop_p = o.drop_p; g.drop_stream = o.drop_stream; g.seed = c.seed; }
+  if (o.R) { g.R = o.R; g.ldr = o.ldr ? o.ldr : o.N; }
+  if (o.lda) g.lda = o.lda;
+  if (o.ldc) g.ldc = o.ldc;
+  if (o.epilogue == NBEST_EPI_BIAS_DROP_RES) { g.drop_p = o.drop_p; g.drop_stream = o.drop_stream; g.seed = c.seed; g.drop_row_stride = o.drop_rows; }
   if (o.epilogue == NBEST_EPI_BIAS_GELU || o.epilogue == NBEST_EPI_DGELU) { g.U = o.U; g.ldu = o.N; }
   if (o.epilogue == NBEST_EPI_DGELU) {
     g.colsum_out = o.colsum; g.colsum_accumulate = g.accumulate = c.accumulate; g.ws = c.colsum_ws; g.ws_bytes = c.colsum_ws_bytes;
@@ -297,6 +304,30 @@
   const GemmPass g = {d->dtype, z.M, stream, d->seed, Ptrs{(const char*)wts, prm, z.esz}, d->wpk, false, fp8_forward_active(d),
                       d->w8, d->w8p, d->w8_inv_scale, d->aamax_prev, d->aamax_new, nullptr, 0, 0};
   return Fwd{d, g, key_mask, d->w8 && d->aamax_new && d->dtype == NBEST_BF16};
+}
+
+static int layer_forward_cls_tail(const Fwd& c, int l, const void* xin, void* xout, const LayerBufs& b) {
+  const nbest_encoder_desc* d = c.d;
+  const nbest_layer_offsets& o = d->layers_host[l];
+  GemmPass g = c.g;
+  g.M = d->B; g.packed = nullptr;
+  const Ptrs& P = g.W;
+  const int64_t B = d->B, SH = (int64_t)d->S * d->H;
+  const int H = d->H, F = d->F, dt = d->dtype, t = 4 * l;
+  const uint32_t s0 = d->drop_stream_base + 1 + 4 * l;
+  GemmOp wo = {b.ctx, nullptr, t + 1, o.wo, t + 1, b.r1, H, H, NBEST_EPI_BIAS_DROP_RES, P.P(o.bo)};
+  wo.lda = SH; wo.R = xin; wo.ldr = SH; wo.drop_p = d->hidden_drop; wo.drop_stream = s0 + 1; wo.drop_rows = d->S;
+  RUN(layer_gemm(g, wo));
+  RUN(nbest_internal_layernorm_fwd8(b.r1, P.P(o.ln1_g), P.P(o.ln1_b), b.x1, nullptr, b.st1, B, H, d->ln_eps, dt, g.stream, nullptr, nullptr));
+  GemmOp w1 = {b.x1, nullptr, t + 2, o.w1, t + 2, b.hact, F, H, NBEST_EPI_BIAS_GELU, P.P(o.b1)};
+  w1.U = b.u;
+  RUN(layer_gemm(g, w1));
+  GemmOp w2 = {b.hact, nullptr, t + 3, o.w2, t + 3, b.r2, H, F, NBEST_EPI_BIAS_DROP_RES, P.P(o.b2)};
+  w2.R = b.x1; w2.drop_p = d->hidden_drop; w2.drop_stream = s0 + 2; w2.drop_rows = d->S;
+  RUN(layer_gemm(g, w2));
+  LnRows rows = {};
+  rows.y_ld = SH;
+  return nbest_internal_layernorm_fwd_rows(b.r2, P.P(o.ln2_g), P.P(o.ln2_b), xout, b.st2, B, H, d->ln_eps, dt, g.stream, rows);
 }
 
 static int layer_forward(const Fwd& c, int l, const void* xin, void* xout, const LayerBufs& b, uint8_t* x8_next, float* cls_probs) {
@@ -318,6 +349,7 @@
   RUN(nbest_internal_attention_fwd8(b.qkv, c.key_mask, b.ctx, b.ctx8, b.lse, d->B, d->S, d->heads, 64, dt, d->attn_drop, d->seed, s0 + 0,
                                     stream, b.keep, c.AP(t + 1), c.AN(t + 1)));
   RUN(c.calib(b.ctx, M * H, t + 1));
+  if (l == d->L - 1 && cls_last_layer(d)) return layer_forward_cls_tail(c, l, xin, xout, b);
   GemmOp wo = {b.ctx, b.ctx8, t + 1, o.wo, t + 1, b.r1, H, H, NBEST_EPI_BIAS_DROP_RES, P.P(o.bo)};
   wo.R = xin; wo.drop_p = d->hidden_drop; wo.drop_stream = s0 + 1;
   RUN(layer_gemm(c.g, wo));
@@ -399,6 +431,7 @@
   const uint8_t *dY8, *X8;
   int64_t w_off, rows, cols;
   int g_idx, a_idx;
+  int64_t tokens, lda, ldb;
 };
 }
 
@@ -462,8 +495,10 @@
   const GemmPass dg = {dt, M, stream, 0, Ptrs{(const char*)(wt ? wts_t : wts), prm, z.esz}, wt ? d->wpkt : nullptr, !wt, f8b,
                        d->w8t, d->w8tp, d->w8_inv_scale, d->gamax_prev, d->gamax_new, red1, w.red_bytes, accumulate};
   auto wgrad_args_of = [&](const WGrad* x) {
-    nbest_gemm_args g = wgrad_args(dt, x->rows, x->cols, M);
+    nbest_gemm_args g = wgrad_args(dt, x->rows, x->cols, x->tokens ? x->tokens : M);
     g.A = x->dY; g.B = x->X; g.C = G(x->w_off); g.accumulate = accumulate;
+    if (x->lda) g.lda = x->lda;
+    if (x->ldb) g.ldb = x->ldb;
     return g;
   };
   auto wgrad_launch = [&](int l, const WGrad* wg, int j, int j2) -> int {
@@ -492,6 +527,13 @@
     stamp(1);
     return NBEST_OK;
   };
+  auto wgrad_cls = [&](int l, const WGrad* wg, int j) -> int {
+    const bool stamped = !grouped && !(j == 1 && paired);
+    if (stamped) stamp(0);
+    RUN(wgrad_launch(l, wg, j, -1));
+    if (stamped) stamp(1);
+    return NBEST_OK;
+  };
   nbest_gemm_args pend[8];
   int n_pend = 0;
 
@@ -509,27 +551,61 @@
       dRd2 = W + w.gset[gpos][0]; dBigL = W + w.gset[gpos][1]; dRd1 = W + w.gset[gpos][2]; dqkvL = W + w.gset[gpos][3];
       if (!hdrop) { dR2 = dRd2; dR1 = dRd1; }
     }
-    const WGrad wg[4] = {{dqkvL, X(l), dqkv8, b.x8, o.wqkv, 3 * H, H, t + 3, t + 0},
-                         {dRd1, b.ctx, dRd8, b.ctx8, o.wo, H, H, t + 2, t + 1},
-                         {dBigL, b.x1, dBig8, b.x18, o.w1, F, H, t + 1, t + 2},
-                         {dRd2, b.hact, dRd8, b.h8, o.w2, H, F, t + 0, t + 3}};
+    WGrad wg[4] = {{dqkvL, X(l), dqkv8, b.x8, o.wqkv, 3 * H, H, t + 3, t + 0},
+                   {dRd1, b.ctx, dRd8, b.ctx8, o.wo, H, H, t + 2, t + 1},
+                   {dBigL, b.x1, dBig8, b.x18, o.w1, F, H, t + 1, t + 2},
+                   {dRd2, b.hact, dRd8, b.h8, o.w2, H, F, t + 0, t + 3}};
+    const bool cls = l == d->L - 1 && cls_last_layer(d);
+    const int64_t Bc = d->B, SH = (int64_t)d->S * H;
+    if (cls) {
+      wg[1].tokens = wg[2].tokens = wg[3].tokens = Bc;
+      wg[1].lda = hdrop ? H : SH; wg[1].ldb = SH;
+    }
     if (!npg) nbest_internal_rowred_batch_begin();
-    RUN(nbest_internal_layernorm_bwd8(dA, b.r2, b.st2, P.P(o.ln2_g), dR2, (hdrop && !f8b) ? dRd2 : nullptr, GP(o.ln2_g), GP(o.ln2_b), GP(o.b2), M, H,
-                                      dt, accumulate, d->hidden_drop, d->seed, s0 + 2, red, w.red_bytes, stream, fg(dRd8, t + 0)));
-    GemmOp dw2 = {dRd2, dRd8, t + 0, o.w2, t + 3, f8b ? nullptr : dBigL, F, H, NBEST_EPI_DGELU};
-    dw2.U = b.u; dw2.colsum = GP(o.b1); dw2.C8 = dBig8; dw2.c_idx = t + 1;
-    RUN(layer_gemm(dg, dw2));
-    if (rec && !f8b) RUN(nbest_internal_amax_bf16(dBigL, M * F, GN(t + 1), st));
-    if (!grouped) RUN(wgrad(l, wg, 3, -1));
-    GemmOp dw1 = {dBigL, dBig8, t + 1, o.w1, t + 2, dB1, H, F, NBEST_EPI_RES};
-    dw1.R = dR2;
-    RUN(layer_gemm(dg, dw1));
-    if (!grouped) RUN(wgrad(l, wg, 2, -1));
-    RUN(nbest_internal_layernorm_bwd8(dB1, b.r1, b.st1, P.P(o.ln1_g), dR1, (hdrop && !f8b) ? dRd1 : nullptr, GP(o.ln1_g), GP(o.ln1_b), GP(o.bo), M, H,
-                                      dt, accumulate, d->hidden_drop, d->seed, s0 + 1, red2, w.red_bytes, stream, fg(dRd8, t + 2)));
-    const GemmOp dwo = {dRd1, dRd8, t + 2, o.wo, t + 1, dctx, H, H, NBEST_EPI_NONE};
-    RUN(layer_gemm(dg, dwo));
-    if (!paired && !grouped) RUN(wgrad(l, wg, 1, -1));
+    if (cls) {
+      NB_CHECK(!f8b, NBEST_ERR_ARG, "encoder_backward: the CLS-mode layer has no fp8 backward");
+      GemmPass dgc = dg;
+      dgc.M = Bc; dgc.packed = nullptr;
+      LnRows rows2 = {}, rows1 = {};
+      rows2.dy_ld = SH; rows2.drop_row_stride = d->S;
+      RUN(nbest_internal_layernorm_bwd_rows(dA, b.r2, b.st2, P.P(o.ln2_g), dR2, hdrop ? dRd2 : nullptr, GP(o.ln2_g), GP(o.ln2_b), GP(o.b2), Bc, H, dt,
+                                            accumulate, d->hidden_drop, d->seed, s0 + 2, red, w.red_bytes, stream, rows2));
+      GemmOp dw2 = {dRd2, nullptr, t + 0, o.w2, t + 3, dBigL, F, H, NBEST_EPI_DGELU};
+      dw2.U = b.u; dw2.colsum = GP(o.b1);
+      RUN(layer_gemm(dgc, dw2));
+      RUN(wgrad_cls(l, wg, 3));
+      GemmOp dw1 = {dBigL, nullptr, t + 1, o.w1, t + 2, dB1, H, F, NBEST_EPI_RES};
+      dw1.R = dR2;
+      RUN(layer_gemm(dgc, dw1));
+      RUN(wgrad_cls(l, wg, 2));
+      hipError_t e = hipMemsetAsync(dR1, 0, (size_t)M * H * z.esz, st);
+      if (e == hipSuccess) e = hipMemsetAsync(dctx, 0, (size_t)M * H * z.esz, st);
+      NB_CHECK(e == hipSuccess, NBEST_ERR_LAUNCH, "encoder_backward: memset failed: %s", hipGetErrorString(e));
+      rows1.dx_ld = SH; rows1.drop_row_stride = d->S;
+      RUN(nbest_internal_layernorm_bwd_rows(dB1, b.r1, b.st1, P.P(o.ln1_g), dR1, hdrop ? dRd1 : nullptr, GP(o.ln1_g), GP(o.ln1_b), GP(o.bo), Bc, H, dt,
+                                            accumulate, d->hidden_drop, d->seed, s0 + 1, red2, w.red_bytes, stream, rows1));
+      GemmOp dwo = {dRd1, nullptr, t + 2, o.wo, t + 1, dctx, H, H, NBEST_EPI_NONE};
+      dwo.lda = hdrop ? H : SH; dwo.ldc = SH;
+      RUN(layer_gemm(dgc, dwo));
+      RUN(wgrad_cls(l, wg, 1));
+    } else {
+      RUN(nbest_internal_layernorm_bwd8(dA, b.r2, b.st2, P.P(o.ln2_g), dR2, (hdrop && !f8b) ? dRd2 : nullptr, GP(o.ln2_g), GP(o.ln2_b), GP(o.b2), M, H,
+                                        dt, accumulate, d->hidden_drop, d->seed, s0 + 2, red, w.red_bytes, stream, fg(dRd8, t + 0)));
+      GemmOp dw2 = {dRd2, dRd8, t + 0, o.w2, t + 3, f8b ? nullptr : dBigL, F, H, NBEST_EPI_DGELU};
+      dw2.U = b.u; dw2.colsum = GP(o.b1); dw2.C8 = dBig8; dw2.c_idx = t + 1;
+      RUN(layer_gemm(dg, dw2));
+      if (rec && !f8b) RUN(nbest_internal_amax_bf16(dBigL, M * F, GN(t + 1), st));
+      if (!grouped) RUN(wgrad(l, wg, 3, -1));
+      GemmOp dw1 = {dBigL, dBig8, t + 1, o.w1, t + 2, dB1, H, F, NBEST_EPI_RES};
+      dw1.R = dR2;
+      RUN(layer_gemm(dg, dw1));
+      if (!grouped) RUN(wgrad(l, wg, 2, -1));
+      RUN(nbest_internal_layernorm_bwd8(dB1, b.r1, b.st1, P.P(o.ln1_g), dR1, (hdrop && !f8b) ? dRd1 : nullptr, GP(o.ln1_g), GP(o.ln1_b), GP(o.bo), M, H,
+                                        dt, accumulate, d->hidden_drop, d->seed, s0 + 1, red2, w.red_bytes, stream, fg(dRd8, t + 2)));
+      const GemmOp dwo = {dRd1, dRd8, t + 2, o.wo, t + 1, dctx, H, H, NBEST_EPI_NONE};
+      RUN(layer_gemm(dg, dwo));
+      if (!paired && !grouped) RUN(wgrad(l, wg, 1, -1));
+    }
     RUN(nbest_internal_attention_bwd8(b.qkv, key_mask, b.ctx, dctx, b.lse, f8b ? nullptr : dqkvL, GP(o.bqkv), accumulate, red3, w.red_bytes, d->B, d->S,
                                       d->heads, 64, dt, d->attn_drop, d->seed, s0 + 0, stream, fg(dqkv8, t + 3), b.keep));
     if (input_grad) {
@@ -538,17 +614,19 @@
       RUN(layer_gemm(dg, dwqkv));
     }
     if (!grouped) {
-      RUN(wgrad(l, wg, 0, paired ? 1 : -1));
+      RUN(wgrad(l, wg, 0, (paired && !cls) ? 1 : -1));
     } else if (group_ends && gpos + 1 < gl && d->wgrad_group != NBEST_WGRAD_GROUP_ALWAYS) {
       stamp(0);
-      RUN(wgrad_launch(l, wg, 3, -1));
-      RUN(wgrad_launch(l, wg, 2, -1));
-      if (!paired) RUN(wgrad_launch(l, wg, 1, -1));
-      RUN(wgrad_launch(l, wg, 0, paired ? 1 : -1));
+      if (!cls) {
+        RUN(wgrad_launch(l, wg, 3, -1));
+        RUN(wgrad_launch(l, wg, 2, -1));
+        if (!paired) RUN(wgrad_launch(l, wg, 1, -1));
+      }
+      RUN(wgrad_launch(l, wg, 0, (paired && !cls) ? 1 : -1));
       stamp(1);
     } else {
       for (int j = 0; j < 4; ++j)
-        if (!skip(l, j)) pend[n_pend++] = wgrad_args_of(wg + j);
+        if (!skip(l, j) && !(cls && j > 0)) pend[n_pend++] = wgrad_args_of(wg + j);
       if (group_ends) {
         stamp(0);
         if (n_pend) RUN(nbest_wgrad_group(pend, n_pend, stream));
diff --git a/n-best-asr-transformer_amd/csrc/gemm.hip b/n-best-asr-transformer_amd/csrc/gemm.hip
--- a/n-best-asr-transformer_amd/csrc/gemm.hip
+++ b/n-best-asr-transformer_amd/csrc/gemm.hip
@@ -36,8 +36,9 @@
   const int64_t b_rows = a->trans_b ? a->K : a->N, b_cols = a->trans_b ? a->N : a->K;
   const int64_t ab = ((a_rows - 1) * a->lda + a_cols) * 2, bb = ((b_rows - 1) * a->ldb + b_cols) * 2;
   NB_CHECK(ab < ((int64_t)1 << 32) && bb < ((int64_t)1 << 32), NBEST_ERR_SHAPE, "gemm(bf16): operand larger than 4 GiB");
-  NB_CHECK(a->M * a->N < ((int64_t)1 << 32) || make_drop(a->drop_p, a->seed, a->drop_stream).thr16 == 0, NBEST_ERR_SHAPE,
-           "gemm(bf16): dropout counter overflow");
+  NB_CHECK(a->drop_row_stride >= 0, NBEST_ERR_ARG, "gemm(bf16): negative drop_row_stride");
+  NB_CHECK((a->M - 1) * nb_drop_pitch(a) + a->N < ((int64_t)1 << 32) || make_drop(a->drop_p, a->seed, a->drop_stream).thr16 == 0,
+           NBEST_ERR_SHAPE, "gemm(bf16): dropout counter overflow");
   return check_epilogue_operands(a, 8, 16);
 }
 
diff --git a/n-best-asr-transformer_amd/csrc/gemm_bf16.hip b/n-best-asr-transformer_amd/csrc/gemm_bf16.hip
--- a/n-best-asr-transformer_amd/csrc/gemm_bf16.hip
+++ b/n-best-asr-transformer_amd/csrc/gemm_bf16.hip
@@ -11,6 +11,7 @@
   const bf16* A; const bf16* B; void* C; const float* bias; const bf16* R; bf16* U; float* slab; float* colpart;
   int64_t M, N, K, lda, ldb, ldc, ldr, ldu;
   int64_t k_per_split;
+  int64_t dN;
   int tiles_m, tiles_n, splits, accumulate;
   uint32_t a_bytes, b_bytes;
   DropCfg drop;
@@ -181,8 +182,8 @@
   const int64_t er0 = m0 + wm * 64 + (lane >> 3), ec8 = n0 + wn * 64 + (lane & 7) * 8;
   int64_t oC = er0 * p.ldc + ec8, oU = er0 * p.ldu + ec8, oS = ((int64_t)z * p.M + er0) * p.N + ec8;
   const int64_t sC = 8 * p.ldc, sU = 8 * p.ldu, sS = 8 * p.N;
-  uint32_t dbase = (uint32_t)(er0 * p.N + ec8);
-  const uint32_t sD = 8u * (uint32_t)p.N;
+  uint32_t dbase = (uint32_t)(er0 * p.dN + ec8);
+  const uint32_t sD = 8u * (uint32_t)p.dN;
 #pragma unroll
   for (int it = 0; it < 8; ++it, oC += sC, oU += sU, oS += sS, dbase += sD) {
     const int pidx = it * 64 + lane, row = pidx >> 3, c8 = pidx & 7;
@@ -316,6 +317,7 @@
   const int64_t ab = ((a_rows - 1) * a->lda + a_cols) * 2, bb = ((b_rows - 1) * a->ldb + b_cols) * 2;
   p.a_bytes = (uint32_t)ab; p.b_bytes = (uint32_t)bb;
   p.drop = make_drop(a->drop_p, a->seed, a->drop_stream);
+  p.dN = nb_drop_pitch(a);
   p.stream_out = 1;
   p.gn = (int)(a->N / BN);
   const int epi = a->epilogue;
diff --git a/n-best-asr-transformer_amd/csrc/gemm_bf16_v2.hip b/n-best-asr-transformer_amd/csrc/gemm_bf16_v2.hip
--- a/n-best-asr-transformer_amd/csrc/gemm_bf16_v2.hip
+++ b/n-best-asr-transformer_amd/csrc/gemm_bf16_v2.hip
@@ -9,6 +9,7 @@
   const bf16* A; const bf16* B; void* C; const float* bias; const bf16* R; bf16* U; float* slab; float* colpart;
   int64_t M, N, K, lda, ldb, ldc, ldr, ldu;
   int64_t k_per_split;
+  int64_t dN;
   int tiles_m, tiles_n, splits, accumulate;
   uint32_t a_bytes, b_bytes;
   uint32_t c_bytes, r_bytes, u_bytes;
@@ -618,7 +619,7 @@
 #pragma unroll
     for (int j = 0; j < TNt; ++j) colacc[j] = 0.f;
     const uint32_t voC = (uint32_t)((drow0 * p.ldc + dcol) * 2), svC = (uint32_t)(2 * p.ldc);
-    const uint32_t dbase0 = (uint32_t)(drow0 * p.N + dcol), sD = (uint32_t)p.N;
+    const uint32_t dbase0 = (uint32_t)(drow0 * p.dN + dcol), sD = (uint32_t)p.dN;
     constexpr bool kCols = (EPI == NBEST_EPI_DGELU);
     const bool want_cols = kCols && p.colpart != nullptr;
 #pragma unroll
@@ -718,8 +719,8 @@
   int64_t oC = erow0 * p.ldc + en8, oU = erow0 * p.ldu + en8;
   int64_t oS = ((int64_t)z * p.M + erow0) * p.N + en8;
   const int64_t sC = 8 * p.ldc, sU = 8 * p.ldu, sS = 8 * p.N;
-  uint32_t dbase = (uint32_t)(erow0 * p.N + en8);
-  const uint32_t sD = 8u * (uint32_t)p.N;
+  uint32_t dbase = (uint32_t)(erow0 * p.dN + en8);
+  const uint32_t sD = 8u * (uint32_t)p.dN;
 #pragma unroll
   for (int c = 0; c < TMt / 2; ++c) {
 #pragma unroll
@@ -1014,6 +1015,7 @@
     p.u_bytes = a->U ? (uint32_t)(a->M * a->ldu) : 0;
   }
   p.drop = make_drop(a->drop_p, a->seed, a->drop_stream);
+  p.dN = nb_drop_pitch(a);
   p.stream_out = 1;
   p.gn = (!a->trans_a && !a->trans_b) ? nb_group_cols(a->N / pl.bn, (int64_t)pl.bn * a->K * 2, 2400) : (int)(a->N / pl.bn);
   if (pl.bm == 128 && pl.bn >= 384 && (a->N / pl.bn) % 2 == 0) p.gn = 2;
diff --git a/n-best-asr-transformer_amd/csrc/gemm_f32.hip b/n-best-asr-transformer_amd/csrc/gemm_f32.hip
--- a/n-best-asr-transformer_amd/csrc/gemm_f32.hip
+++ b/n-best-asr-transformer_amd/csrc/gemm_f32.hip
@@ -7,6 +7,7 @@
 struct GemmF {
   const float* A; const float* B; float* C; const float* bias; const float* R; float* U;
   int64_t M, N, K, lda, ldb, ldc, ldr, ldu;
+  int64_t dN;
   int accumulate;
   DropCfg drop;
 };
@@ -69,7 +70,7 @@
       if (EPI == NBEST_EPI_BIAS_GELU) { p.U[m * p.ldu + n] = dgelu_f(v); v = gelu_f(v); }
       if (EPI == kEpiBiasGeluNoU) v = gelu_f(v);
       if (EPI == NBEST_EPI_BIAS_DROP_RES) {
-        if (p.drop.thr16) v = nb_keep(p.drop, (uint32_t)(m * p.N + n)) ? v * p.drop.scale : 0.f;
+        if (p.drop.thr16) v = nb_keep(p.drop, (uint32_t)(m * p.dN + n)) ? v * p.drop.scale : 0.f;
         v += p.R[m * p.ldr + n];
       }
       if (EPI == NBEST_EPI_RES) v += p.R[m * p.ldr + n];
@@ -102,6 +103,7 @@
   p.U = (float*)a->U;
   p.M = a->M; p.N = a->N; p.K = a->K; p.lda = a->lda; p.ldb = a->ldb; p.ldc = a->ldc; p.ldr = a->ldr; p.ldu = a->ldu;
   p.accumulate = a->accumulate;
+  p.dN = nb_drop_pitch(a);
   p.drop = make_drop(a->drop_p, a->seed, a->drop_stream);
   dim3 grid((unsigned)((a->N + TN - 1) / TN), (unsigned)((a->M + TM - 1) / TM));
   const int kepi = nb_kernel_epilogue(a->epilogue, a->U);
diff --git a/n-best-asr-transformer_amd/csrc/internal.h b/n-best-asr-transformer_amd/csrc/internal.h
--- a/n-best-asr-transformer_amd/csrc/internal.h
+++ b/n-best-asr-transformer_amd/csrc/internal.h
@@ -15,6 +15,12 @@
                                   void* dx_drop, float* dgamma, float* dbeta, float* dbias, int64_t M, int H, int dtype,
                                   int accumulate, float drop_p, uint64_t seed, uint32_t drop_stream, void* ws,
                                   size_t ws_bytes, nbest_stream_t stream, Fp8Grad f8);
+struct LnRows { int64_t y_ld, dy_ld, dx_ld; int drop_row_stride; };
+int nbest_internal_layernorm_fwd_rows(const void* x, const float* gamma, const float* beta, void* y, float* stats, int64_t M, int H,
+                                      float eps, int dtype, nbest_stream_t stream, LnRows rows);
+int nbest_internal_layernorm_bwd_rows(const void* dy, const void* x, const float* stats, const float* gamma, void* dx, void* dx_drop,
+                                      float* dgamma, float* dbeta, float* dbias, int64_t M, int H, int dtype, int accumulate, float drop_p,
+                                      uint64_t seed, uint32_t drop_stream, void* ws, size_t ws_bytes, nbest_stream_t stream, LnRows rows);
 int nbest_internal_partial_rows_sum(const float* part, int nrows, int N, float* out, int accumulate, hipStream_t st);
 void nbest_internal_rowred_batch_begin();
 void nbest_internal_rowred_batch_abort();
diff --git a/n-best-asr-transformer_amd/csrc/norm_embed.hip b/n-best-asr-transformer_amd/csrc/norm_embed.hip
--- a/n-best-asr-transformer_amd/csrc/norm_embed.hip
+++ b/n-best-asr-transformer_amd/csrc/norm_embed.hip
@@ -16,7 +16,7 @@
 template <typename T, int VPL>
 __global__ __launch_bounds__(256) void ln_fwd_kernel(const T* __restrict__ x, const float* __restrict__ gamma,
                                                      const float* __restrict__ beta, T* __restrict__ y,
-                                                     float* __restrict__ stats, int64_t M, int H, float eps) {
+                                                     float* __restrict__ stats, int64_t M, int H, float eps, int64_t y_ld) {
   const int lane = threadIdx.x & 63, wpb = blockDim.x >> 6, nvec = H >> 2;
   const float invH = 1.0f / (float)H;
   for (int64_t row = (int64_t)blockIdx.x * wpb + (threadIdx.x >> 6); row < M; row += (int64_t)gridDim.x * wpb) {
@@ -36,7 +36,7 @@
       if (c < nvec) { f32x4 d = v[i] - mean; q += sum4(d * d); }
     }
     const float rstd = 1.0f / sqrtf(wave_sum(q) * invH + eps);
-    T* yr = y + row * H;
+    T* yr = y + row * y_ld;
 #pragma unroll
     for (int i = 0; i < VPL; ++i) {
       const int c = lane + 64 * i;
@@ -127,7 +127,8 @@
 __global__ __launch_bounds__(256) void ln_bwd_kernel(const T* __restrict__ dy, const T* __restrict__ x,
                                                      const float* __restrict__ stats, const float* __restrict__ gamma,
                                                      T* __restrict__ dx, T* __restrict__ dx_drop, float* __restrict__ part,
-                                                     int64_t M, int H, int rows_per_block, int with_dbias, DropCfg drop) {
+                                                     int64_t M, int H, int rows_per_block, int with_dbias, DropCfg drop,
+                                                     int64_t dy_ld, int64_t dx_ld, int64_t drop_ld) {
   extern __shared__ __attribute__((aligned(16))) float acc[];
   const int lane = threadIdx.x & 63, wave = threadIdx.x >> 6, wpb = blockDim.x >> 6, nvec = H >> 2;
   const float invH = 1.0f / (float)H;
@@ -153,7 +154,7 @@
 #pragma unroll
       for (int i = 0; i < VPL; ++i) {
         const int c = lane + 64 * i;
-        if (c < nvec) { nx[i] = Vec4<T>::raw_load(x + row * H + 4 * c); nd[i] = Vec4<T>::raw_load(dy + row * H + 4 * c); }
+        if (c < nvec) { nx[i] = Vec4<T>::raw_load(x + row * H + 4 * c); nd[i] = Vec4<T>::raw_load(dy + row * dy_ld + 4 * c); }
       }
     }
   }
@@ -168,7 +169,7 @@
 #pragma unroll
       for (int i = 0; i < VPL; ++i) {
         const int c = lane + 64 * i;
-        if (c < nvec) { nx[i] = Vec4<T>::raw_load(x + nrow * H + 4 * c); nd[i] = Vec4<T>::raw_load(dy + nrow * H + 4 * c); }
+        if (c < nvec) { nx[i] = Vec4<T>::raw_load(x + nrow * H + 4 * c); nd[i] = Vec4<T>::raw_load(dy + nrow * dy_ld + 4 * c); }
       }
     }
     f32x4 xh[VPL], g[VPL], d[VPL];
@@ -193,13 +194,13 @@
       const int c = lane + 64 * i;
       if (c < nvec) {
         f32x4 o = (g[i] - s1 - xh[i] * s2) * rstd;
-        Vec4<T>::store(dx + row * H + 4 * c, o);
+        Vec4<T>::store(dx + row * dx_ld + 4 * c, o);
         if constexpr (PARAMS) {
           ag[i] += d[i] * xh[i];
           ab[i] += d[i];
         }
         if (drop.thr16) {
-          const uint32_t k = nb_keep4(drop, (uint32_t)(row * H + 4 * c));
+          const uint32_t k = nb_keep4(drop, (uint32_t)(row * drop_ld + 4 * c));
 #pragma unroll
           for (int e = 0; e < 4; ++e) o[e] = (k >> e & 1) ? o[e] * drop.scale : 0.f;
           Vec4<T>::store(dx_drop + row * H + 4 * c, o);
@@ -1083,16 +1084,18 @@
          (size_t)chunks * 2 * H * sizeof(float) + (size_t)(chunks + 4) * sizeof(int);
 }
 
-int nbest_internal_layernorm_fwd8(const void* x, const float* gamma, const float* beta, void* y, void* y8, float* stats,
-                                  int64_t M, int H, float eps, int dtype, nbest_stream_t stream, const uint32_t* a_prev, uint32_t* a_new) {
+static int ln_fwd_impl(const void* x, const float* gamma, const float* beta, void* y, void* y8, float* stats, int64_t M, int H, float eps,
+                       int dtype, nbest_stream_t stream, const uint32_t* a_prev, uint32_t* a_new, const LnRows* rows) {
   if (int e = check_h(H)) return e;
+  const int64_t y_ld = (rows && rows->y_ld) ? rows->y_ld : H;
+  NB_CHECK(y_ld >= H && y_ld % 4 == 0 && (!rows || !y8), NBEST_ERR_ARG, "layernorm_fwd: bad row pitch %lld", (long long)y_ld);
   NB_CHECK(x && gamma && beta && y && stats && M > 0, NBEST_ERR_ARG, "layernorm_fwd: null pointer or M <= 0");
   NB_CHECK(!y8 || (dtype == NBEST_BF16 && H % 256 == 0 && H <= 1024), NBEST_ERR_SHAPE, "layernorm_fwd: fp8 copy needs bf16 and H in {256..1024}");
   hipStream_t st = (hipStream_t)stream;
   const int grid0 = grid_rows(M, 4);
   if (dtype == NBEST_F32) {
-    DISPATCH_VPL(H, (ln_fwd_kernel<float, VPL><<<grid0, 256, 0, st>>>((const float*)x, gamma, beta, (float*)y, stats, M, H, eps)));
-  } else if (dtype == NBEST_BF16 && H % 256 == 0 && H <= 1024) {
+    DISPATCH_VPL(H, (ln_fwd_kernel<float, VPL><<<grid0, 256, 0, st>>>((const float*)x, gamma, beta, (float*)y, stats, M, H, eps, y_ld)));
+  } else if (dtype == NBEST_BF16 && H % 256 == 0 && H <= 1024 && !rows) {
     const int grid = grid0 < 1024 ? grid0 : 1024;
     switch (H / 256) {
       case 1: ln_fwd_fast_kernel<1><<<grid, 256, 0, st>>>((const bf16*)x, gamma, beta, (bf16*)y, stats, M, eps, (uint8_t*)y8, a_prev, a_new); break;
@@ -1101,29 +1104,41 @@
       default: ln_fwd_fast_kernel<4><<<grid, 256, 0, st>>>((const bf16*)x, gamma, beta, (bf16*)y, stats, M, eps, (uint8_t*)y8, a_prev, a_new); break;
     }
   } else if (dtype == NBEST_BF16) {
-    DISPATCH_VPL(H, (ln_fwd_kernel<bf16, VPL><<<grid0, 256, 0, st>>>((const bf16*)x, gamma, beta, (bf16*)y, stats, M, H, eps)));
+    DISPATCH_VPL(H, (ln_fwd_kernel<bf16, VPL><<<grid0, 256, 0, st>>>((const bf16*)x, gamma, beta, (bf16*)y, stats, M, H, eps, y_ld)));
   } else NB_CHECK(false, NBEST_ERR_DTYPE, "layernorm_fwd: bad dtype %d", dtype);
   NB_LAUNCH_CHECK();
   return NBEST_OK;
 }
 
+int nbest_internal_layernorm_fwd8(const void* x, const float* gamma, const float* beta, void* y, void* y8, float* stats,
+                                  int64_t M, int H, float eps, int dtype, nbest_stream_t stream, const uint32_t* a_prev, uint32_t* a_new) {
+  return ln_fwd_impl(x, gamma, beta, y, y8, stats, M, H, eps, dtype, stream, a_prev, a_new, nullptr);
+}
+int nbest_internal_layernorm_fwd_rows(const void* x, const float* gamma, const float* beta, void* y, float* stats, int64_t M, int H,
+                                      float eps, int dtype, nbest_stream_t stream, LnRows rows) {
+  return ln_fwd_impl(x, gamma, beta, y, nullptr, stats, M, H, eps, dtype, stream, nullptr, nullptr, &rows);
+}
+
 extern "C" int nbest_layernorm_fwd(const void* x, const float* gamma, const float* beta, void* y, float* stats,
                                    int64_t M, int H, float eps, int dtype, nbest_stream_t stream) {
   return nbest_internal_layernorm_fwd8(x, gamma, beta, y, nullptr, stats, M, H, eps, dtype, stream, nullptr, nullptr);
 }
 
-int nbest_internal_layernorm_bwd8(const void* dy, const void* x, const float* stats, const float* gamma, void* dx,
-                                  void* dx_drop, float* dgamma, float* dbeta, float* dbias, int64_t M, int H, int dtype,
-                                  int accumulate, float drop_p, uint64_t seed, uint32_t drop_stream, void* ws,
-                                  size_t ws_bytes, nbest_stream_t stream, Fp8Grad f8) {
+static int ln_bwd_impl(const void* dy, const void* x, const float* stats, const float* gamma, void* dx, void* dx_drop, float* dgamma,
+                       float* dbeta, float* dbias, int64_t M, int H, int dtype, int accumulate, float drop_p, uint64_t seed,
+                       uint32_t drop_stream, void* ws, size_t ws_bytes, nbest_stream_t stream, Fp8Grad f8, const LnRows* rows) {
   if (int e = check_h(H)) return e;
+  const int64_t dy_ld = (rows && rows->dy_ld) ? rows->dy_ld : H, dx_ld = (rows && rows->dx_ld) ? rows->dx_ld : H;
+  const int64_t drs = (rows && rows->drop_row_stride > 1) ? rows->drop_row_stride : 1, drop_ld = drs * H;
+  NB_CHECK(dy_ld >= H && dx_ld >= H && dy_ld % 4 == 0 && dx_ld % 4 == 0 && (!rows || !f8.amax_new), NBEST_ERR_ARG,
+           "layernorm_bwd: bad row pitch (%lld, %lld)", (long long)dy_ld, (long long)dx_ld);
   NB_CHECK(!f8.amax_new || (dtype == NBEST_BF16 && H % 256 == 0 && H <= 1024), NBEST_ERR_SHAPE, "layernorm_bwd: fp8 copy needs bf16 and H in {256..1024}");
   const bool params = dgamma || dbeta || dbias;
   NB_CHECK(dy && x && stats && gamma && dx && M > 0 && (!params || (dgamma && dbeta && ws)), NBEST_ERR_ARG, "layernorm_bwd: null pointer");
   NB_CHECK(!params || ws_bytes >= nbest_rowred_ws_bytes(M, H), NBEST_ERR_WORKSPACE, "layernorm_bwd: workspace too small");
   const DropCfg d = make_drop(drop_p, seed, drop_stream);
   NB_CHECK(d.thr16 == 0 || (dx_drop && dx_drop != dx) || (!dx_drop && f8.out8), NBEST_ERR_ARG, "layernorm_bwd: dropout needs a separate dx_drop buffer");
-  NB_CHECK(M * (int64_t)H < (int64_t)1 << 32 || d.thr16 == 0, NBEST_ERR_SHAPE, "layernorm_bwd: dropout counter overflow");
+  NB_CHECK((M - 1) * drop_ld + H < (int64_t)1 << 32 || d.thr16 == 0, NBEST_ERR_SHAPE, "layernorm_bwd: dropout counter overflow");
   hipStream_t st = (hipStream_t)stream;
   int nblk = (int)((M + 31) / 32 < 1 ? 1 : ((M + 31) / 32 > kMaxLnBwdBlocks ? kMaxLnBwdBlocks : (M + 31) / 32));
   if (nblk > 512) nblk = 512;
@@ -1136,8 +1151,8 @@
   if (!params) {
     if (dtype == NBEST_F32) {
       DISPATCH_VPL(H, (ln_bwd_kernel<float, VPL, false><<<nblk, 256, 0, st>>>((const float*)dy, (const float*)x, stats, gamma,
-                                                                               (float*)dx, (float*)dx_drop, nullptr, M, H, rpb, 0, d)));
-    } else if (dtype == NBEST_BF16 && H % 256 == 0 && H <= 1024) {
+                                                                               (float*)dx, (float*)dx_drop, nullptr, M, H, rpb, 0, d, dy_ld, dx_ld, drop_ld)));
+    } else if (dtype == NBEST_BF16 && H % 256 == 0 && H <= 1024 && !rows) {
 #define NB_LNB0(V, D) ln_bwd_fast_kernel<V, D, false, waves, false><<<nblk, waves * 64, 0, st>>>((const bf16*)dy, (const bf16*)x, stats, gamma, \
                                                                                                (bf16*)dx, (bf16*)dx_drop, nullptr, M, rpb, d, f8)
 #define NB_LNB0_V(V)                      \
@@ -1155,15 +1170,15 @@
 #undef NB_LNB0
     } else if (dtype == NBEST_BF16) {
       DISPATCH_VPL(H, (ln_bwd_kernel<bf16, VPL, false><<<nblk, 256, 0, st>>>((const bf16*)dy, (const bf16*)x, stats, gamma,
-                                                                              (bf16*)dx, (bf16*)dx_drop, nullptr, M, H, rpb, 0, d)));
+                                                                              (bf16*)dx, (bf16*)dx_drop, nullptr, M, H, rpb, 0, d, dy_ld, dx_ld, drop_ld)));
     } else NB_CHECK(false, NBEST_ERR_DTYPE, "layernorm_bwd: bad dtype %d", dtype);
     NB_LAUNCH_CHECK();
     return NBEST_OK;
   }
   if (dtype == NBEST_F32) {
     DISPATCH_VPL(H, (ln_bwd_kernel<float, VPL><<<nblk, 256, smem, st>>>((const float*)dy, (const float*)x, stats, gamma,
-                                                                         (float*)dx, (float*)dx_drop, part, M, H, rpb, wb, d)));
-  } else if (dtype == NBEST_BF16 && H % 256 == 0 && H <= 1024) {
+                                                                         (float*)dx, (float*)dx_drop, part, M, H, rpb, wb, d, dy_ld, dx_ld, drop_ld)));
+  } else if (dtype == NBEST_BF16 && H % 256 == 0 && H <= 1024 && !rows) {
 #define NB_LNB(V, D, B)                                                                                                        \
   do {                                                                                                                         \
     if (waves == 8) {                                                                                                          \
@@ -1190,10 +1205,24 @@
 #undef NB_LNB
   } else if (dtype == NBEST_BF16) {
     DISPATCH_VPL(H, (ln_bwd_kernel<bf16, VPL><<<nblk, 256, smem, st>>>((const bf16*)dy, (const bf16*)x, stats, gamma,
-                                                                        (bf16*)dx, (bf16*)dx_drop, part, M, H, rpb, wb, d)));
+                                                                        (bf16*)dx, (bf16*)dx_drop, part, M, H, rpb, wb, d, dy_ld, dx_ld, drop_ld)));
   } else NB_CHECK(false, NBEST_ERR_DTYPE, "layernorm_bwd: bad dtype %d", dtype);
   NB_LAUNCH_CHECK();
   return finalize(part, nblk, H, dgamma, accumulate, dbeta, accumulate, dbias, accumulate, st);
+}
+
+int nbest_internal_layernorm_bwd8(const void* dy, const void* x, const float* stats, const float* gamma, void* dx,
+                                  void* dx_drop, float* dgamma, float* dbeta, float* dbias, int64_t M, int H, int dtype,
+                                  int accumulate, float drop_p, uint64_t seed, uint32_t drop_stream, void* ws,
+                                  size_t ws_bytes, nbest_stream_t stream, Fp8Grad f8) {
+  return ln_bwd_impl(dy, x, stats, gamma, dx, dx_drop, dgamma, dbeta, dbias, M, H, dtype, accumulate, drop_p, seed, drop_stream, ws, ws_bytes,
+                     stream, f8, nullptr);
+}
+int nbest_internal_layernorm_bwd_rows(const void* dy, const void* x, const float* stats, const float* gamma, void* dx, void* dx_drop,
+                                      float* dgamma, float* dbeta, float* dbias, int64_t M, int H, int dtype, int accumulate, float drop_p,
+                                      uint64_t seed, uint32_t drop_stream, void* ws, size_t ws_bytes, nbest_stream_t stream, LnRows rows) {
+  return ln_bwd_impl(dy, x, stats, gamma, dx, dx_drop, dgamma, dbeta, dbias, M, H, dtype, accumulate, drop_p, seed, drop_stream, ws, ws_bytes,
+                     stream, Fp8Grad{nullptr, nullptr, nullptr}, &rows);
 }
 
 extern "C" int nbest_layernorm_bwd(const void* dy, const void* x, const float* stats, const float* gamma, void* dx,
diff --git a/n-best-asr-transformer_amd/hipabi.py b/n-best-asr-transformer_amd/hipabi.py
--- a/n-best-asr-transformer_amd/hipabi.py
+++ b/n-best-asr-transformer_amd/hipabi.py
@@ -32,7 +32,8 @@
                 ("trans_a", C.c_int32), ("trans_b", C.c_int32), ("epilogue", C.c_int32), ("dtype", C.c_int32),
                 ("accumulate", C.c_int32), ("drop_p", C.c_float), ("drop_stream", C.c_uint32), ("seed", C.c_uint64),
                 ("colsum_out", C.c_void_p), ("colsum_accumulate", C.c_int32), ("flags", C.c_int32),
-                ("B_packed", C.c_void_p), ("b_pack_bn", C.c_int32), ("pad_", C.c_int32)]
+                ("B_packed", C.c_void_p), ("b_pack_bn", C.c_int32), ("pad_", C.c_int32),
+                ("drop_row_stride", C.c_int32), ("pad2_", C.c_int32)]
 
 
 class GemmFp8Args(C.Structure):
@@ -75,7 +76,7 @@
                 ("w8", C.c_void_p), ("w8_inv_scale", C.c_void_p), ("w8t", C.c_void_p), ("gamax_prev", C.c_void_p),
                 ("gamax_new", C.c_void_p), ("fp8_bwd", C.c_int32), ("pad2", C.c_int32),
                 ("wpk", C.c_void_p), ("wpkt", C.c_void_p), ("w8p", C.c_void_p), ("w8tp", C.c_void_p),
-                ("word_perm", C.c_void_p), ("aamax_prev", C.c_void_p), ("aamax_new", C.c_void_p), ("fp8_act", C.c_int32), ("pad4", C.c_int32),
+                ("word_perm", C.c_void_p), ("aamax_prev", C.c_void_p), ("aamax_new", C.c_void_p), ("fp8_act", C.c_int32), ("cls_last_layer", C.c_int32),
                 ("first_trainable", C.c_int32), ("no_input_grad", C.c_int32), ("wgrad_skip_host", C.c_void_p),
                 ("base_ids", C.c_void_p), ("alpha", C.c_void_p), ("no_param_grad", C.c_int32), ("pad5", C.c_int32)]
     wgrad_group = property(lambda self: self.pad5, lambda self, v: setattr(self, "pad5", int(v)))
@@ -249,7 +250,7 @@
 
 def gemm(A, B, M, N, K, trans_a=False, trans_b=False, epilogue=EPI_NONE, bias=None, R=None, U=None, out=None,
          accumulate=False, drop_p=0.0, seed=0, drop_stream=0, colsum_out=None, defer_reduce=False, B_packed=None, b_pack_bn=0,
-         want_u=True):
+         want_u=True, drop_row_stride=0):
     dt = dtype_code(A.dtype)
     dev = A.device
     if out is None:
@@ -269,6 +270,7 @@
     g.accumulate, g.drop_p, g.drop_stream, g.seed = int(accumulate), drop_p, drop_stream, seed
     g.colsum_out = colsum_out.data_ptr() if colsum_out is not None else None
     g.flags = 1 if defer_reduce else 0
+    g.drop_row_stride = int(drop_row_stride)
     if B_packed is not None:
         g.B_packed, g.b_pack_bn = B_packed.data_ptr(), b_pack_bn
     nb = lib().nbest_gemm_ws_bytes(C.byref(g))
diff --git a/n-best-asr-transformer_amd/model.py b/n-best-asr-transformer_amd/model.py
--- a/n-best-asr-transformer_amd/model.py
+++ b/n-best-asr-transformer_amd/model.py
@@ -83,6 +83,7 @@
         d.drop_stream_base = 1000 * slot if train else 0
         d.first_trainable = first_trainable
         d.wgrad_group = model.wgrad_group
+        d.cls_last_layer = int(model.cls_last_layer)
         if model.fp8_forward and train:
             d.w8, d.w8_inv_scale = a.w8.data_ptr(), a.w8_inv_scale.data_ptr()
         self.desc = d
@@ -147,12 +148,14 @@
 
 class NBestSTCModel(nn.Module):
     def __init__(self, cfg: EncoderConfig, labels: LabelSpace, device="cuda", compute_dtype=torch.bfloat16, dropout=0.0,
-                 seed=999, fp8_forward=False, fp8_backward=None, wgrad_group=hb.WGRAD_GROUP_PLAN):
+                 seed=999, fp8_forward=False, fp8_backward=None, wgrad_group=hb.WGRAD_GROUP_PLAN,
+                 cls_last_layer=True):
         super().__init__()
         self.cfg, self.labels, self.compute_dtype = cfg, labels, compute_dtype
         self.dropout = float(dropout)
         self.device = torch.device(device)
         self.wgrad_group = int(wgrad_group)
+        self.cls_last_layer = bool(cls_last_layer)
         self.arena = ParamArena(cfg, labels, self.device, compute_dtype)
         self.fp8_forward = bool(fp8_forward)
         self.fp8_backward = self.fp8_forward if fp8_backward is None else bool(fp8_backward)
```
